# coganlab/cross_patient_speech_decoding

Hardware: AMD Instinct MI355X
Metric: ECoG trials/sec seq2seq-RNN training (higher is better)
Workload: dtype bf16x3; 1 GPU; configs[3] per-GPU shard: 8-patient MCCA-aligned input (d = 30), enc 2x bi-GRU H=512, dec 1x GRU, T=200 (T'=20), F=100, full-batch step of 2048 trials per GPU (8 patients x 2048 trials over 8 GPUs), dropout 0.3, teacher forcing 0.5, clip 0.5, AdamW; trials_per_gpu=2048, global_batch=2048, parallelism=dp1, collective=none (single process)

## Files before the change

cross_patient_speech_decoding_amd/csrc/xps_gru.hip:

```cpp
#include <stdlib.h>
#include "xps_common.h"
#include "xps_gemm_tile.h"
using xps_tile::bf16x4;
using xps_tile::bf16x8;
using xps_tile::bf_split;

bool xps_internal_gru_cluster_usable(int B, int H, int ndir);
size_t xps_internal_gru_cluster_fwd_workspace(int B, int H, int ndir);
size_t xps_internal_gru_cluster_bwd_workspace(int B, int H, int ndir);
size_t xps_internal_gru_cluster_status_offset(int B, int H, int ndir);
int xps_internal_gru_cluster_fwd(const float* gi, const float* const* w_hh, const float* const* b_hh, const float* h0,
                                 float* y_ext, float* saved, int T, int B, int H, int ndir, void* workspace, hipStream_t st,
                                 float* y_split, float* yd_split, float drop_p, unsigned long long drop_seed);
int xps_internal_gru_cluster_bwd(const float* dy, const float* dhn, const float* y_ext, const float* saved,
                                 const float* const* w_hh_t, float* dgi, float* dghn, float* dh0,
                                 int T, int B, int H, int ndir, void* workspace, hipStream_t st, int split_out);
bool xps_internal_gru_cluster_ximg_ok(int B, int H, int ndir);

namespace {

constexpr int GBM = 16;
#ifndef XPS_GRU_BF_WAVES
#define XPS_GRU_BF_WAVES 8
#endif
constexpr int GRU_BF_WAVES = XPS_GRU_BF_WAVES;

struct GruFwdParams {
    const float* gi;
    const float* w_hh[2];
    const float* b_hh[2];
    const float* h0;
    float* y_ext;
    float* saved;
    int T, B, H, ndir, Hp, ldh;
    float* y_drop;
    float drop_p, drop_scale;
    unsigned long long drop_seed;
};

template <bool VEC>
__device__ inline float4 load_w4(const float* __restrict__ row, int k, int H) {
    if (VEC) {
        if (k + 3 < H) return *reinterpret_cast<const float4*>(row + k);
    }
    float4 t = make_float4(0.f, 0.f, 0.f, 0.f);
    if (k + 0 < H) t.x = row[k + 0];
    if (k + 1 < H) t.y = row[k + 1];
    if (k + 2 < H) t.z = row[k + 2];
    if (k + 3 < H) t.w = row[k + 3];
    return t;
}

__device__ inline float f4get(const float4& v, int i) { return i == 0 ? v.x : (i == 1 ? v.y : (i == 2 ? v.z : v.w)); }

template <bool VEC>
__global__ __launch_bounds__(256) void gru_fwd_kernel(GruFwdParams p) {
    extern __shared__ __attribute__((aligned(16))) float lds[];
    const int tid = threadIdx.x, lane = tid & 63, wave = tid >> 6;
    const int n = lane & 15, kq = lane >> 4;
    const int dir = blockIdx.y, b0 = blockIdx.x * GBM;
    const int T = p.T, B = p.B, H = p.H, Hp = p.Hp, ldh = p.ldh;
    const int ldy = p.ndir * H;
    const float* __restrict__ W = p.w_hh[dir];
    const float* __restrict__ bh = p.b_hh[dir];
    const float* __restrict__ gi = p.gi + (long long)dir * T * B * 3 * H;

    for (int i = tid; i < 2 * GBM * ldh; i += 256) lds[i] = 0.f;
    __syncthreads();
    {
        const int slot_h0 = (dir == 0) ? 0 : T + 1, slot_other = (dir == 0) ? T + 1 : 0;
        for (int i = tid; i < GBM * H; i += 256) {
            const int r = i / H, k = i % H, b = b0 + r;
            if (b < B) {
                float v = p.h0 ? p.h0[((long long)dir * B + b) * H + k] : 0.f;
                lds[r * ldh + k] = v;
                p.y_ext[((long long)slot_h0 * B + b) * ldy + dir * H + k] = v;
                p.y_ext[((long long)slot_other * B + b) * ldy + dir * H + k] = 0.f;
            }
        }
    }
    __syncthreads();

    const int ntile = Hp / 16;
    for (int s = 0; s < T; ++s) {
        const int t = (dir == 0) ? s : T - 1 - s;
        const float* hc = lds + (s & 1) * GBM * ldh;
        float* hn = lds + ((s & 1) ^ 1) * GBM * ldh;

        for (int jt = wave; jt < ntile; jt += 4) {
            const int j = jt * 16 + n;
            const int jc = j < H ? j : H - 1;
            float g_r[4], g_z[4], g_n[4];
#pragma unroll
            for (int i = 0; i < 4; ++i) {
                int b = b0 + 4 * kq + i;
                b = b < B ? b : B - 1;
                const float* gp = gi + ((long long)t * B + b) * 3 * H;
                g_r[i] = gp[jc];
                g_z[i] = gp[H + jc];
                g_n[i] = gp[2 * H + jc];
// ... 941 lines not shown
    const int t = (dir == 0) ? p.s : T - 1 - p.s;
    const int slot_prev = (dir == 0) ? t : t + 2;
    const float* __restrict__ in_dhn = p.dhn;
    const float* __restrict__ in_keep = p.keep_in;
    const float* __restrict__ in_dy = p.dy;
    const float* __restrict__ in_saved = p.saved;
    const float* __restrict__ in_y = p.y_ext;
    float* __restrict__ out_dgi = p.dgi;
    float* __restrict__ out_dghn = p.dghn;
    float* __restrict__ out_keep = p.keep_out;
    float* __restrict__ out_dh0 = p.dh0;
#pragma unroll
    for (int jn = 0; jn < 2; ++jn) {
        const int j = n0 + wn + jn * 32 + li;
        if (j >= H) continue;
        float v_base[16], v_dy[16], v_r[16], v_z[16], v_n[16], v_q[16], v_hp[16];
#pragma unroll
        for (int r = 0; r < 16; ++r) {
            const int b = m0 + wm + (r & 3) + 8 * (r >> 2) + 4 * lk;
            const bool ok = b < B;
            const int bc = ok ? b : 0;
            const long long ob = ((long long)dir * B + bc) * H + j;
            v_base[r] = p.first ? (in_dhn ? in_dhn[ob] : 0.f) : in_keep[ob];
            if (!p.final) {
                v_dy[r] = in_dy ? in_dy[((long long)t * B + bc) * ldy + dir * H + j] : 0.f;
                const float* sv = in_saved + (((long long)dir * T + t) * B + bc) * 4 * H;
                v_r[r] = sv[j]; v_z[r] = sv[H + j]; v_n[r] = sv[2 * H + j]; v_q[r] = sv[3 * H + j];
                v_hp[r] = in_y[((long long)slot_prev * B + bc) * ldy + dir * H + j];
            }
        }
#pragma unroll
        for (int r = 0; r < 16; ++r) {
            const int b = m0 + wm + (r & 3) + 8 * (r >> 2) + 4 * lk;
            if (b >= B) continue;
            const long long ob = ((long long)dir * B + b) * H + j;
            float dh = p.first ? v_base[r] : acc[0][jn][r] + v_base[r];
            if (p.final) { out_dh0[ob] = dh; continue; }
            dh += v_dy[r];
            const float rg = v_r[r], zg = v_z[r], ng = v_n[r], q = v_q[r], hp = v_hp[r];
            const float dn = dh * (1.f - zg);
            const float dz = dh * (hp - ng);
            const float dan = dn * (1.f - ng * ng);
            const long long o = (((long long)dir * T + t) * B + b) * 3 * H;
            out_dgi[o + j] = dan * q * rg * (1.f - rg);
            out_dgi[o + H + j] = dz * zg * (1.f - zg);
            out_dgi[o + 2 * H + j] = dan;
            out_dghn[(((long long)dir * T + t) * B + b) * H + j] = dan * rg;
            out_keep[ob] = dh * zg;
        }
    }
}

__global__ void transpose_kernel(const float* __restrict__ src, float* __restrict__ dst, int rows, int cols) {
    __shared__ float tile[32][33];
    const int bx = blockIdx.x * 32, by = blockIdx.y * 32;
    for (int i = threadIdx.y; i < 32; i += blockDim.y) {
        int r = by + i, c = bx + threadIdx.x;
        tile[i][threadIdx.x] = (r < rows && c < cols) ? src[(long long)r * cols + c] : 0.f;
    }
    __syncthreads();
    for (int i = threadIdx.y; i < 32; i += blockDim.y) {
        int c = bx + i, r = by + threadIdx.x;
        if (c < cols && r < rows) dst[(long long)c * rows + r] = tile[threadIdx.x][i];
    }
}

struct TransposeBatch { const float* src[4]; float* dst[4]; };
__global__ void transpose_batched_kernel(TransposeBatch tb, int rows, int cols) {
    __shared__ float tile[32][33];
    const float* __restrict__ src = tb.src[blockIdx.z];
    float* __restrict__ dst = tb.dst[blockIdx.z];
    const int bx = blockIdx.x * 32, by = blockIdx.y * 32;
    for (int i = threadIdx.y; i < 32; i += blockDim.y) {
        int r = by + i, c = bx + threadIdx.x;
        tile[i][threadIdx.x] = (r < rows && c < cols) ? src[(long long)r * cols + c] : 0.f;
    }
    __syncthreads();
    for (int i = threadIdx.y; i < 32; i += blockDim.y) {
        int c = bx + i, r = by + threadIdx.x;
        if (c < cols && r < rows) dst[(long long)c * rows + r] = tile[threadIdx.x][i];
    }
}

inline bool aligned16(const void* p) { return (reinterpret_cast<uintptr_t>(p) & 15) == 0; }

inline bool use_step_path() {
    static const bool on = [] { const char* e = getenv("XPS_GRU_STEP_PATH"); return !(e && e[0] == '0'); }();
    return on;
}

}

static bool cluster_shape_ok(int T, int B, int H, int ndir) {
    return xps_internal_gru_cluster_usable(B, H, ndir) && (long long)ndir * (T + 2) * B * 4 * H * 4 < (1ll << 32);
}

extern "C" size_t xps_gru_seq_fwd_f32_workspace(int T, int B, int H, int ndir) {
    if (T <= 0 || B <= 0 || H <= 0 || (ndir != 1 && ndir != 2)) return 16;
    return cluster_shape_ok(T, B, H, ndir) ? xps_internal_gru_cluster_fwd_workspace(B, H, ndir) : 16;
}

extern "C" long long xps_gru_seq_status_offset(int T, int B, int H, int ndir) {
    if (T <= 0 || B <= 0 || H <= 0 || (ndir != 1 && ndir != 2)) return -1;
    return cluster_shape_ok(T, B, H, ndir) ? (long long)xps_internal_gru_cluster_status_offset(B, H, ndir) : -1;
}

extern "C" int xps_gru_seq_fused_dropout_supported(int T, int B, int H, int ndir) {
    if (T < 1 || B < 1 || (ndir != 1 && ndir != 2)) return 0;
    if (cluster_shape_ok(T, B, H, ndir)) return 0;
    return (H == 128 || H == 64) ? 1 : 0;
}

static int gru_seq_fwd_impl(const float* gi, const float* const* w_hh, const float* const* b_hh,
                            const float* h0, float* y_ext, float* saved,
                            int T, int B, int H, int ndir, float* y_drop, float drop_p, unsigned long long drop_seed,
                            void* workspace, size_t workspace_bytes, void* stream);

extern "C" int xps_gru_seq_fwd_f32(const float* gi, const float* const* w_hh, const float* const* b_hh,
                                   const float* h0, float* y_ext, float* saved,
                                   int T, int B, int H, int ndir, void* workspace, size_t workspace_bytes, void* stream) {
    return gru_seq_fwd_impl(gi, w_hh, b_hh, h0, y_ext, saved, T, B, H, ndir, nullptr, 0.f, 0ull, workspace, workspace_bytes, stream);
}

extern "C" int xps_gru_seq_fwd_drop_f32(const float* gi, const float* const* w_hh, const float* const* b_hh,
                                        const float* h0, float* y_ext, float* saved,
                                        int T, int B, int H, int ndir, float* y_drop, float drop_p, uint64_t drop_seed,
                                        void* workspace, size_t workspace_bytes, void* stream) {
    XPS_CHECK_ARG(y_drop && drop_p >= 0.f && drop_p < 1.f, "y_drop must be given, 0 <= p < 1");
    XPS_CHECK_ARG(xps_gru_seq_fused_dropout_supported(T, B, H, ndir) && aligned16(y_drop),
                  "fused dropout: shape not on the resident kernels (see xps_gru_seq_fused_dropout_supported)");
    return gru_seq_fwd_impl(gi, w_hh, b_hh, h0, y_ext, saved, T, B, H, ndir, y_drop, drop_p, (unsigned long long)drop_seed, workspace,
                            workspace_bytes, stream);
}

extern "C" int xps_gru_seq_fwd_images_supported(int T, int B, int H, int ndir) {
    if (T < 1 || B < 1 || H < 1 || (ndir != 1 && ndir != 2)) return 0;
    return (cluster_shape_ok(T, B, H, ndir) && xps_internal_gemm_mode() == 1 && H % 4 == 0) ? 1 : 0;
}

extern "C" int xps_gru_seq_fwd_image_exchange_supported(int T, int B, int H, int ndir) {
    return (xps_gru_seq_fwd_images_supported(T, B, H, ndir) && xps_internal_gru_cluster_ximg_ok(B, H, ndir)) ? 1 : 0;
}

extern "C" int xps_gru_seq_fwd_images_f32(const float* gi, const float* const* w_hh, const float* const* b_hh,
                                          const float* h0, float* y_ext, float* saved, int T, int B, int H, int ndir,
                                          float* y_split, float* y_drop_split, float drop_p, uint64_t drop_seed,
                                          void* workspace, size_t workspace_bytes, void* stream) {
    XPS_CHECK_ARG(gi && w_hh && b_hh && y_ext, "null argument");
    XPS_CHECK_ARG(T >= 1 && B >= 1 && H >= 1 && (ndir == 1 || ndir == 2), "bad shape");
    XPS_CHECK_ARG(drop_p >= 0.f && drop_p < 1.f, "0 <= p < 1");
    XPS_CHECK_ARG(xps_gru_seq_fwd_images_supported(T, B, H, ndir),
                  "XPS_FMT_SPLIT4 images: cluster-persistent shapes in bf16x3 mode only (see xps_gru_seq_fwd_images_supported)");
    XPS_CHECK_ARG(w_hh[0] && b_hh[0] && (ndir == 1 || (w_hh[1] && b_hh[1])), "null weight pointer");
    if (!workspace || workspace_bytes < xps_gru_seq_fwd_f32_workspace(T, B, H, ndir)) {
        xps_set_error("xps_gru_seq_fwd_images_f32: workspace too small");
        return XPS_E_WORKSPACE;
    }
    return xps_internal_gru_cluster_fwd(gi, w_hh, b_hh, h0, y_ext, saved, T, B, H, ndir, workspace, (hipStream_t)stream,
                                        y_split, y_drop_split, drop_p, (unsigned long long)drop_seed);
}

static int gru_seq_fwd_impl(const float* gi, const float* const* w_hh, const float* const* b_hh,
                            const float* h0, float* y_ext, float* saved,
                            int T, int B, int H, int ndir, float* y_drop, float drop_p, unsigned long long drop_seed,
                            void* workspace, size_t workspace_bytes, void* stream) {
    XPS_CHECK_ARG(gi && w_hh && b_hh && y_ext, "null argument");
    XPS_CHECK_ARG(T >= 1 && B >= 1 && H >= 1, "T, B, H must be >= 1");
    XPS_CHECK_ARG(ndir == 1 || ndir == 2, "ndir must be 1 or 2");
    if (cluster_shape_ok(T, B, H, ndir)) {
        XPS_CHECK_ARG(w_hh[0] && b_hh[0] && (ndir == 1 || (w_hh[1] && b_hh[1])), "null weight pointer");
        if (!workspace || workspace_bytes < xps_gru_seq_fwd_f32_workspace(T, B, H, ndir)) {
            xps_set_error("xps_gru_seq_fwd_f32: workspace too small");
            return XPS_E_WORKSPACE;
        }
        return xps_internal_gru_cluster_fwd(gi, w_hh, b_hh, h0, y_ext, saved, T, B, H, ndir, workspace, (hipStream_t)stream,
                                            nullptr, nullptr, 0.f, 0ull);
    }
    GruFwdParams p;
    p.gi = gi; p.h0 = h0; p.y_ext = y_ext; p.saved = saved;
    p.T = T; p.B = B; p.H = H; p.ndir = ndir;
    p.y_drop = y_drop; p.drop_p = drop_p; p.drop_scale = 1.0f / (1.0f - drop_p); p.drop_seed = drop_seed;
    p.Hp = ((H + 15) / 16) * 16;
    p.ldh = p.Hp + 4;
    bool vec = (H % 4 == 0);
    for (int d = 0; d < 2; ++d) {
        p.w_hh[d] = w_hh[d < ndir ? d : 0];
        p.b_hh[d] = b_hh[d < ndir ? d : 0];
        XPS_CHECK_ARG(p.w_hh[d] && p.b_hh[d], "null weight pointer");
        vec = vec && aligned16(p.w_hh[d]);
    }
    const size_t lds_bytes = (size_t)2 * GBM * p.ldh * sizeof(float);
    XPS_CHECK_ARG(lds_bytes <= 160 * 1024, "hidden size too large for the LDS-resident state tile");
    XPS_CHECK_ARG(!y_drop || vec, "fused dropout needs 16-byte aligned weights");
    if (H > 128 && use_step_path()) {
        hipStream_t st = (hipStream_t)stream;
        hipLaunchKernelGGL(gru_init_slots_kernel, dim3(cdiv((long long)ndir * B * H, 256) > 1024 ? 1024 : cdiv((long long)ndir * B * H, 256)),
                           dim3(256), 0, st, h0, y_ext, T, B, H, ndir);
        GruStepFwd q;
        q.gi = gi; q.y_ext = y_ext; q.saved = saved; q.T = T; q.B = B; q.H = H; q.ndir = ndir;
        for (int d = 0; d < 2; ++d) { q.w_hh[d] = p.w_hh[d]; q.b_hh[d] = p.b_hh[d]; }
        q.vecA = (int)(H % 4 == 0 && aligned16(y_ext));
        q.vecB = (int)vec;
        dim3 sgrid(cdiv(H, 32), cdiv(B, 128), ndir);
        for (int s = 0; s < T; ++s) {
            q.s = s;
            if (xps_internal_gemm_mode() == 1) hipLaunchKernelGGL(gru_step_fwd_kernel<true>, sgrid, dim3(256), 0, st, q);
            else hipLaunchKernelGGL(gru_step_fwd_kernel<false>, sgrid, dim3(256), 0, st, q);
        }
        XPS_CHECK_LAUNCH();
        return XPS_OK;
    }
    dim3 grid(cdiv(B, GBM), ndir);
    if (vec && (H == 128 || H == 64)) {
        const bool bf = xps_internal_gemm_mode() == 1;
        if (H == 128 && bf) hipLaunchKernelGGL((gru_fwd_resident_kernel<128, true, GRU_BF_WAVES>), grid, dim3(GRU_BF_WAVES * 64), 0, (hipStream_t)stream, p);
        else if (H == 128) hipLaunchKernelGGL((gru_fwd_resident_kernel<128, false>), grid, dim3(256), 0, (hipStream_t)stream, p);
        else if (bf) hipLaunchKernelGGL((gru_fwd_resident_kernel<64, true>), grid, dim3(256), 0, (hipStream_t)stream, p);
        else hipLaunchKernelGGL((gru_fwd_resident_kernel<64, false>), grid, dim3(256), 0, (hipStream_t)stream, p);
        XPS_CHECK_LAUNCH();
        return XPS_OK;
    }
    if (vec) {
        if (lds_bytes > 64 * 1024)
            if (hipFuncSetAttribute((const void*)gru_fwd_kernel<true>, hipFuncAttributeMaxDynamicSharedMemorySize, (int)lds_bytes) != hipSuccess) { xps_set_error("hipFuncSetAttribute failed"); return XPS_E_HIP; }
        hipLaunchKernelGGL(gru_fwd_kernel<true>, grid, dim3(256), lds_bytes, (hipStream_t)stream, p);
    } else {
        if (lds_bytes > 64 * 1024)
            if (hipFuncSetAttribute((const void*)gru_fwd_kernel<false>, hipFuncAttributeMaxDynamicSharedMemorySize, (int)lds_bytes) != hipSuccess) { xps_set_error("hipFuncSetAttribute failed"); return XPS_E_HIP; }
        hipLaunchKernelGGL(gru_fwd_kernel<false>, grid, dim3(256), lds_bytes, (hipStream_t)stream, p);
    }
    XPS_CHECK_LAUNCH();
    return XPS_OK;
}

extern "C" size_t xps_gru_seq_bwd_f32_workspace(int T, int B, int H, int ndir) {
    (void)T;
    if (B <= 0 || H <= 0 || ndir <= 0) return 16;
    if (T > 0 && (ndir == 1 || ndir == 2) && cluster_shape_ok(T, B, H, ndir)) return xps_internal_gru_cluster_bwd_workspace(B, H, ndir);
    return (size_t)2 * ndir * B * H * sizeof(float) + 16;
}

static int gru_seq_bwd_impl(const float* dy, const float* dhn, const float* y_ext, const float* saved,
                            const float* const* w_hh, const float* const* w_hh_t, float* dgi, float* dghn, float* dh0,
                            int T, int B, int H, int ndir, int has_drop, float drop_p, unsigned long long drop_seed,
                            void* workspace, size_t workspace_bytes, void* stream, int split_out = 0);

extern "C" int xps_gru_seq_bwd_f32(const float* dy, const float* dhn, const float* y_ext, const float* saved,
                                   const float* const* w_hh, const float* const* w_hh_t, float* dgi, float* dghn, float* dh0,
                                   int T, int B, int H, int ndir, void* workspace, size_t workspace_bytes, void* stream) {
    return gru_seq_bwd_impl(dy, dhn, y_ext, saved, w_hh, w_hh_t, dgi, dghn, dh0, T, B, H, ndir, 0, 0.f, 0ull, workspace, workspace_bytes, stream);
}

extern "C" int xps_gru_seq_bwd_drop_f32(const float* dy, const float* dhn, const float* y_ext, const float* saved,
                                        const float* const* w_hh, const float* const* w_hh_t, float* dgi, float* dghn, float* dh0,
                                        int T, int B, int H, int ndir, float drop_p, uint64_t drop_seed,
                                        void* workspace, size_t workspace_bytes, void* stream) {
    XPS_CHECK_ARG(dy && drop_p >= 0.f && drop_p < 1.f, "dy must be given, 0 <= p < 1");
    XPS_CHECK_ARG(xps_gru_seq_fused_dropout_supported(T, B, H, ndir),
                  "fused dropout: shape not on the resident kernels (see xps_gru_seq_fused_dropout_supported)");
    return gru_seq_bwd_impl(dy, dhn, y_ext, saved, w_hh, w_hh_t, dgi, dghn, dh0, T, B, H, ndir, 1, drop_p, (unsigned long long)drop_seed,
                            workspace, workspace_bytes, stream);
}

extern "C" int xps_gru_seq_bwd_split4_supported(int T, int B, int H, int ndir) {
    if (T < 1 || B < 1 || (ndir != 1 && ndir != 2) || xps_internal_gemm_mode() != 1) return 0;
    if (cluster_shape_ok(T, B, H, ndir)) return 1;
    return xps_gru_seq_fused_dropout_supported(T, B, H, ndir);
}

extern "C" int xps_gru_seq_bwd_split4_f32(const float* dy, const float* dhn, const float* y_ext, const float* saved,
                                          const float* const* w_hh, const float* const* w_hh_t, float* dgi, float* dghn, float* dh0,
                                          int T, int B, int H, int ndir, float drop_p, uint64_t drop_seed,
                                          void* workspace, size_t workspace_bytes, void* stream) {
    XPS_CHECK_ARG(drop_p >= 0.f && drop_p < 1.f, "0 <= p < 1");
    XPS_CHECK_ARG(drop_p == 0.f || (dy && xps_gru_seq_fused_dropout_supported(T, B, H, ndir) && !cluster_shape_ok(T, B, H, ndir)),
                  "fused dropout: dy must be given and the shape must be on the resident kernels");
    return gru_seq_bwd_impl(dy, dhn, y_ext, saved, w_hh, w_hh_t, dgi, dghn, dh0, T, B, H, ndir, drop_p > 0.f ? 1 : 0, drop_p,
                            (unsigned long long)drop_seed, workspace, workspace_bytes, stream, 1);
}

static int gru_seq_bwd_impl(const float* dy, const float* dhn, const float* y_ext, const float* saved,
                            const float* const* w_hh, const float* const* w_hh_t, float* dgi, float* dghn, float* dh0,
                            int T, int B, int H, int ndir, int has_drop, float drop_p, unsigned long long drop_seed,
                            void* workspace, size_t workspace_bytes, void* stream, int split_out) {
    XPS_CHECK_ARG(y_ext && saved && w_hh && w_hh_t && dgi && dghn, "null argument");
    XPS_CHECK_ARG(!split_out || xps_gru_seq_bwd_split4_supported(T, B, H, ndir),
                  "XPS_FMT_SPLIT4 outputs: shape / precision mode not served (see xps_gru_seq_bwd_split4_supported)");
    XPS_CHECK_ARG(dy || dhn, "at least one of dy / dhn must be given");
    XPS_CHECK_ARG(T >= 1 && B >= 1 && H >= 1, "T, B, H must be >= 1");
    XPS_CHECK_ARG(ndir == 1 || ndir == 2, "ndir must be 1 or 2");
    if (cluster_shape_ok(T, B, H, ndir)) {
        XPS_CHECK_ARG(w_hh_t[0] && (ndir == 1 || w_hh_t[1]), "null weight pointer");
        if (!workspace || workspace_bytes < xps_gru_seq_bwd_f32_workspace(T, B, H, ndir)) {
            xps_set_error("xps_gru_seq_bwd_f32: workspace too small");
            return XPS_E_WORKSPACE;
        }
        return xps_internal_gru_cluster_bwd(dy, dhn, y_ext, saved, w_hh_t, dgi, dghn, dh0, T, B, H, ndir, workspace, (hipStream_t)stream, split_out);
    }
    GruBwdParams p;
    p.dy = dy; p.dhn = dhn; p.y_ext = y_ext; p.saved = saved; p.dgi = dgi; p.dghn = dghn; p.dh0 = dh0;
    p.T = T; p.B = B; p.H = H; p.ndir = ndir;
    p.has_drop = has_drop; p.drop_p = drop_p; p.drop_scale = 1.0f / (1.0f - drop_p); p.drop_seed = drop_seed;
    p.split_out = split_out;
    p.Hp = ((H + 15) / 16) * 16;
    p.ldg = 3 * p.Hp + 4;
    p.ldc = p.Hp + 4;
    bool vec = (H % 4 == 0);
    for (int d = 0; d < 2; ++d) {
        p.w_hh_t[d] = w_hh_t[d < ndir ? d : 0];
        XPS_CHECK_ARG(p.w_hh_t[d], "null weight pointer");
        vec = vec && aligned16(p.w_hh_t[d]);
    }
    const size_t lds_bytes = (size_t)GBM * (p.ldg + p.ldc) * sizeof(float);
    XPS_CHECK_ARG(lds_bytes <= 160 * 1024, "hidden size too large for the LDS-resident gradient tile");
    XPS_CHECK_ARG(!has_drop || vec, "fused dropout needs 16-byte aligned weights");
    XPS_CHECK_ARG(!split_out || (vec && (H == 128 || H == 64)), "XPS_FMT_SPLIT4 outputs need the resident kernels (16-byte aligned weights)");
    if (H > 128 && use_step_path()) {
        if (!workspace || workspace_bytes < xps_gru_seq_bwd_f32_workspace(T, B, H, ndir) || !aligned16(workspace)) {
            xps_set_error("xps_gru_seq_bwd_f32: workspace too small or misaligned");
            return XPS_E_WORKSPACE;
        }
        hipStream_t st = (hipStream_t)stream;
        GruStepBwd q;
        q.dy = dy; q.dhn = dhn; q.y_ext = y_ext; q.saved = saved; q.dgi = dgi; q.dghn = dghn; q.dh0 = dh0;
        q.T = T; q.B = B; q.H = H; q.ndir = ndir;
        bool vb = (H % 4 == 0);
        for (int d = 0; d < 2; ++d) {
            q.w_hh[d] = w_hh[d < ndir ? d : 0];
            XPS_CHECK_ARG(q.w_hh[d], "null weight pointer");
            vb = vb && aligned16(q.w_hh[d]);
        }
        q.vecB = (int)vb;
        q.vecA1 = (int)(H % 4 == 0 && aligned16(dgi));
        q.vecA2 = (int)(H % 4 == 0 && aligned16(dghn));
        float* keep[2] = {(float*)workspace, (float*)workspace + (size_t)ndir * B * H};
        dim3 sgrid(cdiv(H, 128), cdiv(B, 64), ndir);
        int pp = 0;
        for (int s = T - 1; s >= 0; --s) {
            q.s = s; q.first = (s == T - 1); q.final = 0;
            q.keep_in = keep[pp]; q.keep_out = keep[pp ^ 1];
            if (xps_internal_gemm_mode() == 1) hipLaunchKernelGGL(gru_step_bwd_kernel<true>, sgrid, dim3(256), 0, st, q);
            else hipLaunchKernelGGL(gru_step_bwd_kernel<false>, sgrid, dim3(256), 0, st, q);
            pp ^= 1;
        }
        if (dh0) {
            q.s = 0; q.first = 0; q.final = 1; q.keep_in = keep[pp]; q.keep_out = keep[pp ^ 1];
            if (xps_internal_gemm_mode() == 1) hipLaunchKernelGGL(gru_step_bwd_kernel<true>, sgrid, dim3(256), 0, st, q);
            else hipLaunchKernelGGL(gru_step_bwd_kernel<false>, sgrid, dim3(256), 0, st, q);
        }
        XPS_CHECK_LAUNCH();
        return XPS_OK;
    }
    dim3 grid(cdiv(B, GBM), ndir);
    if (vec && (H == 128 || H == 64)) {
        const bool bf = xps_internal_gemm_mode() == 1;
        if (H == 128 && bf) hipLaunchKernelGGL((gru_bwd_resident_kernel<128, true, GRU_BF_WAVES>), grid, dim3(GRU_BF_WAVES * 64), 0, (hipStream_t)stream, p);
        else if (H == 128) hipLaunchKernelGGL((gru_bwd_resident_kernel<128, false>), grid, dim3(256), 0, (hipStream_t)stream, p);
        else if (bf) hipLaunchKernelGGL((gru_bwd_resident_kernel<64, true>), grid, dim3(256), 0, (hipStream_t)stream, p);
        else hipLaunchKernelGGL((gru_bwd_resident_kernel<64, false>), grid, dim3(256), 0, (hipStream_t)stream, p);
        XPS_CHECK_LAUNCH();
        return XPS_OK;
    }
    if (vec) {
        if (lds_bytes > 64 * 1024)
            if (hipFuncSetAttribute((const void*)gru_bwd_kernel<true>, hipFuncAttributeMaxDynamicSharedMemorySize, (int)lds_bytes) != hipSuccess) { xps_set_error("hipFuncSetAttribute failed"); return XPS_E_HIP; }
        hipLaunchKernelGGL(gru_bwd_kernel<true>, grid, dim3(256), lds_bytes, (hipStream_t)stream, p);
    } else {
        if (lds_bytes > 64 * 1024)
            if (hipFuncSetAttribute((const void*)gru_bwd_kernel<false>, hipFuncAttributeMaxDynamicSharedMemorySize, (int)lds_bytes) != hipSuccess) { xps_set_error("hipFuncSetAttribute failed"); return XPS_E_HIP; }
        hipLaunchKernelGGL(gru_bwd_kernel<false>, grid, dim3(256), lds_bytes, (hipStream_t)stream, p);
    }
    XPS_CHECK_LAUNCH();
    return XPS_OK;
}

#ifdef XPS_STAMP
extern "C" int xps_debug_read_stamps(unsigned long long* host, int n) {
    return hipMemcpyFromSymbol(host, HIP_SYMBOL(g_stamp), sizeof(unsigned long long) * n) == hipSuccess ? 0 : -2;
}
#endif

extern "C" int xps_transpose_f32(const float* src, float* dst, int rows, int cols, void* stream) {
    XPS_CHECK_ARG(src && dst && rows >= 0 && cols >= 0, "bad argument");
    if (rows == 0 || cols == 0) return XPS_OK;
    dim3 grid(cdiv(cols, 32), cdiv(rows, 32));
    hipLaunchKernelGGL(transpose_kernel, grid, dim3(32, 8), 0, (hipStream_t)stream, src, dst, rows, cols);
    XPS_CHECK_LAUNCH();
    return XPS_OK;
}

extern "C" int xps_transpose_batched_f32(const float* const* src, float* const* dst, int n, int rows, int cols, void* stream) {
    XPS_CHECK_ARG(src && dst && n >= 1 && n <= 4 && rows >= 0 && cols >= 0, "bad argument (1..4 matrices)");
    if (rows == 0 || cols == 0) return XPS_OK;
    TransposeBatch tb;
    for (int i = 0; i < 4; ++i) {
        const int j = i < n ? i : 0;
        XPS_CHECK_ARG(src[j] && dst[j], "null matrix pointer");
        tb.src[i] = src[j]; tb.dst[i] = dst[j];
    }
    hipLaunchKernelGGL(transpose_batched_kernel, dim3(cdiv(cols, 32), cdiv(rows, 32), n), dim3(32, 8), 0, (hipStream_t)stream,
                       tb, rows, cols);
    XPS_CHECK_LAUNCH();
    return XPS_OK;
}
```

cross_patient_speech_decoding_amd/csrc/xps_gru_cluster.hip:

```cpp
#include <stdlib.h>
#include <string.h>
#include <type_traits>
#include "xps_common.h"
#include <atomic>
#include "xps_gemm_tile.h"
using xps_tile::bf16x4;
using xps_tile::bf16x8;
using xps_tile::bf_split;

namespace {

typedef unsigned u32x4 __attribute__((ext_vector_type(4)));
typedef unsigned u32x2 __attribute__((ext_vector_type(2)));
constexpr int AUX_SC1 = 16;
constexpr unsigned RSRC_FLAGS = 0x00020000;

template <int KSPLIT, bool BF, int KSEG>
struct ClCfg {
    static constexpr int KP = 256 * KSPLIT;
    static constexpr int NUT = 4 / KSPLIT;
    static constexpr int U = 16 * NUT;
    static constexpr int CHUNK_BYTES = 32 * KP * 4;
    static constexpr int NPIECE = CHUNK_BYTES / 1024;
    static constexpr int TRIAL_BYTES = KP * 4;
    static constexpr int PPT = TRIAL_BYTES / 1024;
    static constexpr int TS = TRIAL_BYTES + 32;
    static constexpr int PS = BF ? (PPT == 2 ? 1040 : 512) : 0;
    static constexpr int TILE_BYTES = 32 * TS;
    static constexpr int XACC_BYTES = KSEG == 1 ? 4 * 2 * 3 * 1024 : 2 * 4 * 2 * 1024;
    static constexpr int LDS_BYTES = 2 * TILE_BYTES + XACC_BYTES + 64;
    static constexpr int KSEGS = KSEG;
    __host__ __device__ static constexpr int piece_off(int j) {
        return PPT == 2 ? (j >> 1) * TS + (j & 1) * (BF ? PS : 1024) : j * TS;
    }
};

#ifdef XPS_CL_STAMP
__device__ unsigned long long g_clstamp[2048 * 8];
__device__ unsigned long long g_clstamp2[2048 * 8];
#define CL_STAMP(var)                                                                  \
    __builtin_amdgcn_sched_barrier(0);                                                 \
    asm volatile("s_memtime %0\n\ts_waitcnt lgkmcnt(0)" : "=s"(var)::"memory");        \
    __builtin_amdgcn_sched_barrier(0);
#define CL_ACC(sum, a, b) sum += (b) - (a);
#else
#define CL_STAMP(var)
#define CL_ACC(sum, a, b)
#endif

__device__ inline float cl_sigmoid(float x) { return __builtin_amdgcn_rcpf(1.0f + __expf(-x)); }
__device__ inline float cl_tanh(float x) { return 2.0f * cl_sigmoid(2.0f * x) - 1.0f; }

__device__ inline void cl_wait(const unsigned* flags, unsigned need, int cs, int lane, unsigned first, unsigned* status, unsigned* sticky) {
    unsigned v = first;
    if (__all(v >= need)) return;
    const unsigned long long t0 = __builtin_amdgcn_s_memrealtime();
    bool ok = false;
    for (;;) {
        v = need;
        if (lane < cs) v = __hip_atomic_load(flags + lane, __ATOMIC_RELAXED, __HIP_MEMORY_SCOPE_AGENT);
        if (__all(v >= need)) { ok = true; break; }
        __builtin_amdgcn_s_sleep(2);
        if (__builtin_amdgcn_s_memrealtime() - t0 > 300000000ull) break;
    }
    if (lane == 0) {
        const unsigned dt = (unsigned)(__builtin_amdgcn_s_memrealtime() - t0);
        if (!ok) {
            __hip_atomic_store(status, 1u, __ATOMIC_RELAXED, __HIP_MEMORY_SCOPE_AGENT);
            if (sticky) __hip_atomic_store(sticky, 1u, __ATOMIC_RELAXED, __HIP_MEMORY_SCOPE_AGENT);
        }
        __hip_atomic_fetch_add(status + 1, 1u, __ATOMIC_RELAXED, __HIP_MEMORY_SCOPE_AGENT);
        __hip_atomic_fetch_add(status + 2, dt, __ATOMIC_RELAXED, __HIP_MEMORY_SCOPE_AGENT);
        __hip_atomic_fetch_max(status + 3, dt, __ATOMIC_RELAXED, __HIP_MEMORY_SCOPE_AGENT);
    }
}

__device__ inline bool cl_same_xcd(unsigned* tab, int member, int cs, int lane, bool leader, unsigned* status, unsigned* sticky, unsigned* lds_word) {
    if (leader) {
        unsigned id;
        asm volatile("s_getreg_b32 %0, hwreg(HW_REG_XCC_ID)" : "=s"(id));
        id = (id & 15u) + 1u;
        if (lane == 0) __hip_atomic_store(tab + member, id, __ATOMIC_RELAXED, __HIP_MEMORY_SCOPE_AGENT);
        const unsigned long long t0 = __builtin_amdgcn_s_memrealtime();
        unsigned v = id;
        bool ok = false;
        for (;;) {
            v = id;
            if (lane < cs) v = __hip_atomic_load(tab + lane, __ATOMIC_RELAXED, __HIP_MEMORY_SCOPE_AGENT);
// ... 405 lines not shown
            const unsigned so = !live ? CL_OOB : p.saved_mm
                ? (unsigned)((((((long long)dir * T + t) * p.CS + cm.member) * B + b) * 128 + (ju & 31)) * 4)
                : (unsigned)(((((long long)dir * T + t) * B + b) * 4 * H + ju) * 4);
            __builtin_amdgcn_raw_buffer_store_b128(__builtin_bit_cast(u32x4, rg), sr, so, 0, 0);
            __builtin_amdgcn_raw_buffer_store_b128(__builtin_bit_cast(u32x4, zg), sr, live ? so + gstride : CL_OOB, 0, 0);
            __builtin_amdgcn_raw_buffer_store_b128(__builtin_bit_cast(u32x4, ng), sr, live ? so + 2u * gstride : CL_OOB, 0, 0);
            __builtin_amdgcn_raw_buffer_store_b128(__builtin_bit_cast(u32x4, qv), sr, live ? so + 3u * gstride : CL_OOB, 0, 0);
        }
    };
    f32x4 prod[3];
    auto take_products = [&](int rounds_done) {
#pragma unroll
        for (int g = 0; g < 3; ++g) {
            const int ut_ = guq >> 2, te_ = gtr >> 4, lo_ = ((guq & 3) * 16 + (gtr & 15)) * 16;
            const f32x4 lo = *reinterpret_cast<const f32x4*>(xacc + (((2 * ut_) * 2 + te_) * 3 + g) * 1024 + lo_);
            const f32x4 hi = *reinterpret_cast<const f32x4*>(xacc + (((2 * ut_ + 1) * 2 + te_) * 3 + g) * 1024 + lo_);
            prod[g] = lo + hi;
        }
        if (lane == 0) __hip_atomic_store(consumed + hw, (unsigned)rounds_done, __ATOMIC_RELEASE, __HIP_MEMORY_SCOPE_WORKGROUP);
    };

    EpiIn ein[3];
    int s_pv = p.s_begin, r_pv = -1;
    int s_n2 = p.s_begin, r_n2 = 0;
    epi_load(s_n2, r_n2, ein[0]);
    if (++r_n2 == NR) { r_n2 = 0; ++s_n2; }
    if (it_begin + 1 < it_end) epi_load(s_n2, r_n2, ein[1]);
    if (++r_n2 == NR) { r_n2 = 0; ++s_n2; }
    auto round_body = [&](int it, auto SLOT) {
        constexpr int cur = decltype(SLOT)::value;
        constexpr int prv = (cur + 2) % 3;
        if (p.handoff && wave == 4 && lane == 0 && it >= it_begin + 2) {
            int rp = r_pv - 1, sp = s_pv;
            if (rp < 0) { rp = NR - 1; --sp; }
            __hip_atomic_store(myflags + rp * 16 + cm.member, (unsigned)(sp + 1), __ATOMIC_RELAXED, __HIP_MEMORY_SCOPE_AGENT);
        }
        const bool do_poll = p.handoff && wave == 4 && it + 2 < it_end && s_n2 > p.s_begin;
        unsigned fl = 0xffffffffu;
        if (do_poll && lane < p.CS) fl = __hip_atomic_load(myflags + r_n2 * 16 + lane, __ATOMIC_RELAXED, __HIP_MEMORY_SCOPE_AGENT);
        CL_FENCE();
        int younger = 0;
        if (it > it_begin) {
            take_products(it - it_begin);
            epilogue(s_pv, r_pv, ein[prv], prod);
            younger += (has_saved ? 5 : 1) + (images ? 2 : 0) + (img_drop ? 1 : 0);
        }
        CL_FENCE();
        if (it + 2 < it_end) {
            epi_load(s_n2, r_n2, ein[prv]);
#ifndef XPS_CL_ABL_NOLOAD
            younger += 4;
#endif
        }
        CL_FENCE();
        CL_STAMP(sb3)
        cl_wait_vmcnt(younger);
        if (do_poll) cl_wait(myflags + r_n2 * 16, (unsigned)s_n2, p.CS, lane, fl, p.status, p.sticky);
        CL_STAMP(sb0)
        __syncthreads();
        CL_STAMP(sb1)
        CL_ACC(s_bar, sb0, sb1) CL_ACC(s_work, sb2, sb3) CL_ACC(s_drain, sb3, sb0)
#ifdef XPS_CL_STAMP
        sb2 = sb1;
#endif
        if (++r_pv == NR) { r_pv = 0; ++s_pv; }
        if (++r_n2 == NR) { r_n2 = 0; ++s_n2; }
    };
    for (int it = it_begin; it < it_end; it += 3) {
        round_body(it, std::integral_constant<int, 0>{});
        if (it + 1 < it_end) round_body(it + 1, std::integral_constant<int, 1>{});
        if (it + 2 < it_end) round_body(it + 2, std::integral_constant<int, 2>{});
    }
    if (it_end > it_begin) {
        take_products(it_end - it_begin);
        const int slot = (it_end - 1 - it_begin) % 3;
        if (slot == 0) epilogue(s_pv, r_pv, ein[0], prod);
        else if (slot == 1) epilogue(s_pv, r_pv, ein[1], prod);
        else epilogue(s_pv, r_pv, ein[2], prod);
    }
    CL_STORE_STAMPS()
}

template <bool BF>
__global__ void gru_cluster_init_kernel(const float* __restrict__ h0, float* __restrict__ y_ext, void* __restrict__ xbuf,
                                        int T, int B, int H, int ndir, int Bp, int KP, u32x4* __restrict__ header, int header_u4,
                                        float* __restrict__ y_split) {
    for (int i = blockIdx.x * blockDim.x + threadIdx.x; i < header_u4; i += gridDim.x * blockDim.x) header[i] = (u32x4){0u, 0u, 0u, 0u};
    const long long total = (long long)ndir * Bp * (KP / 4);
    for (long long i = (long long)blockIdx.x * blockDim.x + threadIdx.x; i < total; i += (long long)gridDim.x * blockDim.x) {
        const int k = (int)(i % (KP / 4)) * 4;
        const long long rb = i / (KP / 4);
        const int b = (int)(rb % Bp), dir = (int)(rb / Bp);
        f32x4 v = {0.f, 0.f, 0.f, 0.f};
        const bool in = b < B && k < H;
        if (in && h0) v = *reinterpret_cast<const f32x4*>(h0 + ((long long)dir * B + b) * H + k);
        if (in) {
            const int slot_h0 = (dir == 0) ? 0 : T + 1, slot_other = (dir == 0) ? T + 1 : 0;
            const int ldy = ndir * H;
            *reinterpret_cast<f32x4*>(y_ext + ((long long)slot_h0 * B + b) * ldy + dir * H + k) = v;
            *reinterpret_cast<f32x4*>(y_ext + ((long long)slot_other * B + b) * ldy + dir * H + k) = (f32x4){0.f, 0.f, 0.f, 0.f};
            if constexpr (BF) {
                if (y_split) {
                    *reinterpret_cast<f32x4*>(y_split + ((long long)slot_h0 * B + b) * ldy + dir * H + k) = split4_pack(v);
                    *reinterpret_cast<f32x4*>(y_split + ((long long)slot_other * B + b) * ldy + dir * H + k) = (f32x4){0.f, 0.f, 0.f, 0.f};
                }
            }
        }
        if (!xbuf) continue;
        unsigned char* row = reinterpret_cast<unsigned char*>(xbuf) + ((long long)dir * Bp + b) * KP * 4;
        if constexpr (BF) {
            if (XPS_CL_FWD_PLANES) {
                bf16x4 sh, sl;
#pragma unroll
                for (int e = 0; e < 4; ++e) { __bf16 a, c; bf_split(v[e], a, c); sh[e] = a; sl[e] = c; }
                *reinterpret_cast<bf16x4*>(row + k * 2) = sh;
                *reinterpret_cast<bf16x4*>(row + KP * 2 + k * 2) = sl;
            } else {
                *reinterpret_cast<f32x4*>(row + (k & ~31) * 4 + cl_xslot((unsigned)k >> 2) * 16) = split4_pack(v);
            }
        } else {
            *reinterpret_cast<f32x4*>(row + k * 4) = v;
        }
    }
}

struct ClBwd {
    const float* dy;
    const float* dhn;
    const float* y_ext;
    const float* saved;
    const float* w_hh_t[2];
    float* dgi;
    float* dghn;
    float* dh0;
    float* keep;
    void* xbuf;
    unsigned* flags;
    unsigned* xcc;
    unsigned* status;
    unsigned* sticky;
    unsigned xbuf_bytes;
    int T, B, H, ndir, Bp, Mc, NR, nblk, CS;
    int ps_begin, ps_end, ps_total, handoff;
    int saved_mm;
    int split_out;
};

template <int KSPLIT, bool BF, bool XOUT = false>
__global__ __launch_bounds__(512, 2) void gru_cluster_bwd_kernel(ClBwd p) {
    static_assert(KSPLIT == 2, "the cluster kernels cover 256 < H <= 512");
    static_assert(!XOUT || BF, "outputs as exchange rows: bf16x3 mode only");
    using Cf = ClCfg<KSPLIT, BF, 3>;
    constexpr int KP = Cf::KP, TS = Cf::TS, PS = Cf::PS, TILE = Cf::TILE_BYTES;
    extern __shared__ __attribute__((aligned(16))) unsigned char smem[];
    unsigned char* xacc = smem + 2 * TILE;
    const unsigned lds0 = cl_lds_base(smem);
    const int tid = threadIdx.x, lane = tid & 63;
    const int wave = __builtin_amdgcn_readfirstlane(tid >> 6);
    const int n = lane & 15, kq = lane >> 4;
    const ClMap cm = cl_map(p.CS);
    const int dir = cm.cluster / p.nblk, blk = cm.cluster % p.nblk;
    const int T = p.T, B = p.B, H = p.H, NR = p.NR;
    const int ldy = p.ndir * H;
    const int m_base = blk * p.Mc;
    const int NQ = 3 * NR;
    unsigned* myflags = p.flags + (long long)cm.cluster * NR * 16;
    const bool fast = !p.handoff || cl_same_xcd(p.xcc + cm.cluster * 16, cm.member, p.CS, lane, wave == 4, p.status, p.sticky, reinterpret_cast<unsigned*>(smem));

    const int hw = wave >= 4 ? wave - 4 : 0;
    const int gtr = 8 * hw + (lane >> 3);
    const int guq = lane & 7;
    const int ju = cm.member * Cf::U + 4 * guq;
    const bool ulive = ju < H;
    const int juc = ulive ? ju : 0;
    __amdgpu_buffer_rsrc_t xr = __builtin_amdgcn_make_buffer_rsrc(p.xbuf, 0, p.xbuf_bytes, RSRC_FLAGS);
    __amdgpu_buffer_rsrc_t kr = __builtin_amdgcn_make_buffer_rsrc(p.keep, 0, (unsigned)((long long)p.ndir * p.CS * B * 32 * 4), RSRC_FLAGS);
    __amdgpu_buffer_rsrc_t gr = __builtin_amdgcn_make_buffer_rsrc(p.dgi, 0, (unsigned)((long long)p.ndir * T * B * 3 * H * 4), RSRC_FLAGS);
    __amdgpu_buffer_rsrc_t nr = __builtin_amdgcn_make_buffer_rsrc(p.dghn, 0, (unsigned)((long long)p.ndir * T * B * H * 4), RSRC_FLAGS);
    __amdgpu_buffer_rsrc_t hr = __builtin_amdgcn_make_buffer_rsrc(p.dh0, 0, p.dh0 ? (unsigned)((long long)p.ndir * B * H * 4) : 0u, RSRC_FLAGS);
    const bool has_dy = p.dy != nullptr;

    const unsigned char* xb = reinterpret_cast<const unsigned char*>(p.xbuf);
    const int dw = wave & 3;
    auto dma_src = [&](int ps_, int r_, int g_) -> const unsigned char* {
        if constexpr (XOUT) {
            const int sp = T - 1 - (ps_ - 1);
            const int tp = (dir == 0) ? sp : T - 1 - sp;
            const long long row = ((long long)dir * T + tp) * B + m_base + 32 * r_ + 8 * dw;
            const float* base = g_ < 2 ? p.dgi + row * 3 * H + g_ * H : p.dghn + row * H;
            return reinterpret_cast<const unsigned char*>(base) + cl_ximg_lane(lane) * 16;
        }
        const size_t chunk = (size_t)(((((ps_ - 1) & 1) * p.ndir + dir) * (p.Bp / 32) + (m_base / 32) + r_) * 3 + g_);
        return xb + chunk * Cf::CHUNK_BYTES + (size_t)(dw * 16) * 1024 + lane * 16;
    };
    auto dma_group = [&](const unsigned char* src, int buf, int grp, int g_ = 0) {
        const int j = dw * 16 + grp * 4;
        const unsigned base = lds0 + (unsigned)(buf * TILE) + (unsigned)((j >> 1) * TS);
        const unsigned h = BF ? PS : 1024;
        if constexpr (XOUT) {
            const long long st = (g_ < 2 ? 3LL : 1LL) * H * 4;
            cl_dma2x2(src + (2 * grp) * st, src + (2 * grp + 1) * st, base, base + h - 1024, base + TS, base + TS + h - 1024);
        } else {
            cl_dma4(src + grp * 4096, base, base + h - 1024, base + TS - 2048, base + TS + h - 3072);
        }
    };

// ... 999 lines not shown
    pl.grid = ndir * pl.nblk * 16;
    pl.flags_bytes = (((size_t)ndir * pl.nblk * (pl.NR * 160 + 16) * 4 + 256 + 255) / 256) * 256;
    pl.keep_bytes = (((size_t)ndir * B * 16 * 32 * 4 + 255) / 256) * 256;
    pl.xbuf = (size_t)2 * ndir * (pl.Bp / C2_RT) * 4 * C2_IMG;
    pl.pbuf = (size_t)2 * ndir * pl.nblk * pl.NR * 64 * 2048;
    pl.ok = pl.xbuf < ((size_t)1 << 31) && pl.pbuf < ((size_t)1 << 32);
    return pl;
}

template <typename K>
bool cl_set_lds(K kernel, int bytes) {
    return hipFuncSetAttribute((const void*)kernel, hipFuncAttributeMaxDynamicSharedMemorySize, bytes) == hipSuccess;
}

inline bool cl_aligned16(const void* p) { return (reinterpret_cast<uintptr_t>(p) & 15) == 0; }

template <typename K>
int cl_resident(K kernel, int lds, int kind, int bf) {
    const int dev = cl_device();
    if (dev < 0) return 0;
    std::atomic<int>& slot = g_cldev[dev].resident[kind][bf];
    int v = slot.load(std::memory_order_relaxed);
    if (v < 0) {
        int per_cu = 0;
        if (hipOccupancyMaxActiveBlocksPerMultiprocessor(&per_cu, (const void*)kernel, 512, (size_t)lds) != hipSuccess) per_cu = 0;
        v = per_cu * cl_num_cus();
        slot.store(v, std::memory_order_relaxed);
    }
    return v;
}

bool cl_ximg_enabled() {
    const char* e = getenv("XPS_GRU_XIMG");
    return !(e && e[0] == '0');
}

bool cl_xout_enabled() {
    const char* e = getenv("XPS_GRU_XOUT");
    return e && e[0] == '1';
}

unsigned* cl_sticky() {
    const int dev = cl_device();
    return dev < 0 ? nullptr : g_cldev[dev].sticky;
}

}

extern "C" int xps_gru_set_status_word(unsigned* device_word) {
    const int dev = cl_device();
    if (dev < 0) { xps_set_error("xps_gru_set_status_word: no current device"); return XPS_E_HIP; }
    g_cldev[dev].sticky = device_word;
    return XPS_OK;
}

bool xps_internal_gru_cluster_usable(int B, int H, int ndir) { return cl_plan(B, H, ndir).ok; }

size_t xps_internal_gru_cluster_fwd_workspace(int B, int H, int ndir) {
    const ClPlan pl = cl_plan(B, H, ndir);
    return pl.ok ? pl.flags_bytes + pl.xbuf_fwd : 0;
}

size_t xps_internal_gru_cluster_bwd_workspace(int B, int H, int ndir) {
    const ClPlan pl = cl_plan(B, H, ndir);
    if (!pl.ok) return 0;
    size_t n = pl.flags_bytes + pl.keep_bytes + pl.xbuf_bwd;
    const ClPlan2 p2 = cl_plan2(B, H, ndir);
    if (p2.ok) { const size_t n2 = p2.flags_bytes + p2.keep_bytes + p2.xbuf + p2.pbuf; if (n2 > n) n = n2; }
    return n;
}

size_t xps_internal_gru_cluster_status_offset(int B, int H, int ndir) {
    const ClPlan pl = cl_plan(B, H, ndir);
    return pl.ok ? pl.flags_bytes - 256 : 0;
}

bool xps_internal_gru_cluster_ximg_ok(int B, int H, int ndir) {
    const ClPlan pl = cl_plan(B, H, ndir);
    return pl.ok && H == pl.KP && pl.Bp == B && cl_ximg_enabled();
}

int xps_internal_gru_cluster_fwd(const float* gi, const float* const* w_hh, const float* const* b_hh, const float* h0,
                                 float* y_ext, float* saved, int T, int B, int H, int ndir, void* workspace, hipStream_t st,
                                 float* y_split, float* yd_split, float drop_p, unsigned long long drop_seed) {
    const ClPlan pl = cl_plan(B, H, ndir);
    if (!pl.ok) { xps_set_error("gru cluster forward: unsupported shape"); return XPS_E_INVALID; }
    const bool bf = xps_internal_gemm_mode() == 1;
    if ((y_split || yd_split) && (!bf || H % 4 != 0 || !cl_aligned16(y_split) || !cl_aligned16(yd_split))) {
        xps_set_error("gru cluster forward: XPS_FMT_SPLIT4 images exist in bf16x3 mode only (H a multiple of 4, 16-byte aligned)");
        return XPS_E_INVALID;
    }
    ClFwd p;
    p.gi = gi; p.y_ext = y_ext; p.saved = saved;
    p.y_split = y_split; p.yd_split = yd_split; p.drop_p = drop_p; p.drop_scale = 1.0f / (1.0f - drop_p); p.drop_seed = drop_seed;
    const bool ximg = bf && y_split && H == pl.KP && pl.Bp == B && cl_ximg_enabled();
    for (int d = 0; d < 2; ++d) { p.w_hh[d] = w_hh[d < ndir ? d : 0]; p.b_hh[d] = b_hh[d < ndir ? d : 0]; }
    if (!cl_aligned16(gi) || !cl_aligned16(y_ext) || !cl_aligned16(saved) || !cl_aligned16(p.w_hh[0]) || !cl_aligned16(p.w_hh[1]) ||
        !cl_aligned16(p.b_hh[0]) || !cl_aligned16(p.b_hh[1]) || !cl_aligned16(h0) || !cl_aligned16(workspace)) {
        xps_set_error("gru cluster forward: operands must be 16-byte aligned");
        return XPS_E_INVALID;
    }
    unsigned char* ws = (unsigned char*)workspace;
    p.flags = (unsigned*)ws;
    p.xcc = p.flags + (size_t)ndir * pl.nblk * pl.NR * 16;
    p.status = (unsigned*)(ws + pl.flags_bytes - 256);
    p.xbuf = ws + pl.flags_bytes;
    p.xbuf_bytes = (unsigned)pl.xbuf_fwd;
    p.T = T; p.B = B; p.H = H; p.ndir = ndir; p.Bp = pl.Bp; p.Mc = pl.Mc; p.NR = pl.NR; p.nblk = pl.nblk; p.CS = pl.CS;
    p.saved_mm = (H % 32 == 0) ? 1 : 0;
    if (pl.CS * pl.U < pl.KP) {
        if (hipMemsetAsync(p.xbuf, 0, pl.xbuf_fwd, st) != hipSuccess) { xps_set_error("gru cluster forward: memset failed"); return XPS_E_HIP; }
    }
    {
        const long long total = (long long)ndir * pl.Bp * (pl.KP / 4);
        const int blocks = (int)((total + 255) / 256 > 2048 ? 2048 : (total + 255) / 256);
        if (bf) hipLaunchKernelGGL(gru_cluster_init_kernel<true>, dim3(blocks), dim3(256), 0, st, h0, y_ext, ximg ? (void*)nullptr : p.xbuf, T, B, H, ndir, pl.Bp, pl.KP, (u32x4*)ws, (int)(pl.flags_bytes / 16), y_split);
        else hipLaunchKernelGGL(gru_cluster_init_kernel<false>, dim3(blocks), dim3(256), 0, st, h0, y_ext, p.xbuf, T, B, H, ndir, pl.Bp, pl.KP, (u32x4*)ws, (int)(pl.flags_bytes / 16), (float*)nullptr);
    }
    p.sticky = cl_sticky();
    auto launch = [&](auto kernel, int lds) -> bool {
        if (!cl_set_lds(kernel, lds)) return false;
        const bool persistent = cl_mode() == 2 && pl.grid <= cl_resident(kernel, lds, ximg ? 3 : 0, bf ? 1 : 0);
        if (persistent) {
            p.s_begin = 0; p.s_end = T; p.handoff = 1;
            hipLaunchKernelGGL(kernel, dim3(pl.grid), dim3(512), lds, st, p);
        } else {
            p.handoff = 0;
            for (int s = 0; s < T; ++s) {
                p.s_begin = s; p.s_end = s + 1;
                hipLaunchKernelGGL(kernel, dim3(pl.grid), dim3(512), lds, st, p);
            }
        }
        return true;
    };
    bool ok;
    ok = ximg ? launch(gru_cluster_fwd_kernel<2, true, true>, ClCfg<2, true, 1>::LDS_BYTES)
       : bf ? launch(gru_cluster_fwd_kernel<2, true>, ClCfg<2, true, 1>::LDS_BYTES) : launch(gru_cluster_fwd_kernel<2, false>, ClCfg<2, false, 1>::LDS_BYTES);
    if (!ok) { xps_set_error("gru cluster forward: cannot raise the dynamic LDS limit"); return XPS_E_HIP; }
    XPS_CHECK_LAUNCH();
    return XPS_OK;
}

int xps_internal_gru_cluster_bwd(const float* dy, const float* dhn, const float* y_ext, const float* saved,
                                 const float* const* w_hh_t, float* dgi, float* dghn, float* dh0,
                                 int T, int B, int H, int ndir, void* workspace, hipStream_t st, int split_out) {
    const ClPlan pl = cl_plan(B, H, ndir);
    if (!pl.ok) { xps_set_error("gru cluster backward: unsupported shape"); return XPS_E_INVALID; }
    const bool bf = xps_internal_gemm_mode() == 1;
    if (split_out && !bf) { xps_set_error("gru cluster backward: XPS_FMT_SPLIT4 outputs exist in bf16x3 mode only"); return XPS_E_INVALID; }
    const ClPlan2 p2 = cl_plan2(B, H, ndir);
    if (bf && p2.ok) {
        ClBwd2 q;
        q.dy = dy; q.dhn = dhn; q.y_ext = y_ext; q.saved = saved; q.dgi = dgi; q.dghn = dghn; q.dh0 = dh0;
        q.split_out = split_out;
        for (int d = 0; d < 2; ++d) q.w_hh_t[d] = w_hh_t[d < ndir ? d : 0];
        if (!cl_aligned16(dy) || !cl_aligned16(dhn) || !cl_aligned16(y_ext) || !cl_aligned16(saved) || !cl_aligned16(q.w_hh_t[0]) ||
            !cl_aligned16(q.w_hh_t[1]) || !cl_aligned16(dgi) || !cl_aligned16(dghn) || !cl_aligned16(dh0) || !cl_aligned16(workspace)) {
            xps_set_error("gru cluster backward: operands must be 16-byte aligned");
            return XPS_E_INVALID;
        }
        unsigned char* ws = (unsigned char*)workspace;
        q.flags = (unsigned*)ws;
        q.xcc = q.flags + (size_t)ndir * p2.nblk * p2.NR * 160;
        q.status = (unsigned*)(ws + p2.flags_bytes - 256);
        q.sticky = cl_sticky();
        q.keep = (float*)(ws + p2.flags_bytes);
        q.xbuf = ws + p2.flags_bytes + p2.keep_bytes;
        q.pbuf = (float*)(ws + p2.flags_bytes + p2.keep_bytes + p2.xbuf);
        q.xbuf_bytes = (unsigned)p2.xbuf;
        q.pbuf_bytes = (unsigned)p2.pbuf;
        q.T = T; q.B = B; q.H = H; q.ndir = ndir; q.Bp = p2.Bp; q.Mc = p2.Mc; q.NR = p2.NR; q.nblk = p2.nblk;
        q.saved_mm = (H % 32 == 0) ? 1 : 0;
        if (hipMemsetAsync(ws, 0, p2.flags_bytes, st) != hipSuccess) { xps_set_error("gru cluster backward: memset failed"); return XPS_E_HIP; }
        const int ps_total = T + (dh0 ? 1 : 0);
        q.ps_total = ps_total;
        if (!cl_set_lds(gru_cluster2_bwd_kernel, C2_LDS)) { xps_set_error("gru cluster backward: cannot raise the dynamic LDS limit"); return XPS_E_HIP; }
        const int n_it = (ps_total - 1) * p2.NR;
        const bool persistent = cl_mode() == 2 && p2.grid <= cl_resident(gru_cluster2_bwd_kernel, C2_LDS, 2, 1);
        if (persistent) {
            q.handoff = 1; q.do_ps0 = 1; q.c_begin = 0; q.c_end = n_it; q.g_begin = 0; q.g_end = n_it;
            hipLaunchKernelGGL(gru_cluster2_bwd_kernel, dim3(p2.grid), dim3(512), C2_LDS, st, q);
        } else {
            q.handoff = 0; q.do_ps0 = 1; q.c_begin = q.c_end = q.g_begin = q.g_end = 0;
            hipLaunchKernelGGL(gru_cluster2_bwd_kernel, dim3(p2.grid), dim3(512), C2_LDS, st, q);
            q.do_ps0 = 0;
            for (int ps = 1; ps < ps_total; ++ps) {
                q.c_begin = (ps - 1) * p2.NR; q.c_end = ps * p2.NR; q.g_begin = q.g_end = 0;
                hipLaunchKernelGGL(gru_cluster2_bwd_kernel, dim3(p2.grid), dim3(512), C2_LDS, st, q);
                q.g_begin = q.c_begin; q.g_end = q.c_end; q.c_begin = q.c_end = 0;
                hipLaunchKernelGGL(gru_cluster2_bwd_kernel, dim3(p2.grid), dim3(512), C2_LDS, st, q);
            }
        }
        XPS_CHECK_LAUNCH();
        return XPS_OK;
    }
    ClBwd p;
    p.dy = dy; p.dhn = dhn; p.y_ext = y_ext; p.saved = saved; p.dgi = dgi; p.dghn = dghn; p.dh0 = dh0;
    if (split_out && !bf) { xps_set_error("gru cluster backward: XPS_FMT_SPLIT4 outputs exist in bf16x3 mode only"); return XPS_E_INVALID; }
    p.split_out = split_out;
    for (int d = 0; d < 2; ++d) p.w_hh_t[d] = w_hh_t[d < ndir ? d : 0];
    if (!cl_aligned16(dy) || !cl_aligned16(dhn) || !cl_aligned16(y_ext) || !cl_aligned16(saved) || !cl_aligned16(p.w_hh_t[0]) ||
        !cl_aligned16(p.w_hh_t[1]) || !cl_aligned16(dgi) || !cl_aligned16(dghn) || !cl_aligned16(dh0) || !cl_aligned16(workspace)) {
        xps_set_error("gru cluster backward: operands must be 16-byte aligned");
        return XPS_E_INVALID;
    }
    unsigned char* ws = (unsigned char*)workspace;
    p.flags = (unsigned*)ws;
    p.xcc = p.flags + (size_t)ndir * pl.nblk * pl.NR * 16;
    p.status = (unsigned*)(ws + pl.flags_bytes - 256);
    p.keep = (float*)(ws + pl.flags_bytes);
    p.xbuf = ws + pl.flags_bytes + pl.keep_bytes;
    p.xbuf_bytes = (unsigned)pl.xbuf_bwd;
    p.T = T; p.B = B; p.H = H; p.ndir = ndir; p.Bp = pl.Bp; p.Mc = pl.Mc; p.NR = pl.NR; p.nblk = pl.nblk; p.CS = pl.CS;
    p.saved_mm = (H % 32 == 0) ? 1 : 0;
    const bool xout = bf && split_out && H == pl.KP && pl.Bp == B && cl_xout_enabled();
    if (hipMemsetAsync(ws, 0, pl.flags_bytes, st) != hipSuccess) { xps_set_error("gru cluster backward: memset failed"); return XPS_E_HIP; }
    if (pl.CS * pl.U < pl.KP) {
        if (hipMemsetAsync(p.xbuf, 0, pl.xbuf_bwd, st) != hipSuccess) { xps_set_error("gru cluster backward: memset failed"); return XPS_E_HIP; }
    }
    const int ps_total = T + (dh0 ? 1 : 0);
    p.ps_total = ps_total;
    p.sticky = cl_sticky();
    auto launch = [&](auto kernel, int lds) -> bool {
        if (!cl_set_lds(kernel, lds)) return false;
        const bool persistent = cl_mode() == 2 && pl.grid <= cl_resident(kernel, lds, xout ? 4 : 1, bf ? 1 : 0);
        if (persistent) {
            p.ps_begin = 0; p.ps_end = ps_total; p.handoff = 1;
            hipLaunchKernelGGL(kernel, dim3(pl.grid), dim3(512), lds, st, p);
        } else {
            p.handoff = 0;
            for (int ps = 0; ps < ps_total; ++ps) {
                p.ps_begin = ps; p.ps_end = ps + 1;
                hipLaunchKernelGGL(kernel, dim3(pl.grid), dim3(512), lds, st, p);
            }
        }
        return true;
    };
    bool ok;
    ok = xout ? launch(gru_cluster_bwd_kernel<2, true, true>, ClCfg<2, true, 3>::LDS_BYTES)
       : bf ? launch(gru_cluster_bwd_kernel<2, true>, ClCfg<2, true, 3>::LDS_BYTES) : launch(gru_cluster_bwd_kernel<2, false>, ClCfg<2, false, 3>::LDS_BYTES);
    if (!ok) { xps_set_error("gru cluster backward: cannot raise the dynamic LDS limit"); return XPS_E_HIP; }
    XPS_CHECK_LAUNCH();
    return XPS_OK;
}

extern "C" long long xps_debug_gru_bwd_status_offset(int B, int H, int ndir) {
    const ClPlan2 p2 = cl_plan2(B, H, ndir);
    if (xps_internal_gemm_mode() == 1 && p2.ok) return (long long)p2.flags_bytes - 256;
    const ClPlan pl = cl_plan(B, H, ndir);
    return pl.ok ? (long long)pl.flags_bytes - 256 : -1;
}

#ifdef XPS_CL_STAMP
extern "C" int xps_debug_read_cluster_stamps2(unsigned long long* host, int n) {
    return hipMemcpyFromSymbol(host, HIP_SYMBOL(g_clstamp2), sizeof(unsigned long long) * n) == hipSuccess ? 0 : -2;
}
extern "C" int xps_debug_read_cluster_stamps(unsigned long long* host, int n) {
    return hipMemcpyFromSymbol(host, HIP_SYMBOL(g_clstamp), sizeof(unsigned long long) * n) == hipSuccess ? 0 : -2;
}
#endif

extern "C" int xps_set_gru_cluster_mode(int mode) {
    if (mode < 0 || mode > 2) { xps_set_error("xps_set_gru_cluster_mode: mode must be 0 (off), 1 (one step per launch) or 2 (persistent)"); return XPS_E_INVALID; }
    g_cluster_mode = mode;
    return XPS_OK;
}
extern "C" int xps_get_gru_cluster_mode(void) { return cl_mode(); }
extern "C" int xps_set_gru_bptt_grid(int two_dimensional) {
    if (two_dimensional != 0 && two_dimensional != 1) { xps_set_error("xps_set_gru_bptt_grid: 0 (1-D cluster kernel) or 1 (4 x 4 grid)"); return XPS_E_INVALID; }
    g_cl2 = two_dimensional;
    return XPS_OK;
}
extern "C" int xps_get_gru_bptt_grid(void) { return cl2_enabled() ? 1 : 0; }
```

cross_patient_speech_decoding_amd/csrc/xps_nn.hip:

```cpp
#include "xps_common.h"
#include "xps_ce.h"

namespace {

constexpr int RED_ROWS = 64;

__global__ __launch_bounds__(256) void colsum_stage1(const float* __restrict__ X, long long ldx, int rows, int cols,
                                                     float* __restrict__ part, float* __restrict__ part_sq) {
    __shared__ float s1[4][64], s2[4][64];
    const int c = blockIdx.x * 64 + (threadIdx.x & 63), rq = threadIdx.x >> 6;
    const int r0 = blockIdx.y * RED_ROWS;
    const int r1 = min(rows, r0 + RED_ROWS);
    float a = 0.f, a2 = 0.f;
    if (c < cols) {
#pragma unroll 4
        for (int r = r0 + rq; r < r1; r += 4) {
            float v = X[(long long)r * ldx + c];
            a += v;
            a2 += v * v;
        }
    }
    s1[rq][threadIdx.x & 63] = a;
    s2[rq][threadIdx.x & 63] = a2;
    __syncthreads();
    if (rq == 0 && c < cols) {
        const int l = threadIdx.x;
        part[(long long)blockIdx.y * cols + c] = (s1[0][l] + s1[1][l]) + (s1[2][l] + s1[3][l]);
        if (part_sq) part_sq[(long long)blockIdx.y * cols + c] = (s2[0][l] + s2[1][l]) + (s2[2][l] + s2[3][l]);
    }
}

constexpr int S2_GROUPS = 16;
__global__ __launch_bounds__(1024) void colsum_stage2(const float* __restrict__ part, const float* __restrict__ part_sq,
                                                      int nparts, int cols, float* __restrict__ out,
                                                      float* __restrict__ out_sq, int accumulate,
                                                      float* __restrict__ acc_lo = nullptr, float* __restrict__ acc_hi = nullptr,
                                                      int split = 0) {
    __shared__ float s1[S2_GROUPS][64], s2[S2_GROUPS][64];
    const int l = threadIdx.x & 63, q = threadIdx.x >> 6;
    const int c = blockIdx.x * 64 + l;
    float a = 0.f, a2 = 0.f;
    if (c < cols) {
        int i = q;
        for (; i + 7 * S2_GROUPS < nparts; i += 8 * S2_GROUPS) {
            float v[8], w[8];
#pragma unroll
            for (int u = 0; u < 8; ++u) {
                v[u] = part[(long long)(i + u * S2_GROUPS) * cols + c];
                w[u] = part_sq ? part_sq[(long long)(i + u * S2_GROUPS) * cols + c] : 0.f;
            }
#pragma unroll
            for (int u = 0; u < 8; ++u) { a += v[u]; a2 += w[u]; }
        }
        for (; i < nparts; i += S2_GROUPS) {
            a += part[(long long)i * cols + c];
            if (part_sq) a2 += part_sq[(long long)i * cols + c];
        }
    }
    s1[q][l] = a;
    s2[q][l] = a2;
    __syncthreads();
    if (q == 0 && c < cols) {
        a = 0.f; a2 = 0.f;
#pragma unroll
        for (int k = 0; k < S2_GROUPS; ++k) { a += s1[k][l]; a2 += s2[k][l]; }
        if (accumulate) {
            a += out[c];
            if (out_sq) a2 += out_sq[c];
        }
        out[c] = a;
        if (out_sq) out_sq[c] = a2;
        if (acc_lo && c < split) acc_lo[c] += a;
        if (acc_hi && c >= split) acc_hi[c - split] += a;
    }
}

__device__ __forceinline__ double bn_stats_mean(const float* __restrict__ stats, double count, int c) {
    return (double)stats[c] / count;
}
__device__ __forceinline__ double bn_stats_var(const float* __restrict__ stats, double count, int F, int c, double m) {
    const double d = m - (double)(float)m;
    double var = (double)stats[F + c] / count - d * d;
    return var < 0 ? 0 : var;
}
// ... 137 lines not shown
                                    long long total, int F) {
    for (long long i = (long long)blockIdx.x * blockDim.x + threadIdx.x; i < total; i += (long long)gridDim.x * blockDim.x) {
        const int c = (int)(i % F);
        float g = dout[i];
        if (mask) g = g * mask[i] * scale;
        if (relu && !(out[i] > 0.f)) g = 0.f;
        const float xh = (y[i] - mean[c]) * rstd[c];
        dy[i] = gamma[c] * rstd[c] * (g - sums[c] * inv_count - xh * sums[F + c] * inv_count);
    }
}

__global__ void gather_rows_kernel(const float* __restrict__ table, const long long* __restrict__ idx, float* __restrict__ out,
                                   int B, int cols, int n_rows) {
    const long long total = (long long)B * cols;
    for (long long i = (long long)blockIdx.x * blockDim.x + threadIdx.x; i < total; i += (long long)gridDim.x * blockDim.x) {
        const int b = (int)(i / cols), c = (int)(i % cols);
        long long r = idx[b];
        r = r < 0 ? 0 : (r >= n_rows ? n_rows - 1 : r);
        out[i] = table[r * cols + c];
    }
}

constexpr int SC_CHUNK = 64, SC_MAXROWS = 16;
__global__ __launch_bounds__(256) void scatter_rows_stage1(const float* __restrict__ dout, const long long* __restrict__ idx,
                                                           float* __restrict__ part, int B, int cols, int n_rows) {
    __shared__ float tab[4][SC_MAXROWS][64];
    const int l = threadIdx.x & 63, q = threadIdx.x >> 6;
    const int c = blockIdx.x * 64 + l;
    for (int r = 0; r < n_rows; ++r) tab[q][r][l] = 0.f;
    const int b0 = blockIdx.y * SC_CHUNK;
    const int b1 = min(B, b0 + SC_CHUNK);
    if (c < cols)
        for (int b = b0 + q; b < b1; b += 4) {
            long long r = idx[b];
            r = r < 0 ? 0 : (r >= n_rows ? n_rows - 1 : r);
            tab[q][r][l] += dout[(long long)b * cols + c];
        }
    __syncthreads();
    if (c < cols)
        for (int r = q; r < n_rows; r += 4)
            part[((long long)blockIdx.y * n_rows + r) * cols + c] = (tab[0][r][l] + tab[1][r][l]) + (tab[2][r][l] + tab[3][r][l]);
}
__global__ __launch_bounds__(256) void scatter_rows_stage2(const float* __restrict__ part, int nchunks, float* __restrict__ dtable,
                                                           long long total, int accumulate) {
    __shared__ float red[4][64];
    const int l = threadIdx.x & 63, w = threadIdx.x >> 6;
    const long long i = (long long)blockIdx.x * 64 + l;
    float a = 0.f;
    if (i < total) {
        int k = w;
        for (; k + 28 < nchunks; k += 32) {
            float v[8];
#pragma unroll
            for (int u = 0; u < 8; ++u) v[u] = part[(long long)(k + 4 * u) * total + i];
#pragma unroll
            for (int u = 0; u < 8; ++u) a += v[u];
        }
        for (; k < nchunks; k += 4) a += part[(long long)k * total + i];
    }
    red[w][l] = a;
    __syncthreads();
    if (w == 0 && i < total) {
        a = (red[0][l] + red[1][l]) + (red[2][l] + red[3][l]);
        dtable[i] = accumulate ? dtable[i] + a : a;
    }
}

__global__ void next_token_kernel(const float* __restrict__ logits, int C, const long long* __restrict__ teacher,
                                  long long tstride, const int* __restrict__ use_teacher, long long* __restrict__ next, int B) {
    const int b = blockIdx.x * blockDim.x + threadIdx.x;
    if (b >= B) return;
    if (use_teacher && teacher && use_teacher[0]) {
        next[b] = teacher[(long long)b * tstride];
        return;
    }
    const float* p = logits + (long long)b * C;
    float best = p[0];
    int bi = 0;
    for (int c = 1; c < C; ++c)
        if (p[c] > best) { best = p[c]; bi = c; }
    next[b] = bi;
}

constexpr int SEL_MAXC = 16;
__global__ __launch_bounds__(256) void decoder_select_kernel(const float* __restrict__ h, const float* __restrict__ w_fc,
                                                             const float* __restrict__ b_fc, float* __restrict__ logits,
                                                             const long long* __restrict__ teacher, long long tstride,
                                                             const int* __restrict__ use_teacher, const float* __restrict__ table,
                                                             long long* __restrict__ next, float* __restrict__ gi_next,
                                                             int B, int H, int C, int ntok) {
    const int lane = threadIdx.x & 63;
    const int b = blockIdx.x * 4 + (threadIdx.x >> 6);
    if (b >= B) return;
    float acc[SEL_MAXC];
#pragma unroll
    for (int c = 0; c < SEL_MAXC; ++c) acc[c] = 0.f;
    const float* hr = h + (long long)b * H;
    for (int k = lane * 4; k < H; k += 256) {
        const f32x4 hv = *reinterpret_cast<const f32x4*>(hr + k);
#pragma unroll
        for (int c = 0; c < SEL_MAXC; ++c) {
            if (c < C) {
                const f32x4 wv = *reinterpret_cast<const f32x4*>(w_fc + (long long)c * H + k);
                acc[c] += (hv[0] * wv[0] + hv[1] * wv[1]) + (hv[2] * wv[2] + hv[3] * wv[3]);
            }
        }
    }
#pragma unroll
    for (int c = 0; c < SEL_MAXC; ++c) {
        if (c < C) {
#pragma unroll
            for (int o = 32; o > 0; o >>= 1) acc[c] += __shfl_xor(acc[c], o);
        }
    }
    float best = 0.f;
    int bi = 0;
#pragma unroll
    for (int c = 0; c < SEL_MAXC; ++c) {
        if (c < C) {
            const float v = acc[c] + b_fc[c];
            if (lane == c) logits[(long long)b * C + c] = v;
            if (c == 0 || v > best) { best = v; bi = c; }
        }
    }
    if (!next) return;
    long long tok = bi;
    if (use_teacher && teacher && use_teacher[0]) tok = teacher[(long long)b * tstride];
    if (lane == 0) next[b] = tok;
    if (gi_next && tok >= 0 && tok < ntok) {
        const float* src = table + tok * 3LL * H;
        float* dst = gi_next + (long long)b * 3 * H;
        for (int k = lane * 4; k < 3 * H; k += 256) *reinterpret_cast<f32x4*>(dst + k) = *reinterpret_cast<const f32x4*>(src + k);
    }
}

__global__ void mask_scale_kernel(const float* __restrict__ x, const float* __restrict__ mask, float scale,
                                  float* __restrict__ out, long long n) {
    for (long long i = (long long)blockIdx.x * blockDim.x + threadIdx.x; i < n; i += (long long)gridDim.x * blockDim.x)
        out[i] = x[i] * mask[i] * scale;
}

template <bool VEC>
__global__ void dropout_kernel(const float* __restrict__ x, float* __restrict__ out, float* __restrict__ mask,
                               long long n, float p, float scale, unsigned long long seed) {
    if (VEC) {
        const long long nquad = n / 4;
        for (long long q = (long long)blockIdx.x * blockDim.x + threadIdx.x; q < nquad; q += (long long)gridDim.x * blockDim.x) {
            const f32x4 m = dropout_keep4(seed, q, p);
            if (mask) *reinterpret_cast<f32x4*>(mask + 4 * q) = m;
            if (x) {
                const f32x4 v = *reinterpret_cast<const f32x4*>(x + 4 * q);
                *reinterpret_cast<f32x4*>(out + 4 * q) = v * m * scale;
            }
        }
        return;
    }
    const long long npair = (n + 1) / 2;
    for (long long q = (long long)blockIdx.x * blockDim.x + threadIdx.x; q < npair; q += (long long)gridDim.x * blockDim.x) {
        float u0, u1;
        rng_pair(seed, q, u0, u1);
        const long long i = 2 * q;
        const float m0 = u0 >= p ? 1.f : 0.f, m1 = u1 >= p ? 1.f : 0.f;
        if (i + 1 < n) {
            if (mask) *reinterpret_cast<float2*>(mask + i) = make_float2(m0, m1);
            if (x) {
                const float2 v = *reinterpret_cast<const float2*>(x + i);
                *reinterpret_cast<float2*>(out + i) = make_float2(v.x * m0 * scale, v.y * m1 * scale);
            }
        } else {
            if (mask) mask[i] = m0;
            if (x) out[i] = x[i] * m0 * scale;
        }
    }
}

__global__ void split4_kernel(const float* __restrict__ x, float* __restrict__ out, long long nquad, float p, float scale,
                              unsigned long long seed) {
    for (long long q = (long long)blockIdx.x * blockDim.x + threadIdx.x; q < nquad; q += (long long)gridDim.x * blockDim.x) {
        f32x4 v = *reinterpret_cast<const f32x4*>(x + 4 * q);
        if (p > 0.f) v = v * dropout_keep4(seed, q, p) * scale;
        *reinterpret_cast<f32x4*>(out + 4 * q) = split4_pack(v);
    }
}

__global__ void add_kernel(const float* __restrict__ a, const float* __restrict__ b, float* __restrict__ out, long long n) {
    for (long long i = (long long)blockIdx.x * blockDim.x + threadIdx.x; i < n; i += (long long)gridDim.x * blockDim.x)
        out[i] = a[i] + b[i];
}

__global__ void ce_rows_kernel(const float* __restrict__ logits, const long long* __restrict__ target,
                               float* __restrict__ row_loss, long long rows, int C) {
    const long long r = (long long)blockIdx.x * blockDim.x + threadIdx.x;
    if (r >= rows) return;
    const float* p = logits + r * C;
    float mx = p[0];
    for (int c = 1; c < C; ++c) mx = fmaxf(mx, p[c]);
    float s = 0.f;
    for (int c = 0; c < C; ++c) s += expf(p[c] - mx);
    row_loss[r] = (logf(s) + mx) - p[target[r]];
}

__global__ __launch_bounds__(1024) void ce_mean_kernel(const float* __restrict__ row_loss, long long rows, float* loss) {
    __shared__ double sh[1024];
    double a = 0.0;
    for (long long i = threadIdx.x; i < rows; i += 1024) a += (double)row_loss[i];
    sh[threadIdx.x] = a;
    __syncthreads();
    for (int s = 512; s > 0; s >>= 1) {
        if ((int)threadIdx.x < s) sh[threadIdx.x] += sh[threadIdx.x + s];
        __syncthreads();
    }
    if (threadIdx.x == 0) loss[0] = (float)(sh[0] / (double)rows);
}

constexpr int CE_FUSED_ROWS = 1024;
__global__ __launch_bounds__(1024) void ce_fused_kernel(const float* __restrict__ logits, const long long* __restrict__ target,
                                                        float* __restrict__ row_loss, float* __restrict__ loss, long long rows,
                                                        int C) {
    __shared__ double sh[1024];
    double a = 0.0;
    for (long long r = threadIdx.x; r < rows; r += 1024) {
        const float* p = logits + r * C;
        float mx = p[0];
        for (int c = 1; c < C; ++c) mx = fmaxf(mx, p[c]);
        float s = 0.f;
        for (int c = 0; c < C; ++c) s += expf(p[c] - mx);
        const float l = (logf(s) + mx) - p[target[r]];
        row_loss[r] = l;
        a += (double)l;
    }
    sh[threadIdx.x] = a;
    __syncthreads();
    for (int s = 512; s > 0; s >>= 1) {
        if ((int)threadIdx.x < s) sh[threadIdx.x] += sh[threadIdx.x + s];
        __syncthreads();
    }
    if (threadIdx.x == 0) loss[0] = (float)(sh[0] / (double)rows);
}

__global__ void ce_bwd_kernel(const float* __restrict__ logits, const long long* __restrict__ target,
                              const float* __restrict__ gout, float* __restrict__ dlogits, long long rows, int C) {
    const long long r = (long long)blockIdx.x * blockDim.x + threadIdx.x;
    if (r >= rows) return;
    const float* p = logits + r * C;
    float mx = p[0];
    for (int c = 1; c < C; ++c) mx = fmaxf(mx, p[c]);
    float s = 0.f;
    for (int c = 0; c < C; ++c) s += expf(p[c] - mx);
    const float g = gout[0] / (float)rows, inv = 1.f / s;
    const long long tg = target[r];
    for (int c = 0; c < C; ++c) dlogits[r * C + c] = g * (expf(p[c] - mx) * inv - (c == tg ? 1.f : 0.f));
}

constexpr int SS_CHUNK = 2048;
__global__ __launch_bounds__(256) void sumsq_stage1(const float* __restrict__ g, long long n, double* __restrict__ part) {
    __shared__ double sh[256];
    const long long i0 = (long long)blockIdx.x * SS_CHUNK;
    const long long i1 = i0 + SS_CHUNK < n ? i0 + SS_CHUNK : n;
    double a = 0.0;
    for (long long i = i0 + threadIdx.x; i < i1; i += 256) { const double v = g[i]; a += v * v; }
    sh[threadIdx.x] = a;
    __syncthreads();
    for (int s = 128; s > 0; s >>= 1) {
        if ((int)threadIdx.x < s) sh[threadIdx.x] += sh[threadIdx.x + s];
        __syncthreads();
// ... 190 lines not shown
                       dout, out, y, mean, rstd, drop_mask, drop_scale, relu, (long long)rows, F, part);
    XPS_CHECK_LAUNCH();
    hipLaunchKernelGGL(colsum_stage2, dim3(cdiv(2 * F, 64)), dim3(1024), 0, (hipStream_t)stream,
                       part, (const float*)nullptr, nparts, 2 * F, sums, (float*)nullptr, 0, dbeta_acc, dgamma_acc, F);
    XPS_CHECK_LAUNCH();
    return XPS_OK;
}

extern "C" int xps_bn_bwd_apply_f32(const float* dout, const float* out, const float* y, const float* mean,
                                    const float* rstd, const float* gamma, const float* drop_mask, float drop_scale,
                                    int relu, const float* sums, double count, float* dy, int64_t rows, int F,
                                    void* stream) {
    XPS_CHECK_ARG(dout && y && mean && rstd && gamma && sums && dy && rows >= 0 && F >= 1 && count >= 1, "bad argument");
    XPS_CHECK_ARG(!relu || out, "relu backward needs the forward output");
    const long long total = (long long)rows * F;
    if (total == 0) return XPS_OK;
    hipLaunchKernelGGL(bn_bwd_apply_kernel, dim3(ew_grid(total)), dim3(256), 0, (hipStream_t)stream,
                       dout, out, y, mean, rstd, gamma, drop_mask, drop_scale, relu, sums, (float)(1.0 / count), dy,
                       total, F);
    XPS_CHECK_LAUNCH();
    return XPS_OK;
}

extern "C" int xps_gather_rows_f32(const float* table, const int64_t* idx, float* out, int B, int cols, int n_rows,
                                   void* stream) {
    XPS_CHECK_ARG(table && idx && out && B >= 0 && cols >= 1 && n_rows >= 1, "bad argument");
    if (B == 0) return XPS_OK;
    hipLaunchKernelGGL(gather_rows_kernel, dim3(ew_grid((long long)B * cols)), dim3(256), 0, (hipStream_t)stream,
                       table, (const long long*)idx, out, B, cols, n_rows);
    XPS_CHECK_LAUNCH();
    return XPS_OK;
}

extern "C" size_t xps_scatter_rows_f32_workspace(int B, int cols, int n_rows) {
    if (B <= 0 || cols <= 0 || n_rows <= 0) return 16;
    return (size_t)cdiv(B, SC_CHUNK) * n_rows * cols * sizeof(float) + 16;
}

extern "C" int xps_scatter_rows_f32(const float* dout, const int64_t* idx, float* dtable, int B, int cols, int n_rows,
                                    int accumulate, void* workspace, size_t workspace_bytes, void* stream) {
    XPS_CHECK_ARG(dout && idx && dtable && B >= 0 && cols >= 1 && n_rows >= 1, "bad argument");
    XPS_CHECK_ARG(n_rows <= SC_MAXROWS, "table has too many rows for the scatter kernel (max 16)");
    if (workspace_bytes < xps_scatter_rows_f32_workspace(B, cols, n_rows) || !workspace) {
        xps_set_error("xps_scatter_rows_f32: workspace too small");
        return XPS_E_WORKSPACE;
    }
    const int nchunks = B > 0 ? cdiv(B, SC_CHUNK) : 0;
    float* part = (float*)workspace;
    if (nchunks > 0) {
        hipLaunchKernelGGL(scatter_rows_stage1, dim3(cdiv(cols, 64), nchunks), dim3(256), 0, (hipStream_t)stream,
                           dout, (const long long*)idx, part, B, cols, n_rows);
        XPS_CHECK_LAUNCH();
    }
    const long long total = (long long)n_rows * cols;
    hipLaunchKernelGGL(scatter_rows_stage2, dim3(cdiv(total, 64)), dim3(256), 0, (hipStream_t)stream,
                       part, nchunks, dtable, total, accumulate);
    XPS_CHECK_LAUNCH();
    return XPS_OK;
}

extern "C" int xps_next_token(const float* logits, int n_classes, const int64_t* teacher, int64_t teacher_stride,
                              const int32_t* use_teacher, int64_t* next, int B, void* stream) {
    XPS_CHECK_ARG(logits && next && n_classes >= 1 && B >= 0, "bad argument");
    if (B == 0) return XPS_OK;
    hipLaunchKernelGGL(next_token_kernel, dim3(cdiv(B, 256)), dim3(256), 0, (hipStream_t)stream,
                       logits, n_classes, (const long long*)teacher, (long long)teacher_stride, (const int*)use_teacher,
                       (long long*)next, B);
    XPS_CHECK_LAUNCH();
    return XPS_OK;
}

extern "C" int xps_decoder_select_f32(const float* h, const float* w_fc, const float* b_fc, float* logits,
                                      const int64_t* teacher, int64_t teacher_stride, const int32_t* use_teacher,
                                      const float* table, int64_t* next, float* gi_next, int B, int H, int C, int ntok,
                                      void* stream) {
    XPS_CHECK_ARG(h && w_fc && b_fc && logits && B >= 0 && H >= 4 && C >= 1, "bad argument");
    XPS_CHECK_ARG(C <= SEL_MAXC && H % 4 == 0, "at most 16 classes, H a multiple of 4");
    XPS_CHECK_ARG(!gi_next || (table && next && ntok >= 1), "the gather needs the table and the token output");
    const uintptr_t bits = reinterpret_cast<uintptr_t>(h) | reinterpret_cast<uintptr_t>(w_fc) | reinterpret_cast<uintptr_t>(table) |
                           reinterpret_cast<uintptr_t>(gi_next);
    XPS_CHECK_ARG((bits & 15) == 0, "h, w_fc, table and gi_next must be 16-byte aligned");
    if (B == 0) return XPS_OK;
    hipLaunchKernelGGL(decoder_select_kernel, dim3(cdiv(B, 4)), dim3(256), 0, (hipStream_t)stream, h, w_fc, b_fc, logits,
                       (const long long*)teacher, (long long)teacher_stride, (const int*)use_teacher, table, (long long*)next,
                       gi_next, B, H, C, ntok);
    XPS_CHECK_LAUNCH();
    return XPS_OK;
}

extern "C" int xps_mask_scale_f32(const float* x, const float* mask, float scale, float* out, int64_t n, void* stream) {
    XPS_CHECK_ARG(x && mask && out && n >= 0, "bad argument");
    if (n == 0) return XPS_OK;
    hipLaunchKernelGGL(mask_scale_kernel, dim3(ew_grid(n)), dim3(256), 0, (hipStream_t)stream, x, mask, scale, out,
                       (long long)n);
    XPS_CHECK_LAUNCH();
    return XPS_OK;
}

extern "C" int xps_dropout_f32(const float* x, float* out, float* mask, int64_t n, float p, uint64_t seed, void* stream) {
    XPS_CHECK_ARG(n >= 0 && p >= 0.f && p < 1.f, "bad argument");
    XPS_CHECK_ARG(mask || x, "nothing to produce: give mask, or x and out");
    XPS_CHECK_ARG((x == nullptr) == (out == nullptr), "x and out must both be given or both NULL");
    const uintptr_t bits = reinterpret_cast<uintptr_t>(mask) | reinterpret_cast<uintptr_t>(x) | reinterpret_cast<uintptr_t>(out);
    XPS_CHECK_ARG((bits & 7) == 0, "buffers must be 8-byte aligned");
    if (n == 0) return XPS_OK;
    if ((bits & 15) == 0 && n % 4 == 0)
        hipLaunchKernelGGL(dropout_kernel<true>, dim3(ew_grid(n / 4)), dim3(256), 0, (hipStream_t)stream, x, out, mask,
                           (long long)n, p, 1.0f / (1.0f - p), (unsigned long long)seed);
    else
        hipLaunchKernelGGL(dropout_kernel<false>, dim3(ew_grid((n + 1) / 2)), dim3(256), 0, (hipStream_t)stream, x, out, mask,
                           (long long)n, p, 1.0f / (1.0f - p), (unsigned long long)seed);
    XPS_CHECK_LAUNCH();
    return XPS_OK;
}

extern "C" int xps_split4_f32(const float* x, float* out, int64_t n, float drop_p, uint64_t seed, void* stream) {
    XPS_CHECK_ARG(x && out && n >= 0 && n % 4 == 0, "bad argument (n must be a multiple of 4)");
    XPS_CHECK_ARG(drop_p >= 0.f && drop_p < 1.f, "drop_p must be in [0, 1)");
    XPS_CHECK_ARG(((reinterpret_cast<uintptr_t>(x) | reinterpret_cast<uintptr_t>(out)) & 15) == 0, "buffers must be 16-byte aligned");
    if (n == 0) return XPS_OK;
    hipLaunchKernelGGL(split4_kernel, dim3(ew_grid(n / 4)), dim3(256), 0, (hipStream_t)stream, x, out, (long long)(n / 4), drop_p,
                       1.0f / (1.0f - drop_p), (unsigned long long)seed);
    XPS_CHECK_LAUNCH();
    return XPS_OK;
}

namespace {
__global__ __launch_bounds__(256) void split4_pad_kernel(const float* __restrict__ x, long long ldx, int rows, int cols, float* __restrict__ out,
                                                         long long ldo) {
    const long long g4 = ldo / 4, idx = (long long)blockIdx.x * 256 + threadIdx.x;
    if (idx >= (long long)rows * g4) return;
    const long long r = idx / g4;
    const int c = (int)(idx % g4) * 4;
    f32x4 v = {0.f, 0.f, 0.f, 0.f};
    if (c < cols) v = split4_pack(*reinterpret_cast<const f32x4*>(x + r * ldx + c));
    *reinterpret_cast<f32x4*>(out + r * ldo + c) = v;
}
}

extern "C" int xps_split4_pad_f32(const float* x, int64_t ldx, int rows, int cols, float* out, int64_t ldo, void* stream) {
    XPS_CHECK_ARG(x && out && rows >= 0 && cols >= 0 && cols % 4 == 0 && ldo % 4 == 0 && ldo >= cols && ldx % 4 == 0 && ldx >= cols, "bad argument");
    XPS_CHECK_ARG(((reinterpret_cast<uintptr_t>(x) | reinterpret_cast<uintptr_t>(out)) & 15) == 0, "buffers must be 16-byte aligned");
    if (rows == 0 || ldo == 0) return XPS_OK;
    hipLaunchKernelGGL(split4_pad_kernel, dim3(cdiv((long long)rows * (ldo / 4), 256)), dim3(256), 0, (hipStream_t)stream, x, (long long)ldx, rows,
                       cols, out, (long long)ldo);
    XPS_CHECK_LAUNCH();
    return XPS_OK;
}

extern "C" int xps_add_f32(const float* a, const float* b, float* out, int64_t n, void* stream) {
    XPS_CHECK_ARG(a && b && out && n >= 0, "bad argument");
    if (n == 0) return XPS_OK;
    hipLaunchKernelGGL(add_kernel, dim3(ew_grid(n)), dim3(256), 0, (hipStream_t)stream, a, b, out, (long long)n);
    XPS_CHECK_LAUNCH();
    return XPS_OK;
}

extern "C" int xps_cross_entropy_fwd_f32(const float* logits, const int64_t* target, float* row_loss, float* loss,
                                         int64_t rows, int n_classes, void* stream) {
    XPS_CHECK_ARG(logits && target && row_loss && loss && rows >= 1 && n_classes >= 1, "bad argument");
    if (rows <= CE_FUSED_ROWS) {
        hipLaunchKernelGGL(ce_fused_kernel, dim3(1), dim3(1024), 0, (hipStream_t)stream, logits, (const long long*)target,
                           row_loss, loss, (long long)rows, n_classes);
        XPS_CHECK_LAUNCH();
        return XPS_OK;
    }
    hipLaunchKernelGGL(ce_rows_kernel, dim3(cdiv(rows, 256)), dim3(256), 0, (hipStream_t)stream,
                       logits, (const long long*)target, row_loss, (long long)rows, n_classes);
    XPS_CHECK_LAUNCH();
    hipLaunchKernelGGL(ce_mean_kernel, dim3(1), dim3(1024), 0, (hipStream_t)stream, row_loss, (long long)rows, loss);
    XPS_CHECK_LAUNCH();
    return XPS_OK;
}

__global__ __launch_bounds__(CE_BLOCK) void ce_loss_grad_kernel(const float* __restrict__ logits, const long long* __restrict__ target,
                                                                float* __restrict__ row_loss, float* __restrict__ loss,
                                                                float* __restrict__ dlogits, double* part, unsigned* ticket,
                                                                long long rows, int C) {
    __shared__ double sh[CE_BLOCK];
    __shared__ unsigned last;
    const long long r = (long long)blockIdx.x * CE_BLOCK + threadIdx.x;
    double l = 0.0;
    if (r < rows) {
        const float rl = ce_row(logits + r * C, target[r], C, rows, dlogits ? dlogits + r * C : nullptr);
        row_loss[r] = rl;
        l = (double)rl;
    }
    if (ce_block_sum_ticket(l, sh, &last, part, ticket) && threadIdx.x == 0) {
        loss[0] = ce_mean_of_partials(part, rows);
        __hip_atomic_store(ticket, 0u, __ATOMIC_RELAXED, __HIP_MEMORY_SCOPE_AGENT);
    }
}

extern "C" size_t xps_cross_entropy_loss_grad_f32_workspace(int64_t rows) {
    return (size_t)(cdiv(rows > 0 ? rows : 1, 256) + 2) * sizeof(double);
}

extern "C" int xps_cross_entropy_loss_grad_f32(const float* logits, const int64_t* target, float* row_loss, float* loss,
                                               float* dlogits, void* workspace, size_t workspace_bytes, int64_t rows,
                                               int n_classes, void* stream) {
    XPS_CHECK_ARG(logits && target && row_loss && loss && rows >= 1 && n_classes >= 1, "bad argument");
    if (!workspace || workspace_bytes < xps_cross_entropy_loss_grad_f32_workspace(rows) || (reinterpret_cast<uintptr_t>(workspace) & 7)) {
        xps_set_error("xps_cross_entropy_loss_grad_f32: workspace too small or misaligned");
        return XPS_E_WORKSPACE;
    }
    const int blocks = cdiv(rows, CE_BLOCK);
    unsigned* ticket = (unsigned*)workspace;
    double* part = (double*)workspace + 2;
    hipLaunchKernelGGL(ce_loss_grad_kernel, dim3(blocks), dim3(CE_BLOCK), 0, (hipStream_t)stream, logits, (const long long*)target,
// ... 70 lines not shown
```

cross_patient_speech_decoding_amd/nn_models/functional.py:

```python
import ctypes as C
import os
from typing import NamedTuple

import torch

from .._dev import need_gpu as _need_gpu, ptr as _ptr, ptr_array as _ptr_array, stream as _stream, workspace as _ws
from .._lib import TnProblem, call, lib, rowmap

_f32 = torch.float32

GEMM_PRECISIONS = {'fp32': 0, 'bf16x3': 1}


def set_gemm_precision(name):
    if name not in GEMM_PRECISIONS:
        raise ValueError(f"gemm precision must be one of {sorted(GEMM_PRECISIONS)}")
    call('xps_set_gemm_precision', GEMM_PRECISIONS[name])


def get_gemm_precision():
    mode = lib().xps_get_gemm_precision()
    return {v: k for k, v in GEMM_PRECISIONS.items()}[mode]


# ... 237 lines not shown
def split4_wanted(T, B, H, ndir):
    return H > 256 and split4_supported(T, B, H, ndir)


def _launch_form(B, H):
    return (lib().xps_get_gru_cluster_mode() != 0, B, H)


def _check_form(was, B, H):
    now = _launch_form(B, H)
    if was is not None and was != now:
        raise RuntimeError(f'GRU backward: the saved gates were written with cluster path {"on" if was[0] else "off"} (B, H = {was[1:]}) '
                           f'but the backward runs with it {"on" if now[0] else "off"} (B, H = {now[1:]}): the launch form '
                           '(set_gru_cluster_mode / XPS_GRU_CLUSTER) must not change between a forward and its backward')


def _gru_forward(gi, w_hh, b_hh, h0, T, B, H, ndir, save, drop=None):
    dev = gi.device
    y_ext = torch.empty(T + 2, B, ndir * H, dtype=_f32, device=dev)
    saved = torch.empty(ndir, T, B, 4 * H, dtype=_f32, device=dev) if save else None
    if save:
        saved.launch_form = _launch_form(B, H)
    nbytes = _gru_ws_bytes('xps_gru_seq_fwd_f32_workspace', T, B, H, ndir)
    ws = _ws(nbytes, dev)
    if nbytes > 16:
        _gru_status_register(dev)
    if drop is not None:
        y_drop = torch.empty(T, B, ndir * H, dtype=_f32, device=dev)
        call('xps_gru_seq_fwd_drop_f32', _ptr(gi), _ptr_array(w_hh), _ptr_array(b_hh), _ptr(h0), _ptr(y_ext),
             _ptr(saved), T, B, H, ndir, _ptr(y_drop), float(drop[0]), int(drop[1]), _ptr(ws), nbytes, _stream())
        return y_ext, saved, y_drop
    call('xps_gru_seq_fwd_f32', _ptr(gi), _ptr_array(w_hh), _ptr_array(b_hh), _ptr(h0), _ptr(y_ext),
         _ptr(saved), T, B, H, ndir, _ptr(ws), nbytes, _stream())
    return y_ext, saved


def hprev_split_wanted(T, B, H, ndir, split4=None):
    return ((split4_wanted(T, B, H, ndir) if split4 is None else split4) and (ndir * H) % 4 == 0 and T * B >= 4096 and H % 256 == 0
            and os.environ.get('XPS_HPREV_SPLIT', '1') != '0' and os.environ.get('XPS_GEMM_DMA', '1') != '0')


def fwd_ysplit_wanted(T, B, H, ndir, hprev=None):
    return (os.environ.get('XPS_FWD_YSPLIT', '1') != '0' and (hprev_split_wanted(T, B, H, ndir) if hprev is None else hprev)
            and bool(lib().xps_gru_seq_fwd_image_exchange_supported(T, B, H, ndir)))


def fwd_images_wanted(T, B, H, ndir, hprev=None):
    return (os.environ.get('XPS_FWD_IMAGES', '0') == '1' and (hprev_split_wanted(T, B, H, ndir) if hprev is None else hprev)
            and bool(lib().xps_gru_seq_fwd_images_supported(T, B, H, ndir)))


def _gru_forward_images(gi, w_hh, b_hh, T, B, H, ndir, save, want_dropped, drop):
    dev = gi.device
    y_ext = torch.empty(T + 2, B, ndir * H, dtype=_f32, device=dev)
    y_split = torch.empty(T + 2, B, ndir * H, dtype=_f32, device=dev) if save else None
    yd_split = torch.empty(T, B, ndir * H, dtype=_f32, device=dev) if want_dropped else None
    saved = torch.empty(ndir, T, B, 4 * H, dtype=_f32, device=dev) if save else None
    if save:
        saved.launch_form = _launch_form(B, H)
    nbytes = _gru_ws_bytes('xps_gru_seq_fwd_f32_workspace', T, B, H, ndir)
    ws = _ws(nbytes, dev)
    _gru_status_register(dev)
    call('xps_gru_seq_fwd_images_f32', _ptr(gi), _ptr_array(w_hh), _ptr_array(b_hh), None, _ptr(y_ext), _ptr(saved), T, B, H, ndir,
         _ptr(y_split), _ptr(yd_split), float(drop[0]) if (drop and want_dropped) else 0.0, int(drop[1]) if (drop and want_dropped) else 0,
         _ptr(ws), nbytes, _stream())
    return y_ext, saved, y_split, yd_split


def gru_forward_training_form(gi, w_hh, b_hh, T, B, H, ndir):
    if fwd_ysplit_wanted(T, B, H, ndir):
        return _gru_forward_images(gi, w_hh, b_hh, T, B, H, ndir, True, False, None)[:2]
    return _gru_forward(gi, w_hh, b_hh, None, T, B, H, ndir, True)


def _gru_backward(dy, dhn, y_ext, saved, w_hh, T, B, H, ndir, need_dh0, drop=None, split4=False, form=None):
    dev = y_ext.device
    _check_form(form if form is not None else getattr(saved, 'launch_form', None), B, H)
    if dy is not None and not dy.is_contiguous():
        dy = dy.contiguous()
    if dhn is not None and not dhn.is_contiguous():
        dhn = dhn.contiguous()
    if dy is None and dhn is None:
        dhn = torch.zeros(ndir, B, H, dtype=_f32, device=dev)
    if len(w_hh) > 1:
        w_t = [torch.empty(H, 3 * H, dtype=_f32, device=dev) for _ in w_hh]
        call('xps_transpose_batched_f32', _ptr_array(w_hh), _ptr_array(w_t), len(w_hh), 3 * H, H, _stream())
    else:
        w_t = [transpose(w, 3 * H, H) for w in w_hh]
    dgi = torch.empty(ndir, T, B, 3 * H, dtype=_f32, device=dev)
    dghn = torch.empty(ndir, T, B, H, dtype=_f32, device=dev)
    dh0 = torch.empty(ndir, B, H, dtype=_f32, device=dev) if need_dh0 else None
    nbytes = _gru_ws_bytes('xps_gru_seq_bwd_f32_workspace', T, B, H, ndir)
    ws = _ws(nbytes, dev)
    _gru_status_register(dev)
    if split4:
        fused = drop is not None and dy is not None
        call('xps_gru_seq_bwd_split4_f32', _ptr(dy), _ptr(dhn), _ptr(y_ext), _ptr(saved), _ptr_array(w_hh), _ptr_array(w_t), _ptr(dgi),
             _ptr(dghn), _ptr(dh0), T, B, H, ndir, float(drop[0]) if fused else 0.0, int(drop[1]) if fused else 0, _ptr(ws), nbytes,
             _stream())
        return dgi, dghn, dh0
    if drop is not None and dy is not None:
        call('xps_gru_seq_bwd_drop_f32', _ptr(dy), _ptr(dhn), _ptr(y_ext), _ptr(saved), _ptr_array(w_hh), _ptr_array(w_t), _ptr(dgi),
             _ptr(dghn), _ptr(dh0), T, B, H, ndir, float(drop[0]), int(drop[1]), _ptr(ws), nbytes, _stream())
        return dgi, dghn, dh0
    call('xps_gru_seq_bwd_f32', _ptr(dy), _ptr(dhn), _ptr(y_ext), _ptr(saved), _ptr_array(w_hh), _ptr_array(w_t), _ptr(dgi),
         _ptr(dghn), _ptr(dh0), T, B, H, ndir, _ptr(ws), nbytes, _stream())
    return dgi, dghn, dh0


def _recurrent_grad_problems(dgi, dghn, y_ext, w_hh_params, b_hh_params, T, B, H, ndir, fmt=0, y_fmt=0):
    dev = y_ext.device
    ldy = ndir * H
    probs, rets = [], []
    for d in range(ndir):
        dw, db, acc_w, rw, rb = _grad_targets(w_hh_params[d], (3 * H, H), b_hh_params[d], (3 * H,), dev)
        first_slot = 0 if d == 0 else 2
        hprev = y_ext.view(-1)[first_slot * B * ldy + d * H:]
        probs.append(tn_problem(dgi[d], hprev, dw, 2 * H, H, T * B, ra=rowmap(3 * H, fmt=fmt), rb=rowmap(ldy, fmt=y_fmt), rc=rowmap(H),
                                colsum_out=db, accumulate=acc_w))
        probs.append(tn_problem(dghn[d], hprev, dw[2 * H:], H, H, T * B, ra=rowmap(H, fmt=fmt), rb=rowmap(ldy, fmt=y_fmt), rc=rowmap(H),
                                colsum_out=db[2 * H:], accumulate=acc_w))
        rets.append((rw, rb))
    return probs, rets


class GRURecurFn(torch.autograd.Function):

    @staticmethod
    def forward(ctx, gi, h0, ndir, *wb):
        _need_gpu(gi, h0, *wb)
        w_hh = [w.contiguous() for w in wb[:ndir]]
        b_hh = [b.contiguous() for b in wb[ndir:]]
        gi = gi.contiguous()
        _, T, B, H3 = gi.shape
        H = H3 // 3
        h0c = None if h0 is None else h0.contiguous()
        save = any(ctx.needs_input_grad)
        y_ext, saved = _gru_forward(gi, w_hh, b_hh, h0c, T, B, H, ndir, save)
        if save:
            ctx.save_for_backward(y_ext, saved, *w_hh)
            ctx.form = saved.launch_form
        ctx.params = wb
        ctx.dims = (T, B, H, ndir)
        ctx.has_h0 = h0 is not None
        return y_ext

    @staticmethod
    def backward(ctx, dy_ext):
        y_ext, saved, *w_hh = ctx.saved_tensors
        T, B, H, ndir = ctx.dims
        need_dh0 = ctx.has_h0 and ctx.needs_input_grad[1]
        dgi, dghn, dh0 = _gru_backward(dy_ext[1:T + 1], None, y_ext, saved, w_hh, T, B, H, ndir, need_dh0, form=ctx.form)
        if need_dh0:
            dh0[0] += dy_ext[0, :, :H]
            if ndir == 2:
                dh0[1] += dy_ext[T + 1, :, H:]
        probs, rets = _recurrent_grad_problems(dgi, dghn, y_ext, ctx.params[:ndir], ctx.params[ndir:], T, B, H, ndir)
        gemm_tn_grouped(probs, y_ext.device)
        return (dgi, dh0, None, *[r[0] for r in rets], *[r[1] for r in rets])


HN_NONE, HN_STACK, HN_SUM = 0, 1, 2


FMT_X_SPLIT4, FMT_Y_SPLIT4 = 1, 2


def split4_mode():
    return lib().xps_get_gemm_precision() == 1 and os.environ.get('XPS_SPLIT4', '1') != '0'


def layer_output_split4_ok(T, B, H, ndir, drop_p):
    return bool(drop_p and drop_p > 0.0 and split4_mode() and H > 256 and (ndir * H) % 4 == 0
                and not fused_dropout_supported(T, B, H, ndir))


def _presplit_weights_ok(rows, In, H3):
    return (split4_mode() and In % 4 == 0 and rows >= 4096 and In * H3 >= int(os.environ.get('XPS_SPLIT4_WEIGHTS_MIN', 1 << 19))
            and os.environ.get('XPS_SPLIT4_WEIGHTS', '1') != '0')


def skinny_dx_wanted(rows, In, K):
    return (os.environ.get('XPS_SKINNY_DX', '0') == '1' and split4_mode() and In % 4 == 0 and In < 256 and rows % 256 == 0
            and rows >= 96 * 256 and K % 32 == 0 and K >= 512 and os.environ.get('XPS_GEMM_DMA', '1') != '0')


def split4_pad(w, ldo):
    w = w.contiguous()
    out = torch.empty(w.shape[0], ldo, dtype=_f32, device=w.device)
    call('xps_split4_pad_f32', _ptr(w), w.shape[1], w.shape[0], w.shape[1], _ptr(out), ldo, _stream())
    return out


def split4(x, drop_p=0.0, seed=0):
    out = torch.empty_like(x)
    call('xps_split4_f32', _ptr(x), _ptr(out), x.numel(), float(drop_p), int(seed), _stream())
    return out


class GruPlan(NamedTuple):
    cluster_on: bool
    precision: int
    drop_fused: bool
    x_fmt: int
    w_fmt: int
    y_out_split: bool
    fwd_images: bool
    fwd_ysplit: bool
    want_dropped: bool
    bwd_split4: int
    y_fmt: int
    skinny_dx: bool


def gru_layer_plan(T, B, In, H, ndir, drop_p, fmt):
    has_drop = bool(drop_p and drop_p > 0.0)
    drop_fused = bool(has_drop and fused_dropout_supported(T, B, H, ndir))
    y_out_split = bool(fmt & FMT_Y_SPLIT4)
    if y_out_split and (not has_drop or drop_fused):
        raise ValueError('FMT_Y_SPLIT4: only with a separate dropout pass (see layer_output_split4_ok)')
    w_fmt = 1 if _presplit_weights_ok(T * B, In, 3 * H) else 0
    split4 = bool(split4_wanted(T, B, H, ndir))
    hprev = bool(hprev_split_wanted(T, B, H, ndir, split4))
    fwd_images = bool(fwd_images_wanted(T, B, H, ndir, hprev))
    return GruPlan(cluster_on=lib().xps_get_gru_cluster_mode() != 0, precision=lib().xps_get_gemm_precision(), drop_fused=drop_fused,
                   x_fmt=1 if (fmt & FMT_X_SPLIT4) else 0, w_fmt=w_fmt, y_out_split=y_out_split, fwd_images=fwd_images,
                   fwd_ysplit=bool(fwd_ysplit_wanted(T, B, H, ndir, hprev)), want_dropped=fwd_images and y_out_split,
                   bwd_split4=int(split4), y_fmt=int(hprev),
                   skinny_dx=bool(split4 and not w_fmt and skinny_dx_wanted(T * B, In, 3 * H)))


class GRULayerFmtFn(torch.autograd.Function):

    @staticmethod
    def forward(ctx, x, ndir, hn_mode, drop_p, fmt, *wb):
        ctx.set_materialize_grads(False)
        _need_gpu(x, *wb)
        x = x.contiguous()
        T, B, In = x.shape
        w_ih = [wb[4 * d + 0].contiguous() for d in range(ndir)]
        w_hh = [wb[4 * d + 1].contiguous() for d in range(ndir)]
        b_ih = [wb[4 * d + 2].contiguous() for d in range(ndir)]
        b_hh = [wb[4 * d + 3].contiguous() for d in range(ndir)]
        H = w_hh[0].shape[1]
        plan = ctx.plan = gru_layer_plan(T, B, In, H, ndir, drop_p, fmt)
        gi = torch.empty(ndir, T, B, 3 * H, dtype=_f32, device=x.device)
        if plan.w_fmt:
            w_ih = [split4(w) for w in w_ih]
        ra, rb, rc = rowmap(In, fmt=plan.x_fmt), rowmap(In, fmt=plan.w_fmt), rowmap(3 * H)
        call('xps_gemm_nt_multi_f32', _ptr(x), C.byref(ra), _ptr_array(w_ih), C.byref(rb), _ptr_array([gi[d] for d in range(ndir)]),
             C.byref(rc), _ptr_array(b_ih), ndir, T * B, 3 * H, In, _stream())
        save = any(ctx.needs_input_grad)
        drop = None
        y_drop = None
        if drop_p and drop_p > 0.0:
            drop = (float(drop_p), next_dropout_seed())
        ctx.drop = drop
        y_split = None
        if (save and (plan.fwd_images or plan.fwd_ysplit)) or plan.want_dropped:
            y_ext, saved, y_split, y_drop = _gru_forward_images(gi, w_hh, b_hh, T, B, H, ndir, save, plan.want_dropped, drop)
        elif plan.drop_fused:
            y_ext, saved, y_drop = _gru_forward(gi, w_hh, b_hh, None, T, B, H, ndir, save, drop)
        else:
            y_ext, saved = _gru_forward(gi, w_hh, b_hh, None, T, B, H, ndir, save)
        if save:
            ctx.save_for_backward(x, y_ext, saved, *w_ih, *w_hh, *([y_split] if y_split is not None else []))
        ctx.params = wb
        ctx.dims = (T, B, H, ndir, In, hn_mode)
        y = y_ext[1:T + 1]
        if y_drop is not None:
            y = y_drop
        elif drop is not None:
            out = torch.empty(T, B, ndir * H, dtype=_f32, device=x.device)
            if plan.y_out_split:
                call('xps_split4_f32', _ptr(y), _ptr(out), out.numel(), drop[0], drop[1], _stream())
            else:
                call('xps_dropout_f32', _ptr(y), _ptr(out), None, out.numel(), drop[0], drop[1], _stream())
            y = out
        if hn_mode == HN_NONE:
            hn = None
        elif hn_mode == HN_SUM:
            hn = y_ext[T, :, :H] + y_ext[1, :, H:] if ndir == 2 else y_ext[T, :, :H].clone()
        else:
            hn = torch.stack([y_ext[T, :, :H]] + ([y_ext[1, :, H:]] if ndir == 2 else []), dim=0)
        return y, hn

    @staticmethod
    def backward(ctx, dy, dhn):
        T, B, H, ndir, In, hn_mode = ctx.dims
        if dhn is not None and hn_mode == HN_SUM:
            dhn = dhn.unsqueeze(0).expand(ndir, B, H).contiguous()
        plan = ctx.plan
        if lib().xps_get_gemm_precision() != plan.precision:
            names = {v: k for k, v in GEMM_PRECISIONS.items()}
            raise RuntimeError(f'GRU backward: the forward chose its operand formats in {names[plan.precision]} mode but the backward '
                               f'runs in {names[lib().xps_get_gemm_precision()]} mode: the product precision (set_gemm_precision / '
                               'XPS_GEMM_PRECISION) must not change between a forward and its backward')
        x, y_ext, saved, *w = ctx.saved_tensors
        y_split = w.pop() if (plan.fwd_images or plan.fwd_ysplit) else None
        w_ih, w_hh = w[:ndir], w[ndir:]
        fmt, y_fmt, x_fmt, w_fmt = plan.bwd_split4, plan.y_fmt, plan.x_fmt, plan.w_fmt
        wb = ctx.params
        if ctx.drop is not None and dy is not None and not plan.drop_fused:
            dyc = dy.contiguous()
            dyd = torch.empty_like(dyc)
            call('xps_dropout_f32', _ptr(dyc), _ptr(dyd), None, dyc.numel(), ctx.drop[0], ctx.drop[1], _stream())
            dy = dyd
        dgi, dghn, _ = _gru_backward(dy, dhn, y_ext, saved, w_hh, T, B, H, ndir, False, ctx.drop if plan.drop_fused else None,
                                     split4=bool(fmt), form=(plan.cluster_on, B, H))
        dev = x.device
        have_img = y_split is not None
        y_src = (y_split if have_img else torch.empty_like(y_ext)) if y_fmt else y_ext
        probs, rets_hh = _recurrent_grad_problems(dgi, dghn, y_src, [wb[4 * d + 1] for d in range(ndir)],
                                                  [wb[4 * d + 3] for d in range(ndir)], T, B, H, ndir, fmt, y_fmt)
        rets_ih = []
        for d in range(ndir):
            dw, db, acc_w, rw, rb = _grad_targets(wb[4 * d + 0], (3 * H, In), wb[4 * d + 2], (3 * H,), dev)
            probs.append(tn_problem(dgi[d], x, dw, 3 * H, In, T * B, ra=rowmap(3 * H, fmt=fmt), rb=rowmap(In, fmt=x_fmt),
                                    colsum_out=db, accumulate=acc_w))
            rets_ih.append((rw, rb))
        direct = all(r[0] is None and r[1] is None for r in rets_ih + rets_hh)
        def launch_group(st):
            if y_fmt and not have_img:
                call('xps_split4_f32', _ptr(y_ext), _ptr(y_src), y_ext.numel(), 0.0, 0, _stream() if st is None else st)
            return gemm_tn_grouped(probs, dev, st)
        _launch_weight_grads(launch_group, dev, (dgi, dghn, x, y_ext, y_src), direct)
        dx = None
        if ctx.needs_input_grad[0]:
            dx = torch.empty(T, B, In, dtype=_f32, device=dev)
            if plan.skinny_dx:
                w_ih = [split4_pad(w, 256) for w in w_ih]
                w_fmt, ldw = 1, 256
            else:
                ldw = In
            if ndir == 2:
                ra, rb, rc = rowmap(3 * H, fmt=fmt), rowmap(ldw, fmt=w_fmt), rowmap(In)
                call('xps_gemm_nn2_f32', _ptr(dgi[0]), _ptr(w_ih[0]), 3 * H, _ptr(dgi[1]), _ptr(w_ih[1]), 3 * H,
                     C.byref(ra), C.byref(rb), _ptr(dx), C.byref(rc), T * B, In, 0, _stream())
            else:
                gemm_nn(dgi[0], w_ih[0], dx, T * B, In, 3 * H, ra=rowmap(3 * H, fmt=fmt), rb=rowmap(ldw, fmt=w_fmt))
        grads = []
        for d in range(ndir):
            grads += [rets_ih[d][0], rets_hh[d][0], rets_ih[d][1], rets_hh[d][1]]
        return (dx, None, None, None, None, *grads)


class GRULayerDropFn(torch.autograd.Function):

    @staticmethod
    def forward(ctx, x, ndir, hn_mode, drop_p, *wb):
        return GRULayerFmtFn.forward(ctx, x, ndir, hn_mode, drop_p, 0, *wb)

    @staticmethod
    def backward(ctx, dy, dhn):
        g = GRULayerFmtFn.backward(ctx, dy, dhn)
        return g[:4] + g[5:]


class GRULayerFn(torch.autograd.Function):

    @staticmethod
    def forward(ctx, x, ndir, hn_mode, *wb):
        return GRULayerDropFn.forward(ctx, x, ndir, hn_mode, 0.0, *wb)

    @staticmethod
    def backward(ctx, dy, dhn):
        g = GRULayerDropFn.backward(ctx, dy, dhn)
        return g[:3] + g[4:]


POST_SYNCBN_HOOKS = []
def _dp_world(group):
    import torch.distributed as dist
    if group is not None and dist.is_available() and dist.is_initialized():
        return dist.get_world_size(group)
    return 1


def _dp_enabled(group):
    return _dp_world(group) > 1


def _dist_sum_(t, group):
    if _dp_enabled(group):
        import torch.distributed as dist
        dist.all_reduce(t, op=dist.ReduceOp.SUM, group=group)
        return True
    return False


def _global_rows(rows, group, device, global_trials, Tp):
    if global_trials is not None:
        return float(global_trials) * Tp
    cnt = torch.tensor([float(rows)], dtype=torch.float64, device=device)
    _dist_sum_(cnt, group)
    return float(cnt.item())


class TemporalConvFn(torch.autograd.Function):

    @staticmethod
    def forward(ctx, x, conv_w, conv_b, gamma, beta, running_mean, running_var, stride, training,
                relu, drop_mask, drop_scale, momentum, eps, group, global_trials=None, num_batches_tracked=None):
        _need_gpu(x, conv_w)
        x = x.contiguous()
        B, T, Cin = x.shape
        F, _, k = conv_w.shape
        Tp = (T - k) // stride + 1
        if Tp < 1:
            raise ValueError('TemporalConv: sequence shorter than the kernel')
        w2 = conv_w.permute(0, 2, 1).contiguous().view(F, k * Cin)
        rows = Tp * B
        y = torch.empty(Tp, B, F, dtype=_f32, device=x.device)
        ra = rowmap(stride * Cin, rpg=Tp, gs=T * Cin)
        rc = rowmap(B * F, rpg=Tp, gs=F)
        gemm_nt(x, w2, y, rows, F, k * Cin, bias=conv_b, ra=ra, rc=rc)
        out = torch.empty_like(y)
        if training:
            stats = torch.empty(2 * F, dtype=_f32, device=x.device)
            nbytes = lib().xps_colsum_f32_workspace(rows, F)
            ws = _ws(nbytes, x.device)
            call('xps_colsum_f32', _ptr(y), F, rows, F, _ptr(stats), None, 0, _ptr(ws), nbytes, _stream())
            count = float(rows)
            if _dist_sum_(stats[:F], group):
                count = _global_rows(rows, group, x.device, global_trials, Tp)
            call('xps_bn_centered_sumsq_f32', _ptr(y), rows, F, _ptr(stats), count, _ptr(stats[F:]), _ptr(ws), nbytes,
                 _stream())
            _dist_sum_(stats[F:], group)
            mean = torch.empty(F, dtype=_f32, device=x.device)
            rstd = torch.empty(F, dtype=_f32, device=x.device)
            call('xps_bn_finalize_apply_f32', _ptr(y), _ptr(stats), count, _ptr(gamma), _ptr(beta), _ptr(mean), _ptr(rstd),
                 _ptr(running_mean), _ptr(running_var), _ptr(num_batches_tracked), momentum, eps, _ptr(drop_mask), drop_scale,
                 _ptr(out), rows, F, int(relu), _stream())
            ctx.save_for_backward(x, w2, y, out, mean, rstd, gamma, drop_mask)
            ctx.cfg = (B, T, Cin, F, k, stride, Tp, relu, drop_scale, count, group)
            ctx.conv_w = conv_w
            ctx.conv_b = conv_b
            ctx.bn_params = (gamma, beta)
        else:
            call('xps_bn_apply_eval_f32', _ptr(y), _ptr(running_mean), _ptr(running_var), eps, _ptr(gamma),
                 _ptr(beta), _ptr(out), rows, F, int(relu), _stream())
        return out

    @staticmethod
    def backward(ctx, dout):
        x, w2, y, out, mean, rstd, gamma, drop_mask = ctx.saved_tensors
        B, T, Cin, F, k, stride, Tp, relu, drop_scale, count, group = ctx.cfg
        rows = Tp * B
        dev = x.device
        dout = dout.contiguous()
        sums = torch.empty(2 * F, dtype=_f32, device=dev)
        nbytes = lib().xps_bn_bwd_workspace(rows, F)
        ws = _ws(nbytes, dev)
        g_beta, acc_beta, _ = _grad_target(ctx.bn_params[1], (F,), dev)
        g_gamma, acc_gamma, _ = _grad_target(ctx.bn_params[0], (F,), dev)
        direct_bn = acc_beta and acc_gamma
        dp = _dp_enabled(group)
        call('xps_bn_bwd_reduce_f32', _ptr(dout), _ptr(out), _ptr(y), _ptr(mean), _ptr(rstd), _ptr(drop_mask),
             drop_scale, int(relu), _ptr(sums), _ptr(g_beta) if direct_bn else None, _ptr(g_gamma) if direct_bn else None,
             rows, F, _ptr(ws), nbytes, _stream())
        dbeta = dgamma = None
        if not direct_bn:
            local = sums.clone() if dp else sums
            dbeta, dgamma = local[:F], local[F:]
        if dp:
            _dist_sum_(sums, group)
            for hook in list(POST_SYNCBN_HOOKS):
                hook()
        dy = torch.empty_like(y)
        call('xps_bn_bwd_apply_f32', _ptr(dout), _ptr(out), _ptr(y), _ptr(mean), _ptr(rstd), _ptr(gamma),
             _ptr(drop_mask), drop_scale, int(relu), _ptr(sums), count, _ptr(dy), rows, F, _stream())
        dconv_b, acc_cb, r_cb = _grad_target(ctx.conv_b, (F,), dev) if ctx.conv_b is not None else (None, False, None)
        if dconv_b is None:
            dconv_b = r_cb = torch.empty(F, dtype=_f32, device=dev)
        dw2 = torch.empty(F, k * Cin, dtype=_f32, device=dev)
        gemm_tn_grouped([tn_problem(dy, x, dw2, F, k * Cin, rows, ra=rowmap(F),
                                    rb=rowmap(T * Cin, rpg=B, gs=stride * Cin), colsum_out=dconv_b,
                                    accumulate_colsum=acc_cb)], dev)
        gw, acc_w, _ = _grad_target(ctx.conv_w, (F, Cin, k), dev)
        if acc_w:
            gw.add_(dw2.view(F, k, Cin).permute(0, 2, 1))
            dconv_w = None
        else:
            dconv_w = dw2.view(F, k, Cin).permute(0, 2, 1).contiguous()
        return (None, dconv_w, r_cb, dgamma, dbeta) + (None,) * 12


def decoder_supported(H, C, L):
    return bool(lib().xps_decoder_supported(int(H), int(C), int(L)))


class DecoderFn(torch.autograd.Function):

    @staticmethod
    def forward(ctx, table, h0, w_hh, b_hh, w_fc, b_fc, teacher, flags, start_token, L):
        ctx.set_materialize_grads(False)
        _need_gpu(table, h0, w_hh, w_fc)
        table, h0c = table.contiguous(), h0.contiguous()
        w_hh_c, b_hh_c, w_fc_c, b_fc_c = w_hh.contiguous(), b_hh.contiguous(), w_fc.contiguous(), b_fc.contiguous()
        B, H = h0c.shape
        C = w_fc_c.shape[0]
        ntok = table.shape[0]
        dev = h0c.device
        save = any(ctx.needs_input_grad)
        logits = torch.empty(B, L, C, dtype=_f32, device=dev)
        tokens = torch.empty(L, B, dtype=torch.int64, device=dev)
        hs = torch.empty(L + 1, B, H, dtype=_f32, device=dev)
        saved = torch.empty(L, B, 4 * H, dtype=_f32, device=dev) if save else None
        if teacher is not None:
            teacher = teacher.contiguous()
            if tuple(teacher.shape) != (B, L):
                raise ValueError('teacher tokens must be (batch, seq_length)')
        call('xps_decoder_fwd_f32', _ptr(table), _ptr(w_hh_c), _ptr(b_hh_c), _ptr(h0c), _ptr(w_fc_c), _ptr(b_fc_c),
             _ptr(teacher), _ptr(flags) if teacher is not None else None, _ptr(logits), _ptr(tokens), _ptr(hs),
             _ptr(saved), B, H, C, L, ntok, int(start_token), _stream())
        if save:
            ctx.save_for_backward(tokens, hs, saved, w_hh_c, w_fc_c)
        ctx.params = (w_hh, b_hh, w_fc, b_fc)
        ctx.dims = (B, H, C, L, ntok)
        ctx.mark_non_differentiable(tokens)
        return logits, tokens

    @staticmethod
    def backward(ctx, dlogits, _dtok):
        tokens, hs, saved, w_hh_c, w_fc_c = ctx.saved_tensors
        B, H, C, L, ntok = ctx.dims
        w_hh, b_hh, w_fc, b_fc = ctx.params
        dev = hs.device
        if dlogits is None:
            return (None,) * 10
        dlogits = dlogits.contiguous()
        w_t = transpose(w_hh_c, 3 * H, H)
        dgi = torch.empty(L, B, 3 * H, dtype=_f32, device=dev)
        dghn = torch.empty(L, B, H, dtype=_f32, device=dev)
        dh0 = torch.empty(B, H, dtype=_f32, device=dev)
        call('xps_decoder_bwd_f32', _ptr(dlogits), _ptr(hs), _ptr(saved), _ptr(w_t), _ptr(w_fc_c), _ptr(dgi), _ptr(dghn),
             _ptr(dh0), B, H, C, L, _stream())
        dtable, r_wh, r_bh, r_wf, r_bf = _decoder_weight_grads(dlogits, dgi, dghn, hs, tokens, ctx.params, B, H, C, L, ntok)
        return dtable, dh0, r_wh, r_bh, r_wf, r_bf, None, None, None, None


def _decoder_weight_grads(dlogits, dgi, dghn, hs, tokens, params, B, H, C, L, ntok):
    w_hh, b_hh, w_fc, b_fc = params
    dev = hs.device
    dwh, acc_h, r_wh = _grad_target(w_hh, (3 * H, H), dev)
    dbh, acc_bh, r_bh = _grad_target(b_hh, (3 * H,), dev)
    dwf, acc_f, r_wf = _grad_target(w_fc, (C, H), dev)
    dbf, acc_bf, r_bf = _grad_target(b_fc, (C,), dev)
    if not (acc_h == acc_bh and acc_f == acc_bf):
        dwh, dbh = torch.empty(3 * H, H, dtype=_f32, device=dev), torch.empty(3 * H, dtype=_f32, device=dev)
        dwf, dbf = torch.empty(C, H, dtype=_f32, device=dev), torch.empty(C, dtype=_f32, device=dev)
        acc_h = acc_f = False
        r_wh, r_bh, r_wf, r_bf = dwh, dbh, dwf, dbf
    hprev = hs
    hnext = hs.view(-1)[B * H:]
    probs = [
        tn_problem(dgi, hprev, dwh, 2 * H, H, L * B, ra=rowmap(3 * H), rb=rowmap(H), rc=rowmap(H),
                   colsum_out=dbh, accumulate=acc_h),
        tn_problem(dghn, hprev, dwh[2 * H:], H, H, L * B, ra=rowmap(H), rb=rowmap(H), rc=rowmap(H),
                   colsum_out=dbh[2 * H:], accumulate=acc_h),
        tn_problem(dlogits, hnext, dwf, C, H, L * B, ra=rowmap(L * C, rpg=B, gs=C), rb=rowmap(H), rc=rowmap(H),
                   colsum_out=dbf, accumulate=acc_f),
    ]
    _launch_weight_grads(lambda st: gemm_tn_grouped(probs, dev, st), dev, (dgi, dghn, hs, dlogits),
                         r_wh is None and r_bh is None and r_wf is None and r_bf is None)
    dtable = torch.empty(ntok, 3 * H, dtype=_f32, device=dev)
    nbytes = lib().xps_scatter_rows_f32_workspace(L * B, 3 * H, ntok)
    ws = _ws(nbytes, dev)
    call('xps_scatter_rows_f32', _ptr(dgi), _ptr(tokens), _ptr(dtable), L * B, 3 * H, ntok, 0, _ptr(ws), nbytes,
         _stream())
    return dtable, r_wh, r_bh, r_wf, r_bf


class DecoderWideFn(torch.autograd.Function):

    @staticmethod
    def forward(ctx, table, h0, w_hh, b_hh, w_fc, b_fc, teacher, flags, start_token, L):
        ctx.set_materialize_grads(False)
        _need_gpu(table, h0, w_hh, w_fc)
        table, h0c = table.contiguous(), h0.contiguous()
        w_hh_c, b_hh_c, w_fc_c, b_fc_c = w_hh.contiguous(), b_hh.contiguous(), w_fc.contiguous(), b_fc.contiguous()
        B, H = h0c.shape
        C = w_fc_c.shape[0]
        ntok = table.shape[0]
        dev = h0c.device
        save = any(ctx.needs_input_grad)
        if teacher is not None:
            teacher = teacher.contiguous()
            if tuple(teacher.shape) != (B, L):
                raise ValueError('teacher tokens must be (batch, seq_length)')
        steps = torch.empty(L, B, C, dtype=_f32, device=dev)
        tokens = torch.empty(L, B, dtype=torch.int64, device=dev)
        tokens[0].fill_(int(start_token))
        hs = torch.empty(L + 2, B, H, dtype=_f32, device=dev)
        saved = torch.empty(1, L, B, 4 * H, dtype=_f32, device=dev) if save else None
        ctx.form = _launch_form(B, H)
        gi = torch.empty(B, 3 * H, dtype=_f32, device=dev)
        nbytes = _gru_ws_bytes('xps_gru_seq_fwd_f32_workspace', 1, B, H, 1)
        _gru_status_register(dev)
        w_arr, b_arr = _ptr_array([w_hh_c]), _ptr_array([b_hh_c])
        rc = rowmap(C)
        fused_select = C <= 16
        for s in range(L):
            if s == 0 or not fused_select:
                call('xps_gather_rows_f32', _ptr(table), _ptr(tokens[s]), _ptr(gi), B, 3 * H, ntok, _stream())
            ws = _ws(nbytes, dev)
            call('xps_gru_seq_fwd_f32', _ptr(gi), w_arr, b_arr, _ptr(h0c if s == 0 else hs[s]), _ptr(hs[s:]),
                 _ptr(saved[0, s]) if save else None, 1, B, H, 1, _ptr(ws), nbytes, _stream())
            tstride = teacher.stride(0) if teacher is not None else 0
            if fused_select:
                last = s + 1 == L
                call('xps_decoder_select_f32', _ptr(hs[s + 1]), _ptr(w_fc_c), _ptr(b_fc_c), _ptr(steps[s]),
                     _ptr(teacher[:, s]) if (teacher is not None and not last) else None, tstride,
                     _ptr(flags[s:s + 1]) if (teacher is not None and not last) else None, _ptr(table),
                     None if last else _ptr(tokens[s + 1]), None if last else _ptr(gi), B, H, C, ntok, _stream())
                continue
            gemm_nt(hs[s + 1], w_fc_c, steps[s], B, C, H, bias=b_fc_c, rc=rc)
            if s + 1 < L:
                call('xps_next_token', _ptr(steps[s]), C, _ptr(teacher[:, s]) if teacher is not None else None, tstride,
                     _ptr(flags[s:s + 1]) if teacher is not None else None, _ptr(tokens[s + 1]), B, _stream())
        logits = steps.permute(1, 0, 2).contiguous()
        if save:
            ctx.save_for_backward(tokens, hs, saved, w_hh_c, w_fc_c)
        ctx.params = (w_hh, b_hh, w_fc, b_fc)
        ctx.dims = (B, H, C, L, ntok)
        ctx.mark_non_differentiable(tokens)
        return logits, tokens

    @staticmethod
    def backward(ctx, dlogits, _dtok):
        tokens, hs, saved, w_hh_c, w_fc_c = ctx.saved_tensors
        B, H, C, L, ntok = ctx.dims
        dev = hs.device
        if dlogits is None:
            return (None,) * 10
        dlogits = dlogits.contiguous()
        dy = torch.empty(L, B, H, dtype=_f32, device=dev)
        gemm_nn(dlogits, w_fc_c, dy, L * B, H, C, ra=rowmap(L * C, rpg=B, gs=C))
        dgi, dghn, dh0 = _gru_backward(dy, None, hs, saved, [w_hh_c], L, B, H, 1, True, form=ctx.form)
        dtable, r_wh, r_bh, r_wf, r_bf = _decoder_weight_grads(dlogits, dgi[0], dghn[0], hs, tokens, ctx.params, B, H, C, L, ntok)
        return dtable, dh0[0], r_wh, r_bh, r_wf, r_bf, None, None, None, None


class GatherRowsFn(torch.autograd.Function):

    @staticmethod
    def forward(ctx, table, idx):
        _need_gpu(table, idx)
        table = table.contiguous()
        idx = idx.contiguous()
        n_rows, cols = table.shape
        out = torch.empty(idx.shape[0], cols, dtype=_f32, device=table.device)
        call('xps_gather_rows_f32', _ptr(table), _ptr(idx), _ptr(out), idx.shape[0], cols, n_rows, _stream())
        ctx.save_for_backward(idx)
        ctx.shape = (n_rows, cols)
        return out

    @staticmethod
    def backward(ctx, dout):
        (idx,) = ctx.saved_tensors
        n_rows, cols = ctx.shape
        dout = dout.contiguous()
        dt = torch.empty(n_rows, cols, dtype=_f32, device=dout.device)
        nbytes = lib().xps_scatter_rows_f32_workspace(idx.shape[0], cols, n_rows)
        ws = _ws(nbytes, dout.device)
        call('xps_scatter_rows_f32', _ptr(dout), _ptr(idx), _ptr(dt), idx.shape[0], cols, n_rows, 0, _ptr(ws), nbytes,
             _stream())
        return dt, None


def gather_rows(table, idx):
    return GatherRowsFn.apply(table, idx)


def next_token(logits, teacher, use_teacher):
    B, Cn = logits.shape
    nxt = torch.empty(B, dtype=torch.int64, device=logits.device)
    tstride = teacher.stride(0) if teacher is not None else 0
    call('xps_next_token', _ptr(logits.contiguous()), Cn, _ptr(teacher), tstride, _ptr(use_teacher), _ptr(nxt),
         B, _stream())
    return nxt


class MaskScaleFn(torch.autograd.Function):
    @staticmethod
    def forward(ctx, x, mask, scale):
        x = x.contiguous()
        out = torch.empty_like(x)
        call('xps_mask_scale_f32', _ptr(x), _ptr(mask), scale, _ptr(out), x.numel(), _stream())
        ctx.save_for_backward(mask)
        ctx.scale = scale
        return out

    @staticmethod
    def backward(ctx, dout):
        (mask,) = ctx.saved_tensors
        dout = dout.contiguous()
        dx = torch.empty_like(dout)
        call('xps_mask_scale_f32', _ptr(dout), _ptr(mask), ctx.scale, _ptr(dx), dout.numel(), _stream())
        return dx, None, None


_DROP_COUNTER = [0]

# ... 443 lines not shown
```

cross_patient_speech_decoding_amd/nn_models/models.py:

```python
import os

import torch
import torch.nn as nn

from . import functional as XF
from ._lightning import LightningModule


def cmat_acc(y_hat, y, num_classes):
    y_pred = torch.argmax(y_hat, dim=1)
    cm = torch.bincount(y * num_classes + y_pred, minlength=num_classes * num_classes)
    cm = cm.view(num_classes, num_classes)
    return cm.diag().sum() / cm.sum()


class _HipCrossEntropyLoss(nn.CrossEntropyLoss):

    def forward(self, input, target):
        plain = (self.weight is None and self.reduction == 'mean' and self.ignore_index == -100
                 and self.label_smoothing == 0.0 and input.dim() == 2 and input.is_cuda)
        if plain:
            return XF.cross_entropy(input, target)
        return super().forward(input, target)


class BaseLightningModel(LightningModule):

    def __init__(self, criterion=None, learning_rate=1e-3, l2_reg=1e-5):
        super().__init__()
        self.criterion = criterion if criterion is not None else _HipCrossEntropyLoss()
        self.learning_rate = learning_rate
        self.l2_reg = l2_reg

    def _shared_step(self, batch, stage):
        x, y = batch
        y_hat = self(x)
        loss = self.criterion(y_hat, y)
        acc = cmat_acc(y_hat, y, self.num_classes)
        self.log_dict({f'{stage}_loss': loss, f'{stage}_acc': acc}, prog_bar=True)
        return loss

    def training_step(self, batch, batch_idx):
        return self._shared_step(batch, 'train')

    def validation_step(self, batch, batch_idx):
        return self._shared_step(batch, 'val')

    def test_step(self, batch, batch_idx):
        return self._shared_step(batch, 'test')

    def predict_step(self, batch, batch_idx):
        x, _ = batch
        return self(x)

    def configure_optimizers(self):
        return torch.optim.AdamW(self.parameters(), lr=self.learning_rate, weight_decay=self.l2_reg)


class TemporalConv(nn.Module):

    def __init__(self, in_channels, out_channels, kernel_size, stride=1, padding=0, dropout=0.2,
                 activation=True):
        super().__init__()
        self.conv = nn.Conv1d(in_channels, out_channels, kernel_size, stride=stride, padding=padding)
        self.bn = nn.BatchNorm1d(out_channels)
        self.relu = nn.ReLU()
        self.dropout = nn.Dropout(dropout)
        self.activation = activation
        self.process_group = None
        self.global_batch = None

    def forward_tm(self, x):
        k, s, pad = self.conv.kernel_size[0], self.conv.stride[0], self.conv.padding[0]
        if pad > 0:
            x = torch.nn.functional.pad(x, (0, 0, pad, pad))
        B, T, _ = x.shape
        Tp = (T - k) // s + 1
        F = self.conv.out_channels
        training = self.training
        mask, scale, p = None, 1.0, self.dropout.p
        if training and p > 0:
            mask = XF.dropout_mask((Tp, B, F), p, x.device)
            scale = 1.0 / (1.0 - p)
        momentum = 0.1 if self.bn.momentum is None else self.bn.momentum
        nbt = self.bn.num_batches_tracked if training and self.bn.track_running_stats else None
        return XF.TemporalConvFn.apply(x, self.conv.weight, self.conv.bias, self.bn.weight, self.bn.bias,
                                       self.bn.running_mean, self.bn.running_var, s, training,
                                       bool(self.activation), mask, scale, momentum, self.bn.eps,
                                       self.process_group, self.global_batch if self.process_group is not None else None,
                                       nbt)

    def forward(self, x):
        return self.forward_tm(x.permute(0, 2, 1)).permute(1, 2, 0)


def _gru_layer_weights(rnn, layer, ndir):
    out = []
    for d in range(ndir):
        sfx = f'_l{layer}' + ('_reverse' if d == 1 else '')
        out += [getattr(rnn, 'weight_ih' + sfx), getattr(rnn, 'weight_hh' + sfx),
                getattr(rnn, 'bias_ih' + sfx), getattr(rnn, 'bias_hh' + sfx)]
    return out


class EncoderRNN(nn.Module):

    def __init__(self, input_size, hidden_size, num_layers, dropout=0.3, model_type='gru'):
        super().__init__()
        self.model_type = model_type
        if model_type == 'gru':
            self.rnn = nn.GRU(input_size, hidden_size, num_layers, batch_first=True, dropout=dropout,
                              bidirectional=True)
        elif model_type == 'lstm':
            raise NotImplementedError("model_type='lstm' is not on the accelerated path (the reference's LSTM "
                                      'branch is itself broken: models.py:280 repeats a tuple)')
        else:
            raise ValueError('model_type must be one of "gru" or "lstm"')

    def forward_tm(self, x):
        y, last = self.forward_tm_last(x)
        return y, last.unsqueeze(0)

    def forward_tm_last(self, x):
        rnn = self.rnn
        L = rnn.num_layers
        y = x
        fmt = 0
        for l in range(L):
            p_drop = float(rnn.dropout) if (l < L - 1 and self.training) else 0.0
            T_, B_ = y.shape[0], y.shape[1]
            out_split = XF.layer_output_split4_ok(T_, B_, rnn.hidden_size, 2, p_drop)
            y, last = XF.GRULayerFmtFn.apply(y, 2, XF.HN_SUM if l == L - 1 else XF.HN_NONE, p_drop,
                                             fmt | (XF.FMT_Y_SPLIT4 if out_split else 0), *_gru_layer_weights(rnn, l, 2))
            fmt = XF.FMT_X_SPLIT4 if out_split else 0
        return y, last

    def forward(self, x):
        y, h = self.forward_tm(x.permute(1, 0, 2))
        return y.permute(1, 0, 2), h


class DecoderRNN(nn.Module):

    def __init__(self, hidden_size, output_size, num_layers, dropout=0.3, model_type='gru'):
        super().__init__()
        self.embedding = nn.Embedding(output_size + 1, hidden_size)
        if model_type != 'gru':
            raise NotImplementedError("model_type='lstm' is not on the accelerated path")
        self.rnn = nn.GRU(hidden_size, hidden_size, num_layers, batch_first=True, dropout=dropout)
        self.fc_out = nn.Linear(hidden_size, output_size)

    def token_projection(self):
        return XF.linear(self.embedding.weight, self.rnn.weight_ih_l0, self.rnn.bias_ih_l0)

    def step(self, tok, hidden, table):
        rnn = self.rnn
        B = tok.shape[0]
        H = rnn.hidden_size
        new_h = []
        gi = XF.gather_rows(table, tok).view(1, 1, B, 3 * H)
        y_ext = XF.GRURecurFn.apply(gi, hidden[0:1], 1, rnn.weight_hh_l0, rnn.bias_hh_l0)
        h = y_ext[1]
        new_h.append(h)
        for l in range(1, rnn.num_layers):
            inp = XF.dropout(h, rnn.dropout, self.training)
            gi = XF.linear(inp, getattr(rnn, f'weight_ih_l{l}'), getattr(rnn, f'bias_ih_l{l}')).view(1, 1, B, 3 * H)
            y_ext = XF.GRURecurFn.apply(gi, hidden[l:l + 1], 1, getattr(rnn, f'weight_hh_l{l}'),
                                        getattr(rnn, f'bias_hh_l{l}'))
            h = y_ext[1]
            new_h.append(h)
        logits = XF.linear(h, self.fc_out.weight, self.fc_out.bias)
        return logits, torch.stack(new_h, dim=0)

# ... 325 lines not shown
```

include/xps.h:

```cpp
#ifndef XPS_H
#define XPS_H

#include <stddef.h>
#include <stdint.h>

#ifdef __cplusplus
extern "C" {
#endif

#define XPS_OK 0
#define XPS_E_INVALID (-1)
#define XPS_E_HIP (-2)
#define XPS_E_WORKSPACE (-3)

typedef struct xps_rowmap {
    int64_t gs;
    int64_t ld;
    int32_t rpg;
    int32_t fmt;
} xps_rowmap;
#define XPS_FMT_F32 0
#define XPS_FMT_SPLIT4 1

const char* xps_last_error(void);
int xps_abi_version(void);
int xps_stream_create_low_priority(void** stream);
int xps_stream_destroy(void* stream);
int xps_set_gemm_precision(int mode);
int xps_get_gemm_precision(void);
int xps_set_gemm_big_tiles(int on);
int xps_get_gemm_big_tiles(void);


int xps_gemm_nt_f32(const float* A, const xps_rowmap* ra, const float* B, const xps_rowmap* rb,
                    float* C, const xps_rowmap* rc, const float* bias,
                    int M, int N, int K, int accumulate, void* stream);
int xps_gemm_nn_f32(const float* A, const xps_rowmap* ra, const float* B, const xps_rowmap* rb,
                    float* C, const xps_rowmap* rc,
                    int M, int N, int K, int accumulate, void* stream);
int xps_gemm_nt_multi_f32(const float* A, const xps_rowmap* ra, const float* const* B, const xps_rowmap* rb,
                          float* const* C, const xps_rowmap* rc, const float* const* bias, int nprob,
                          int M, int N, int K, void* stream);
int xps_gemm_nn2_f32(const float* A1, const float* B1, int K1, const float* A2, const float* B2, int K2,
                     const xps_rowmap* ra, const xps_rowmap* rb, float* C, const xps_rowmap* rc,
                     int M, int N, int accumulate, void* stream);
size_t xps_gemm_tn_f32_workspace(int M, int N, int K);
int xps_gemm_tn_f32(const float* A, const xps_rowmap* ra, const float* B, const xps_rowmap* rb,
                    float* C, const xps_rowmap* rc,
                    int M, int N, int K, int accumulate,
                    void* workspace, size_t workspace_bytes, void* stream);

typedef struct xps_tn_problem {
    const float* A; const float* B; float* C; float* colsum_a;
    xps_rowmap ra, rb, rc;
    int32_t M, N, K, accumulate;
} xps_tn_problem;
size_t xps_gemm_tn_grouped_f32_workspace(const xps_tn_problem* probs, int n);
int xps_gemm_tn_grouped_f32(const xps_tn_problem* probs, int n, void* workspace, size_t workspace_bytes,
                            void* stream);

size_t xps_colsum_f32_workspace(int rows, int cols);
int xps_colsum_f32(const float* X, int64_t ldx, int rows, int cols, float* out, float* out_sq,
                   int accumulate, void* workspace, size_t workspace_bytes, void* stream);

size_t xps_gru_seq_fwd_f32_workspace(int T, int B, int H, int ndir);
long long xps_gru_seq_status_offset(int T, int B, int H, int ndir);
int xps_gru_set_status_word(unsigned* device_word);
int xps_set_gru_bptt_grid(int two_dimensional);
int xps_get_gru_bptt_grid(void);
int xps_set_gru_cluster_mode(int mode);
int xps_get_gru_cluster_mode(void);
int xps_gru_seq_fwd_f32(const float* gi, const float* const* w_hh, const float* const* b_hh,
                        const float* h0, float* y_ext, float* saved,
                        int T, int B, int H, int ndir, void* workspace, size_t workspace_bytes, void* stream);

size_t xps_gru_seq_bwd_f32_workspace(int T, int B, int H, int ndir);
int xps_gru_seq_bwd_f32(const float* dy, const float* dhn, const float* y_ext, const float* saved,
                        const float* const* w_hh, const float* const* w_hh_t, float* dgi, float* dghn, float* dh0,
                        int T, int B, int H, int ndir, void* workspace, size_t workspace_bytes, void* stream);
int xps_gru_seq_fused_dropout_supported(int T, int B, int H, int ndir);
int xps_gru_seq_fwd_drop_f32(const float* gi, const float* const* w_hh, const float* const* b_hh,
                             const float* h0, float* y_ext, float* saved,
                             int T, int B, int H, int ndir, float* y_drop, float drop_p, uint64_t drop_seed,
                             void* workspace, size_t workspace_bytes, void* stream);
int xps_gru_seq_bwd_drop_f32(const float* dy, const float* dhn, const float* y_ext, const float* saved,
                             const float* const* w_hh, const float* const* w_hh_t, float* dgi, float* dghn, float* dh0,
                             int T, int B, int H, int ndir, float drop_p, uint64_t drop_seed,
                             void* workspace, size_t workspace_bytes, void* stream);
int xps_gru_seq_fwd_images_supported(int T, int B, int H, int ndir);
int xps_gru_seq_fwd_image_exchange_supported(int T, int B, int H, int ndir);
int xps_gru_seq_fwd_images_f32(const float* gi, const float* const* w_hh, const float* const* b_hh,
                               const float* h0, float* y_ext, float* saved, int T, int B, int H, int ndir,
                               float* y_split, float* y_drop_split, float drop_p, uint64_t drop_seed,
                               void* workspace, size_t workspace_bytes, void* stream);
int xps_gru_seq_bwd_split4_supported(int T, int B, int H, int ndir);
int xps_gru_seq_bwd_split4_f32(const float* dy, const float* dhn, const float* y_ext, const float* saved,
                               const float* const* w_hh, const float* const* w_hh_t, float* dgi, float* dghn, float* dh0,
                               int T, int B, int H, int ndir, float drop_p, uint64_t drop_seed,
                               void* workspace, size_t workspace_bytes, void* stream);

int xps_transpose_f32(const float* src, float* dst, int rows, int cols, void* stream);
int xps_transpose_batched_f32(const float* const* src, float* const* dst, int n, int rows, int cols, void* stream);

int xps_bn_centered_sumsq_f32(const float* y, int rows, int F, const float* stats, double count, float* out_sq,
                              void* workspace, size_t workspace_bytes, void* stream);
int xps_bn_finalize_f32(const float* stats, double count, float* mean, float* rstd,
                        float* running_mean, float* running_var, int64_t* num_batches_tracked,
                        float momentum, float eps, int F, void* stream);
int xps_bn_apply_f32(const float* y, const float* mean, const float* rstd,
                     const float* gamma, const float* beta, const float* drop_mask, float drop_scale,
                     float* out, int64_t rows, int F, int relu, void* stream);
int xps_bn_finalize_apply_f32(const float* y, const float* stats, double count, const float* gamma, const float* beta,
                              float* mean, float* rstd, float* running_mean, float* running_var,
                              int64_t* num_batches_tracked, float momentum, float eps, const float* drop_mask,
                              float drop_scale, float* out, int64_t rows, int F, int relu, void* stream);
int xps_bn_apply_eval_f32(const float* y, const float* running_mean, const float* running_var, float eps,
                          const float* gamma, const float* beta, float* out,
                          int64_t rows, int F, int relu, void* stream);
size_t xps_bn_bwd_workspace(int64_t rows, int F);
int xps_bn_bwd_reduce_f32(const float* dout, const float* out, const float* y, const float* mean,
                          const float* rstd, const float* drop_mask, float drop_scale, int relu,
                          float* sums, float* dbeta_acc, float* dgamma_acc, int64_t rows, int F,
                          void* workspace, size_t workspace_bytes, void* stream);
int xps_bn_bwd_apply_f32(const float* dout, const float* out, const float* y, const float* mean,
                         const float* rstd, const float* gamma, const float* drop_mask,
                         float drop_scale, int relu, const float* sums, double count,
                         float* dy, int64_t rows, int F, void* stream);

int xps_decoder_supported(int H, int C, int L);
int xps_decoder_fwd_f32(const float* table, const float* w_hh, const float* b_hh, const float* h0,
                        const float* w_fc, const float* b_fc, const int64_t* teacher, const int32_t* flags,
                        float* logits, int64_t* tokens, float* hs, float* saved,
                        int B, int H, int C, int L, int ntok, int start_token, void* stream);
int xps_decoder_bwd_f32(const float* dlogits, const float* hs, const float* saved, const float* w_hh_t,
                        const float* w_fc, float* dgi, float* dghn, float* dh0,
                        int B, int H, int C, int L, void* stream);

int xps_gemv_f32(const float* x, const float* W, const float* bias, float* out, int N, int K, int B,
                 void* stream);
int xps_gru_cell_gemv_f32(const float* x, int K, const float* w_ih, const float* w_hh, const float* b_ih,
                          const float* b_hh, const float* h_prev, float* h_new, int H, int B, void* stream);

int xps_window_shift_f32(const double* power, int k, int C, const double* W, const double* c, const float* src,
                         float* dst, int win, int d, int B, void* stream);
int xps_ctc_collapse_f32(const float* logits, int n_classes, int blank, int64_t* argmax, int32_t* state,
                         int64_t* tokens, int max_tokens, int B, void* stream);

size_t xps_ctc_beam_workspace(int B, int T, int beam_size, int n_classes);
int xps_ctc_beam_f64(const void* log_probs, int is_f32, int B, int T, int n_classes, const int64_t* input_lengths,
                     int blank, int beam_size, int from_logits, int64_t* prefix, int64_t* prefix_len, double* nll,
                     void* workspace, size_t workspace_bytes, void* stream);
size_t xps_ctc_beam_state_bytes(int n_streams, int beam_size, int max_steps);
int xps_ctc_beam_step_f32(const float* logits, int n_classes, int blank, int beam_size, int max_steps, void* state,
                          size_t state_bytes, int B, void* stream);
int xps_ctc_beam_readout(const void* state, size_t state_bytes, int B, int beam_size, int max_steps, int s,
                         int64_t* prefix, int64_t* prefix_len, double* nll, void* stream);

int xps_gather_rows_f32(const float* table, const int64_t* idx, float* out,
                        int B, int cols, int n_rows, void* stream);
size_t xps_scatter_rows_f32_workspace(int B, int cols, int n_rows);
int xps_scatter_rows_f32(const float* dout, const int64_t* idx, float* dtable,
                         int B, int cols, int n_rows, int accumulate,
                         void* workspace, size_t workspace_bytes, void* stream);
int xps_next_token(const float* logits, int n_classes, const int64_t* teacher, int64_t teacher_stride,
                   const int32_t* use_teacher, int64_t* next, int B, void* stream);
int xps_decoder_select_f32(const float* h, const float* w_fc, const float* b_fc, float* logits,
                           const int64_t* teacher, int64_t teacher_stride, const int32_t* use_teacher,
                           const float* table, int64_t* next, float* gi_next, int B, int H, int C, int ntok, void* stream);
int xps_dropout_f32(const float* x, float* out, float* mask, int64_t n, float p, uint64_t seed, void* stream);
int xps_split4_f32(const float* x, float* out, int64_t n, float drop_p, uint64_t seed, void* stream);
int xps_split4_pad_f32(const float* x, int64_t ldx, int rows, int cols, float* out, int64_t ldo, void* stream);
int xps_mask_scale_f32(const float* x, const float* mask, float scale, float* out, int64_t n, void* stream);
int xps_add_f32(const float* a, const float* b, float* out, int64_t n, void* stream);

int xps_cross_entropy_fwd_f32(const float* logits, const int64_t* target, float* row_loss,
                              float* loss, int64_t rows, int n_classes, void* stream);
int xps_cross_entropy_bwd_f32(const float* logits, const int64_t* target, const float* gout,
                              float* dlogits, int64_t rows, int n_classes, void* stream);
size_t xps_cross_entropy_loss_grad_f32_workspace(int64_t rows);
int xps_cross_entropy_loss_grad_f32(const float* logits, const int64_t* target, float* row_loss, float* loss,
                                    float* dlogits, void* workspace, size_t workspace_bytes, int64_t rows,
                                    int n_classes, void* stream);
size_t xps_classify_loss_acc_f32_workspace(int64_t rows);
int xps_classify_loss_acc_f32(const float* logits, const int64_t* target, float* row_loss, float* loss, float* dlogits,
                              int64_t* cmat, float* acc, void* workspace, size_t workspace_bytes, int64_t rows,
                              int n_classes, void* stream);
int xps_time_max_fwd_f32(const float* z, float* out, int* arg, int T, int B, int F, void* stream);
int xps_time_max_bwd_f32(const float* dout, const int* arg, float* dz, int T, int B, int F, void* stream);

int xps_attention_supported(int B, int S, int n_head, int dh);
int xps_attention_fwd_f32(const float* qkv, float* ctx, float* lse, int B, int S, int n_head, int dh, float p, uint64_t seed,
                          void* stream);
size_t xps_attention_bwd_f32_workspace(int B, int S, int n_head, int dh);
int xps_attention_bwd_f32(const float* dctx, const float* qkv, const float* ctx, const float* lse, float* dqkv, int B, int S,
                          int n_head, int dh, float p, uint64_t seed, void* workspace, size_t workspace_bytes, void* stream);
int xps_add_layer_norm_fwd_f32(const float* x, const float* r, const float* gamma, const float* beta, float* y, float* mean,
                               float* rstd, int64_t rows, int D, float eps, float p, uint64_t seed, void* stream);
size_t xps_add_layer_norm_bwd_f32_workspace(int64_t rows, int D);
int xps_add_layer_norm_bwd_f32(const float* dy, const float* x, const float* r, const float* gamma, const float* mean,
                               const float* rstd, float* dx, float* dr, float* dgamma, float* dbeta, int64_t rows, int D, float p,
                               uint64_t seed, void* workspace, size_t workspace_bytes, void* stream);
int xps_relu_dropout_fwd_f32(const float* x, float* out, int64_t n, float p, uint64_t seed, void* stream);
int xps_relu_dropout_bwd_f32(const float* dout, const float* out, float* dx, int64_t n, float p, void* stream);
int xps_add_positional_f32(const float* z, const float* table, float* out, int S, int B, int D, int batch_major, void* stream);
int xps_time_mean_fwd_f32(const float* z, float* out, int T, int B, int F, void* stream);
int xps_time_mean_bwd_f32(const float* dout, float* dz, int T, int B, int F, void* stream);
size_t xps_ctc_loss_f32_workspace(int T, int B, int max_target_len);
int xps_ctc_loss_f32(const float* logits, const int64_t* targets, int64_t target_stride,
                     const int64_t* input_lengths, const int64_t* target_lengths, int T, int B, int C,
                     int max_target_len, int blank, int zero_infinity, float* nll, float* loss,
                     float* dlogits, void* workspace, size_t workspace_bytes, void* stream);
size_t xps_sumsq_f32_workspace(int64_t n);
int xps_sumsq_f32(const float* g, int64_t n, float* sumsq, void* workspace, size_t workspace_bytes,
                  void* stream);
int xps_adamw_f32(float* p, float* g, float* m, float* v, int64_t n, const float* sumsq, float max_norm,
                  float lr, float beta1, float beta2, float eps, float weight_decay, int step,
                  void* stream);
int xps_clip_adamw_f32(float* p, float* g, float* m, float* v, int64_t n, float* sumsq, float max_norm, float lr,
                       float beta1, float beta2, float eps, float weight_decay, int step, void* workspace,
                       size_t workspace_bytes, void* stream);

int xps_cnd_avg_f32(const float* data, const int32_t* order, const int32_t* start, double* out,
                    int n_cond, int64_t row_len, void* stream);
int xps_cnd_avg_f64(const double* data, const int32_t* order, const int32_t* start, double* out,
                    int n_cond, int64_t row_len, void* stream);
size_t xps_colsum_f64_workspace(int64_t n, int d);
int xps_colsum_f64(const void* X, int is_f32, int64_t ldx, int64_t n, int d, double* out,
                   void* workspace, size_t workspace_bytes, void* stream);
size_t xps_xcov_f64_workspace(int64_t n, int da, int db);
int xps_xcov_f64(const void* A, int a_is_f32, int64_t lda, const double* mean_a,
                 const void* B, int b_is_f32, int64_t ldb, const double* mean_b,
                 double* C, int64_t ldc, int64_t n, int da, int db,
                 void* workspace, size_t workspace_bytes, void* stream);
size_t xps_jacobi_f64_workspace(int n);
int xps_jacobi_sweeps_f64(double* W, int64_t ldw, double* V, int64_t ldv, int m, int n, int sweeps,
                          double* off, void* workspace, size_t workspace_bytes, void* stream);
int xps_chol_whiten_supported(int n);
int xps_chol_whiten_f64(const double* R, int64_t ldr, int64_t stride_r, double scale, double shift, double* A, int64_t lda,
                        int64_t stride_a, double* S, int64_t lds, int64_t stride_s, int n, int batch, int32_t* info,
                        void* stream);
int xps_jacobi_small_supported(int m, int n, int want_v);
int xps_jacobi_small_f64(double* W, int64_t ldw, int64_t stride_w, double* V, int64_t ldv, int64_t stride_v,
                         int m, int n, int batch, int max_sweeps, double tol, int32_t* sweeps_done, double* off,
                         void* stream);
size_t xps_process_hg_f64_workspace(int C, int Tn, int bands);
int xps_process_hg_f64(const double* data, int C, int Tn, const uint8_t* good, const double* b, const double* a,
                       int bands, int taps, double* zi, int do_car, double* car_out, double* filtered,
                       double* power, void* workspace, size_t workspace_bytes, void* stream);
size_t xps_pipe_frontend_f64_workspace(int n_streams, int C, int Tn, int bands);
int xps_pipe_frontend_f64(const double* bins, int n_streams, int k, int C, int Tn, const uint8_t* good, const double* b,
                          const double* a, int bands, int taps, double* zi, double* power, void* workspace,
                          size_t workspace_bytes, void* stream);
size_t xps_hg_trials_f64_workspace(int64_t N, int n_bins, int C, int Tn, int bands);
// ... 64 lines not shown
```

Before: 313,100 trials/s.

## Fold cluster init and setup work into neighbouring decoder and GRU kernels

Folds the GRU cluster init (header zeroing, state staging) into the decoder select and start kernels, so each decoder step no longer needs a separate init launch. It also merges the backward transpose of w_hh with header zeroing into one setup kernel, adds a batched split4, a conv prologue that generates the dropout mask, and writes logits straight into the final layout instead of permuting. The aim is fewer small kernel launches across the 20 decoder steps and the backward pass. In exchange the code carries more entry points with 'ready' flags that assume their setup kernels ran first.

New measurement: 317,000 trials/s, median of 5. +1.2%, better.

```diff
diff --git a/cross_patient_speech_decoding_amd/csrc/xps_decoder_glue.h b/cross_patient_speech_decoding_amd/csrc/xps_decoder_glue.h
--- /dev/null
+++ b/cross_patient_speech_decoding_amd/csrc/xps_decoder_glue.h
@@ -0,0 +1,60 @@
+#pragma once
+#include "xps_common.h"
+
+constexpr int SEL_MAXC = 16;
+
+__device__ __forceinline__ void decoder_select_row(const float* __restrict__ h, const float* __restrict__ w_fc,
+                                                   const float* __restrict__ b_fc, float* __restrict__ logits, long long ldl,
+                                                   const long long* __restrict__ teacher, long long tstride,
+                                                   const int* __restrict__ use_teacher, const float* __restrict__ table,
+                                                   long long* __restrict__ next, float* __restrict__ gi_next,
+                                                   int b, int lane, int H, int C, int ntok) {
+    float acc[SEL_MAXC];
+#pragma unroll
+    for (int c = 0; c < SEL_MAXC; ++c) acc[c] = 0.f;
+    const float* hr = h + (long long)b * H;
+    for (int k = lane * 4; k < H; k += 256) {
+        const f32x4 hv = *reinterpret_cast<const f32x4*>(hr + k);
+#pragma unroll
+        for (int c = 0; c < SEL_MAXC; ++c) {
+            if (c < C) {
+                const f32x4 wv = *reinterpret_cast<const f32x4*>(w_fc + (long long)c * H + k);
+                acc[c] += (hv[0] * wv[0] + hv[1] * wv[1]) + (hv[2] * wv[2] + hv[3] * wv[3]);
+            }
+        }
+    }
+#pragma unroll
+    for (int c = 0; c < SEL_MAXC; ++c) {
+        if (c < C) {
+#pragma unroll
+            for (int o = 32; o > 0; o >>= 1) acc[c] += __shfl_xor(acc[c], o);
+        }
+    }
+    float best = 0.f;
+    int bi = 0;
+#pragma unroll
+    for (int c = 0; c < SEL_MAXC; ++c) {
+        if (c < C) {
+            const float v = acc[c] + b_fc[c];
+            if (lane == c) logits[(long long)b * ldl + c] = v;
+            if (c == 0 || v > best) { best = v; bi = c; }
+        }
+    }
+    if (!next) return;
+    long long tok = bi;
+    if (use_teacher && teacher && use_teacher[0]) tok = teacher[(long long)b * tstride];
+    if (lane == 0) next[b] = tok;
+    if (gi_next && tok >= 0 && tok < ntok) {
+        const float* src = table + tok * 3LL * H;
+        float* dst = gi_next + (long long)b * 3 * H;
+        for (int k = lane * 4; k < 3 * H; k += 256) *reinterpret_cast<f32x4*>(dst + k) = *reinterpret_cast<const f32x4*>(src + k);
+    }
+}
+
+__device__ __forceinline__ void decoder_start_rows(const float* __restrict__ table, long long start, long long* __restrict__ tokens,
+                                                   float* __restrict__ gi, int B, int cols, int n_rows, long long tid, long long nthreads) {
+    const long long r = start < 0 ? 0 : (start >= n_rows ? n_rows - 1 : start);
+    const long long total = (long long)B * cols;
+    for (long long i = tid; i < total; i += nthreads) gi[i] = table[r * cols + (int)(i % cols)];
+    for (long long b = tid; b < B; b += nthreads) tokens[b] = start;
+}
diff --git a/cross_patient_speech_decoding_amd/csrc/xps_gru.hip b/cross_patient_speech_decoding_amd/csrc/xps_gru.hip
--- a/cross_patient_speech_decoding_amd/csrc/xps_gru.hip
+++ b/cross_patient_speech_decoding_amd/csrc/xps_gru.hip
@@ -11,11 +11,13 @@
 size_t xps_internal_gru_cluster_status_offset(int B, int H, int ndir);
 int xps_internal_gru_cluster_fwd(const float* gi, const float* const* w_hh, const float* const* b_hh, const float* h0,
                                  float* y_ext, float* saved, int T, int B, int H, int ndir, void* workspace, hipStream_t st,
-                                 float* y_split, float* yd_split, float drop_p, unsigned long long drop_seed);
+                                 float* y_split, float* yd_split, float drop_p, unsigned long long drop_seed, int ready = 0);
 int xps_internal_gru_cluster_bwd(const float* dy, const float* dhn, const float* y_ext, const float* saved,
                                  const float* const* w_hh_t, float* dgi, float* dghn, float* dh0,
-                                 int T, int B, int H, int ndir, void* workspace, hipStream_t st, int split_out);
+                                 int T, int B, int H, int ndir, void* workspace, hipStream_t st, int split_out, int header_ready = 0);
 bool xps_internal_gru_cluster_ximg_ok(int B, int H, int ndir);
+size_t xps_internal_gru_cluster_bwd_header(int B, int H, int ndir);
+bool xps_internal_gru_cluster_fold_ok(int B, int H);
 
 namespace {
 
@@ -1123,6 +1125,26 @@
     }
 }
 
+typedef unsigned gru_u32x4 __attribute__((ext_vector_type(4)));
+__global__ void gru_bwd_setup_kernel(TransposeBatch tb, int rows, int cols, gru_u32x4* __restrict__ header, int header_u4) {
+    __shared__ float tile[32][33];
+    const long long nthreads = (long long)gridDim.x * gridDim.y * gridDim.z * 256;
+    const long long tid = (((long long)blockIdx.z * gridDim.y + blockIdx.y) * gridDim.x + blockIdx.x) * 256 + threadIdx.y * 32 + threadIdx.x;
+    for (long long i = tid; i < header_u4; i += nthreads) header[i] = (gru_u32x4){0u, 0u, 0u, 0u};
+    const float* __restrict__ src = tb.src[blockIdx.z];
+    float* __restrict__ dst = tb.dst[blockIdx.z];
+    const int bx = blockIdx.x * 32, by = blockIdx.y * 32;
+    for (int i = threadIdx.y; i < 32; i += blockDim.y) {
+        int r = by + i, c = bx + threadIdx.x;
+        tile[i][threadIdx.x] = (r < rows && c < cols) ? src[(long long)r * cols + c] : 0.f;
+    }
+    __syncthreads();
+    for (int i = threadIdx.y; i < 32; i += blockDim.y) {
+        int c = bx + i, r = by + threadIdx.x;
+        if (c < cols && r < rows) dst[(long long)c * rows + r] = tile[threadIdx.x][i];
+    }
+}
+
 inline bool aligned16(const void* p) { return (reinterpret_cast<uintptr_t>(p) & 15) == 0; }
 
 inline bool use_step_path() {
@@ -1155,7 +1177,7 @@
 static int gru_seq_fwd_impl(const float* gi, const float* const* w_hh, const float* const* b_hh,
                             const float* h0, float* y_ext, float* saved,
                             int T, int B, int H, int ndir, float* y_drop, float drop_p, unsigned long long drop_seed,
-                            void* workspace, size_t workspace_bytes, void* stream);
+                            void* workspace, size_t workspace_bytes, void* stream, int ready = 0);
 
 extern "C" int xps_gru_seq_fwd_f32(const float* gi, const float* const* w_hh, const float* const* b_hh,
                                    const float* h0, float* y_ext, float* saved,
@@ -1204,7 +1226,7 @@
 static int gru_seq_fwd_impl(const float* gi, const float* const* w_hh, const float* const* b_hh,
                             const float* h0, float* y_ext, float* saved,
                             int T, int B, int H, int ndir, float* y_drop, float drop_p, unsigned long long drop_seed,
-                            void* workspace, size_t workspace_bytes, void* stream) {
+                            void* workspace, size_t workspace_bytes, void* stream, int ready) {
     XPS_CHECK_ARG(gi && w_hh && b_hh && y_ext, "null argument");
     XPS_CHECK_ARG(T >= 1 && B >= 1 && H >= 1, "T, B, H must be >= 1");
     XPS_CHECK_ARG(ndir == 1 || ndir == 2, "ndir must be 1 or 2");
@@ -1215,7 +1237,7 @@
             return XPS_E_WORKSPACE;
         }
         return xps_internal_gru_cluster_fwd(gi, w_hh, b_hh, h0, y_ext, saved, T, B, H, ndir, workspace, (hipStream_t)stream,
-                                            nullptr, nullptr, 0.f, 0ull);
+                                            nullptr, nullptr, 0.f, 0ull, ready);
     }
     GruFwdParams p;
     p.gi = gi; p.h0 = h0; p.y_ext = y_ext; p.saved = saved;
@@ -1284,7 +1306,7 @@
 static int gru_seq_bwd_impl(const float* dy, const float* dhn, const float* y_ext, const float* saved,
                             const float* const* w_hh, const float* const* w_hh_t, float* dgi, float* dghn, float* dh0,
                             int T, int B, int H, int ndir, int has_drop, float drop_p, unsigned long long drop_seed,
-                            void* workspace, size_t workspace_bytes, void* stream, int split_out = 0);
+                            void* workspace, size_t workspace_bytes, void* stream, int split_out = 0, int header_ready = 0);
 
 extern "C" int xps_gru_seq_bwd_f32(const float* dy, const float* dhn, const float* y_ext, const float* saved,
                                    const float* const* w_hh, const float* const* w_hh_t, float* dgi, float* dghn, float* dh0,
@@ -1323,7 +1345,7 @@
 static int gru_seq_bwd_impl(const float* dy, const float* dhn, const float* y_ext, const float* saved,
                             const float* const* w_hh, const float* const* w_hh_t, float* dgi, float* dghn, float* dh0,
                             int T, int B, int H, int ndir, int has_drop, float drop_p, unsigned long long drop_seed,
-                            void* workspace, size_t workspace_bytes, void* stream, int split_out) {
+                            void* workspace, size_t workspace_bytes, void* stream, int split_out, int header_ready) {
     XPS_CHECK_ARG(y_ext && saved && w_hh && w_hh_t && dgi && dghn, "null argument");
     XPS_CHECK_ARG(!split_out || xps_gru_seq_bwd_split4_supported(T, B, H, ndir),
                   "XPS_FMT_SPLIT4 outputs: shape / precision mode not served (see xps_gru_seq_bwd_split4_supported)");
@@ -1336,7 +1358,8 @@
             xps_set_error("xps_gru_seq_bwd_f32: workspace too small");
             return XPS_E_WORKSPACE;
         }
-        return xps_internal_gru_cluster_bwd(dy, dhn, y_ext, saved, w_hh_t, dgi, dghn, dh0, T, B, H, ndir, workspace, (hipStream_t)stream, split_out);
+        return xps_internal_gru_cluster_bwd(dy, dhn, y_ext, saved, w_hh_t, dgi, dghn, dh0, T, B, H, ndir, workspace, (hipStream_t)stream, split_out,
+                                            header_ready);
     }
     GruBwdParams p;
     p.dy = dy; p.dhn = dhn; p.y_ext = y_ext; p.saved = saved; p.dgi = dgi; p.dghn = dghn; p.dh0 = dh0;
@@ -1444,3 +1467,51 @@
     XPS_CHECK_LAUNCH();
     return XPS_OK;
 }
+
+
+extern "C" int xps_gru_seq_fwd_setup_folds(int B, int H) {
+    if (B < 1 || H < 1) return 0;
+    return (cluster_shape_ok(1, B, H, 1) && xps_internal_gru_cluster_fold_ok(B, H)) ? 1 : 0;
+}
+
+extern "C" int xps_gru_seq_fwd_ready_f32(const float* gi, const float* const* w_hh, const float* const* b_hh,
+                                         const float* h0, float* y_ext, float* saved,
+                                         int T, int B, int H, int ndir, void* workspace, size_t workspace_bytes, void* stream) {
+    XPS_CHECK_ARG(T == 1 && ndir == 1 && xps_gru_seq_fwd_setup_folds(B, H), "one step, one direction, a shape xps_gru_seq_fwd_setup_folds accepts");
+    return gru_seq_fwd_impl(gi, w_hh, b_hh, h0, y_ext, saved, T, B, H, ndir, nullptr, 0.f, 0ull, workspace, workspace_bytes, stream, 1);
+}
+
+extern "C" int xps_gru_seq_bwd_setup_f32(const float* const* w_hh, float* const* w_hh_t, int T, int B, int H, int ndir,
+                                         void* workspace, size_t workspace_bytes, void* stream) {
+    XPS_CHECK_ARG(w_hh && w_hh_t && T >= 1 && B >= 1 && H >= 1 && (ndir == 1 || ndir == 2), "bad argument");
+    TransposeBatch tb;
+    for (int i = 0; i < 4; ++i) {
+        const int j = i < ndir ? i : 0;
+        XPS_CHECK_ARG(w_hh[j] && w_hh_t[j], "null matrix pointer");
+        tb.src[i] = w_hh[j]; tb.dst[i] = w_hh_t[j];
+    }
+    size_t header = 0;
+    if (cluster_shape_ok(T, B, H, ndir)) {
+        header = xps_internal_gru_cluster_bwd_header(B, H, ndir);
+        if (!workspace || workspace_bytes < xps_gru_seq_bwd_f32_workspace(T, B, H, ndir) || workspace_bytes < header || !aligned16(workspace)) {
+            xps_set_error("xps_gru_seq_bwd_setup_f32: workspace too small or misaligned");
+            return XPS_E_WORKSPACE;
+        }
+    }
+    const int rows = 3 * H, cols = H;
+    hipLaunchKernelGGL(gru_bwd_setup_kernel, dim3(cdiv(cols, 32), cdiv(rows, 32), ndir), dim3(32, 8), 0, (hipStream_t)stream,
+                       tb, rows, cols, (gru_u32x4*)workspace, (int)(header / 16));
+    XPS_CHECK_LAUNCH();
+    return XPS_OK;
+}
+
+extern "C" int xps_gru_seq_bwd_ready_f32(const float* dy, const float* dhn, const float* y_ext, const float* saved,
+                                         const float* const* w_hh, const float* const* w_hh_t, float* dgi, float* dghn, float* dh0,
+                                         int T, int B, int H, int ndir, float drop_p, uint64_t drop_seed, int split_out,
+                                         void* workspace, size_t workspace_bytes, void* stream) {
+    XPS_CHECK_ARG(drop_p >= 0.f && drop_p < 1.f && (split_out == 0 || split_out == 1), "0 <= p < 1, split_out 0 or 1");
+    XPS_CHECK_ARG(drop_p == 0.f || (dy && xps_gru_seq_fused_dropout_supported(T, B, H, ndir)),
+                  "fused dropout: dy must be given and the shape must be on the resident kernels");
+    return gru_seq_bwd_impl(dy, dhn, y_ext, saved, w_hh, w_hh_t, dgi, dghn, dh0, T, B, H, ndir, drop_p > 0.f ? 1 : 0, drop_p,
+                            (unsigned long long)drop_seed, workspace, workspace_bytes, stream, split_out, 1);
+}
diff --git a/cross_patient_speech_decoding_amd/csrc/xps_gru_cluster.hip b/cross_patient_speech_decoding_amd/csrc/xps_gru_cluster.hip
--- a/cross_patient_speech_decoding_amd/csrc/xps_gru_cluster.hip
+++ b/cross_patient_speech_decoding_amd/csrc/xps_gru_cluster.hip
@@ -4,6 +4,7 @@
 #include "xps_common.h"
 #include <atomic>
 #include "xps_gemm_tile.h"
+#include "xps_decoder_glue.h"
 using xps_tile::bf16x4;
 using xps_tile::bf16x8;
 using xps_tile::bf_split;
@@ -575,12 +576,12 @@
 }
 
 template <bool BF>
-__global__ void gru_cluster_init_kernel(const float* __restrict__ h0, float* __restrict__ y_ext, void* __restrict__ xbuf,
-                                        int T, int B, int H, int ndir, int Bp, int KP, u32x4* __restrict__ header, int header_u4,
-                                        float* __restrict__ y_split) {
-    for (int i = blockIdx.x * blockDim.x + threadIdx.x; i < header_u4; i += gridDim.x * blockDim.x) header[i] = (u32x4){0u, 0u, 0u, 0u};
+__device__ __forceinline__ void cl_init_rows(const float* __restrict__ h0, float* __restrict__ y_ext, void* __restrict__ xbuf,
+                                             int T, int B, int H, int ndir, int Bp, int KP, u32x4* __restrict__ header, int header_u4,
+                                             float* __restrict__ y_split, long long tid, long long nthreads) {
+    for (long long i = tid; i < header_u4; i += nthreads) header[i] = (u32x4){0u, 0u, 0u, 0u};
     const long long total = (long long)ndir * Bp * (KP / 4);
-    for (long long i = (long long)blockIdx.x * blockDim.x + threadIdx.x; i < total; i += (long long)gridDim.x * blockDim.x) {
+    for (long long i = tid; i < total; i += nthreads) {
         const int k = (int)(i % (KP / 4)) * 4;
         const long long rb = i / (KP / 4);
         const int b = (int)(rb % Bp), dir = (int)(rb / Bp);
@@ -615,6 +616,45 @@
             *reinterpret_cast<f32x4*>(row + k * 4) = v;
         }
     }
+}
+
+template <bool BF>
+__global__ void gru_cluster_init_kernel(const float* __restrict__ h0, float* __restrict__ y_ext, void* __restrict__ xbuf,
+                                        int T, int B, int H, int ndir, int Bp, int KP, u32x4* __restrict__ header, int header_u4,
+                                        float* __restrict__ y_split) {
+    cl_init_rows<BF>(h0, y_ext, xbuf, T, B, H, ndir, Bp, KP, header, header_u4, y_split,
+                     (long long)blockIdx.x * blockDim.x + threadIdx.x, (long long)gridDim.x * blockDim.x);
+}
+
+struct ClInitArgs {
+    float* y_ext;
+    void* xbuf;
+    u32x4* header;
+    int header_u4, B, H, Bp, KP;
+};
+
+template <bool BF>
+__global__ __launch_bounds__(256) void decoder_select_init_kernel(const float* __restrict__ h, const float* __restrict__ w_fc,
+                                                                  const float* __restrict__ b_fc, float* __restrict__ logits, long long ldl,
+                                                                  const long long* __restrict__ teacher, long long tstride,
+                                                                  const int* __restrict__ use_teacher, const float* __restrict__ table,
+                                                                  long long* __restrict__ next, float* __restrict__ gi_next,
+                                                                  int B, int H, int C, int ntok, ClInitArgs ci) {
+    cl_init_rows<BF>(h, ci.y_ext, ci.xbuf, 1, ci.B, ci.H, 1, ci.Bp, ci.KP, ci.header, ci.header_u4, nullptr,
+                     (long long)blockIdx.x * blockDim.x + threadIdx.x, (long long)gridDim.x * blockDim.x);
+    const int lane = threadIdx.x & 63;
+    const int b = blockIdx.x * 4 + (threadIdx.x >> 6);
+    if (b >= B) return;
+    decoder_select_row(h, w_fc, b_fc, logits, ldl, teacher, tstride, use_teacher, table, next, gi_next, b, lane, H, C, ntok);
+}
+
+template <bool BF>
+__global__ void decoder_start_init_kernel(const float* __restrict__ table, long long start, long long* __restrict__ tokens,
+                                          float* __restrict__ gi, int B, int cols, int n_rows, const float* __restrict__ h0,
+                                          ClInitArgs ci) {
+    const long long tid = (long long)blockIdx.x * blockDim.x + threadIdx.x, nthreads = (long long)gridDim.x * blockDim.x;
+    cl_init_rows<BF>(h0, ci.y_ext, ci.xbuf, 1, ci.B, ci.H, 1, ci.Bp, ci.KP, ci.header, ci.header_u4, nullptr, tid, nthreads);
+    decoder_start_rows(table, start, tokens, gi, B, cols, n_rows, tid, nthreads);
 }
 
 struct ClBwd {
@@ -1780,9 +1820,10 @@
 
 int xps_internal_gru_cluster_fwd(const float* gi, const float* const* w_hh, const float* const* b_hh, const float* h0,
                                  float* y_ext, float* saved, int T, int B, int H, int ndir, void* workspace, hipStream_t st,
-                                 float* y_split, float* yd_split, float drop_p, unsigned long long drop_seed) {
+                                 float* y_split, float* yd_split, float drop_p, unsigned long long drop_seed, int ready) {
     const ClPlan pl = cl_plan(B, H, ndir);
     if (!pl.ok) { xps_set_error("gru cluster forward: unsupported shape"); return XPS_E_INVALID; }
+    if (ready && (pl.CS * pl.U < pl.KP || y_split || yd_split)) { xps_set_error("gru cluster forward: this shape has no folded set-up"); return XPS_E_INVALID; }
     const bool bf = xps_internal_gemm_mode() == 1;
     if ((y_split || yd_split) && (!bf || H % 4 != 0 || !cl_aligned16(y_split) || !cl_aligned16(yd_split))) {
         xps_set_error("gru cluster forward: XPS_FMT_SPLIT4 images exist in bf16x3 mode only (H a multiple of 4, 16-byte aligned)");
@@ -1809,7 +1850,7 @@
     if (pl.CS * pl.U < pl.KP) {
         if (hipMemsetAsync(p.xbuf, 0, pl.xbuf_fwd, st) != hipSuccess) { xps_set_error("gru cluster forward: memset failed"); return XPS_E_HIP; }
     }
-    {
+    if (!ready) {
         const long long total = (long long)ndir * pl.Bp * (pl.KP / 4);
         const int blocks = (int)((total + 255) / 256 > 2048 ? 2048 : (total + 255) / 256);
         if (bf) hipLaunchKernelGGL(gru_cluster_init_kernel<true>, dim3(blocks), dim3(256), 0, st, h0, y_ext, ximg ? (void*)nullptr : p.xbuf, T, B, H, ndir, pl.Bp, pl.KP, (u32x4*)ws, (int)(pl.flags_bytes / 16), y_split);
@@ -1841,7 +1882,7 @@
 
 int xps_internal_gru_cluster_bwd(const float* dy, const float* dhn, const float* y_ext, const float* saved,
                                  const float* const* w_hh_t, float* dgi, float* dghn, float* dh0,
-                                 int T, int B, int H, int ndir, void* workspace, hipStream_t st, int split_out) {
+                                 int T, int B, int H, int ndir, void* workspace, hipStream_t st, int split_out, int header_ready) {
     const ClPlan pl = cl_plan(B, H, ndir);
     if (!pl.ok) { xps_set_error("gru cluster backward: unsupported shape"); return XPS_E_INVALID; }
     const bool bf = xps_internal_gemm_mode() == 1;
@@ -1869,7 +1910,7 @@
         q.pbuf_bytes = (unsigned)p2.pbuf;
         q.T = T; q.B = B; q.H = H; q.ndir = ndir; q.Bp = p2.Bp; q.Mc = p2.Mc; q.NR = p2.NR; q.nblk = p2.nblk;
         q.saved_mm = (H % 32 == 0) ? 1 : 0;
-        if (hipMemsetAsync(ws, 0, p2.flags_bytes, st) != hipSuccess) { xps_set_error("gru cluster backward: memset failed"); return XPS_E_HIP; }
+        if (!header_ready && hipMemsetAsync(ws, 0, p2.flags_bytes, st) != hipSuccess) { xps_set_error("gru cluster backward: memset failed"); return XPS_E_HIP; }
         const int ps_total = T + (dh0 ? 1 : 0);
         q.ps_total = ps_total;
         if (!cl_set_lds(gru_cluster2_bwd_kernel, C2_LDS)) { xps_set_error("gru cluster backward: cannot raise the dynamic LDS limit"); return XPS_E_HIP; }
@@ -1912,7 +1953,7 @@
     p.T = T; p.B = B; p.H = H; p.ndir = ndir; p.Bp = pl.Bp; p.Mc = pl.Mc; p.NR = pl.NR; p.nblk = pl.nblk; p.CS = pl.CS;
     p.saved_mm = (H % 32 == 0) ? 1 : 0;
     const bool xout = bf && split_out && H == pl.KP && pl.Bp == B && cl_xout_enabled();
-    if (hipMemsetAsync(ws, 0, pl.flags_bytes, st) != hipSuccess) { xps_set_error("gru cluster backward: memset failed"); return XPS_E_HIP; }
+    if (!header_ready && hipMemsetAsync(ws, 0, pl.flags_bytes, st) != hipSuccess) { xps_set_error("gru cluster backward: memset failed"); return XPS_E_HIP; }
     if (pl.CS * pl.U < pl.KP) {
         if (hipMemsetAsync(p.xbuf, 0, pl.xbuf_bwd, st) != hipSuccess) { xps_set_error("gru cluster backward: memset failed"); return XPS_E_HIP; }
     }
@@ -1942,6 +1983,57 @@
     return XPS_OK;
 }
 
+size_t xps_internal_gru_cluster_bwd_header(int B, int H, int ndir) {
+    const ClPlan2 p2 = cl_plan2(B, H, ndir);
+    if (xps_internal_gemm_mode() == 1 && p2.ok) return p2.flags_bytes;
+    const ClPlan pl = cl_plan(B, H, ndir);
+    return pl.ok ? pl.flags_bytes : 0;
+}
+
+bool xps_internal_gru_cluster_fold_ok(int B, int H) {
+    const ClPlan pl = cl_plan(B, H, 1);
+    return pl.ok && pl.CS * pl.U >= pl.KP;
+}
+
+static bool cl_init_args(ClInitArgs& ci, float* hs_next, int B, int H, void* workspace) {
+    const ClPlan pl = cl_plan(B, H, 1);
+    if (!pl.ok || pl.CS * pl.U < pl.KP || !cl_aligned16(hs_next) || !cl_aligned16(workspace)) return false;
+    unsigned char* ws = (unsigned char*)workspace;
+    ci.y_ext = hs_next; ci.xbuf = ws + pl.flags_bytes; ci.header = (u32x4*)ws; ci.header_u4 = (int)(pl.flags_bytes / 16);
+    ci.B = B; ci.H = H; ci.Bp = pl.Bp; ci.KP = pl.KP;
+    return true;
+}
+
+int xps_internal_decoder_select_init(const float* h, const float* w_fc, const float* b_fc, float* logits, long long ldl,
+                                     const long long* teacher, long long tstride, const int* use_teacher, const float* table,
+                                     long long* next, float* gi_next, float* hs_next, int B, int H, int C, int ntok,
+                                     void* workspace, hipStream_t st) {
+    ClInitArgs ci;
+    if (!cl_init_args(ci, hs_next, B, H, workspace)) { xps_set_error("decoder select: this shape has no folded recurrence set-up"); return XPS_E_INVALID; }
+    if (xps_internal_gemm_mode() == 1)
+        hipLaunchKernelGGL(decoder_select_init_kernel<true>, dim3((B + 3) / 4), dim3(256), 0, st, h, w_fc, b_fc, logits, ldl, teacher, tstride,
+                           use_teacher, table, next, gi_next, B, H, C, ntok, ci);
+    else
+        hipLaunchKernelGGL(decoder_select_init_kernel<false>, dim3((B + 3) / 4), dim3(256), 0, st, h, w_fc, b_fc, logits, ldl, teacher, tstride,
+                           use_teacher, table, next, gi_next, B, H, C, ntok, ci);
+    XPS_CHECK_LAUNCH();
+    return XPS_OK;
+}
+
+int xps_internal_decoder_start_init(const float* table, long long start, long long* tokens, float* gi, const float* h0, float* hs,
+                                    int B, int H, int ntok, void* workspace, hipStream_t st) {
+    ClInitArgs ci;
+    if (!cl_init_args(ci, hs, B, H, workspace) || !cl_aligned16(h0)) { xps_set_error("decoder start: this shape has no folded recurrence set-up"); return XPS_E_INVALID; }
+    const long long total = (long long)B * 3 * H;
+    const int blocks = (int)((total + 255) / 256 > 2048 ? 2048 : (total + 255) / 256);
+    if (xps_internal_gemm_mode() == 1)
+        hipLaunchKernelGGL(decoder_start_init_kernel<true>, dim3(blocks), dim3(256), 0, st, table, start, tokens, gi, B, 3 * H, ntok, h0, ci);
+    else
+        hipLaunchKernelGGL(decoder_start_init_kernel<false>, dim3(blocks), dim3(256), 0, st, table, start, tokens, gi, B, 3 * H, ntok, h0, ci);
+    XPS_CHECK_LAUNCH();
+    return XPS_OK;
+}
+
 extern "C" long long xps_debug_gru_bwd_status_offset(int B, int H, int ndir) {
     const ClPlan2 p2 = cl_plan2(B, H, ndir);
     if (xps_internal_gemm_mode() == 1 && p2.ok) return (long long)p2.flags_bytes - 256;
diff --git a/cross_patient_speech_decoding_amd/csrc/xps_nn.hip b/cross_patient_speech_decoding_amd/csrc/xps_nn.hip
--- a/cross_patient_speech_decoding_amd/csrc/xps_nn.hip
+++ b/cross_patient_speech_decoding_amd/csrc/xps_nn.hip
@@ -1,5 +1,13 @@
 #include "xps_common.h"
 #include "xps_ce.h"
+#include "xps_decoder_glue.h"
+
+int xps_internal_decoder_select_init(const float* h, const float* w_fc, const float* b_fc, float* logits, long long ldl,
+                                     const long long* teacher, long long tstride, const int* use_teacher, const float* table,
+                                     long long* next, float* gi_next, float* hs_next, int B, int H, int C, int ntok,
+                                     void* workspace, hipStream_t st);
+int xps_internal_decoder_start_init(const float* table, long long start, long long* tokens, float* gi, const float* h0, float* hs,
+                                    int B, int H, int ntok, void* workspace, hipStream_t st);
 
 namespace {
 
@@ -303,9 +311,8 @@
     next[b] = bi;
 }
 
-constexpr int SEL_MAXC = 16;
 __global__ __launch_bounds__(256) void decoder_select_kernel(const float* __restrict__ h, const float* __restrict__ w_fc,
-                                                             const float* __restrict__ b_fc, float* __restrict__ logits,
+                                                             const float* __restrict__ b_fc, float* __restrict__ logits, long long ldl,
                                                              const long long* __restrict__ teacher, long long tstride,
                                                              const int* __restrict__ use_teacher, const float* __restrict__ table,
                                                              long long* __restrict__ next, float* __restrict__ gi_next,
@@ -313,46 +320,13 @@
     const int lane = threadIdx.x & 63;
     const int b = blockIdx.x * 4 + (threadIdx.x >> 6);
     if (b >= B) return;
-    float acc[SEL_MAXC];
-#pragma unroll
-    for (int c = 0; c < SEL_MAXC; ++c) acc[c] = 0.f;
-    const float* hr = h + (long long)b * H;
-    for (int k = lane * 4; k < H; k += 256) {
-        const f32x4 hv = *reinterpret_cast<const f32x4*>(hr + k);
-#pragma unroll
-        for (int c = 0; c < SEL_MAXC; ++c) {
-            if (c < C) {
-                const f32x4 wv = *reinterpret_cast<const f32x4*>(w_fc + (long long)c * H + k);
-                acc[c] += (hv[0] * wv[0] + hv[1] * wv[1]) + (hv[2] * wv[2] + hv[3] * wv[3]);
-            }
-        }
-    }
-#pragma unroll
-    for (int c = 0; c < SEL_MAXC; ++c) {
-        if (c < C) {
-#pragma unroll
-            for (int o = 32; o > 0; o >>= 1) acc[c] += __shfl_xor(acc[c], o);
-        }
-    }
-    float best = 0.f;
-    int bi = 0;
-#pragma unroll
-    for (int c = 0; c < SEL_MAXC; ++c) {
-        if (c < C) {
-            const float v = acc[c] + b_fc[c];
-            if (lane == c) logits[(long long)b * C + c] = v;
-            if (c == 0 || v > best) { best = v; bi = c; }
-        }
-    }
-    if (!next) return;
-    long long tok = bi;
-    if (use_teacher && teacher && use_teacher[0]) tok = teacher[(long long)b * tstride];
-    if (lane == 0) next[b] = tok;
-    if (gi_next && tok >= 0 && tok < ntok) {
-        const float* src = table + tok * 3LL * H;
-        float* dst = gi_next + (long long)b * 3 * H;
-        for (int k = lane * 4; k < 3 * H; k += 256) *reinterpret_cast<f32x4*>(dst + k) = *reinterpret_cast<const f32x4*>(src + k);
-    }
+    decoder_select_row(h, w_fc, b_fc, logits, ldl, teacher, tstride, use_teacher, table, next, gi_next, b, lane, H, C, ntok);
+}
+
+__global__ void decoder_start_kernel(const float* __restrict__ table, long long start, long long* __restrict__ tokens,
+                                     float* __restrict__ gi, int B, int cols, int n_rows) {
+    decoder_start_rows(table, start, tokens, gi, B, cols, n_rows, (long long)blockIdx.x * blockDim.x + threadIdx.x,
+                       (long long)gridDim.x * blockDim.x);
 }
 
 __global__ void mask_scale_kernel(const float* __restrict__ x, const float* __restrict__ mask, float scale,
@@ -362,11 +336,11 @@
 }
 
 template <bool VEC>
-__global__ void dropout_kernel(const float* __restrict__ x, float* __restrict__ out, float* __restrict__ mask,
-                               long long n, float p, float scale, unsigned long long seed) {
+__device__ __forceinline__ void dropout_rows(const float* __restrict__ x, float* __restrict__ out, float* __restrict__ mask,
+                                             long long n, float p, float scale, unsigned long long seed, long long tid, long long nthreads) {
     if (VEC) {
         const long long nquad = n / 4;
-        for (long long q = (long long)blockIdx.x * blockDim.x + threadIdx.x; q < nquad; q += (long long)gridDim.x * blockDim.x) {
+        for (long long q = tid; q < nquad; q += nthreads) {
             const f32x4 m = dropout_keep4(seed, q, p);
             if (mask) *reinterpret_cast<f32x4*>(mask + 4 * q) = m;
             if (x) {
@@ -377,7 +351,7 @@
         return;
     }
     const long long npair = (n + 1) / 2;
-    for (long long q = (long long)blockIdx.x * blockDim.x + threadIdx.x; q < npair; q += (long long)gridDim.x * blockDim.x) {
+    for (long long q = tid; q < npair; q += nthreads) {
         float u0, u1;
         rng_pair(seed, q, u0, u1);
         const long long i = 2 * q;
@@ -395,6 +369,25 @@
     }
 }
 
+template <bool VEC>
+__global__ void dropout_kernel(const float* __restrict__ x, float* __restrict__ out, float* __restrict__ mask,
+                               long long n, float p, float scale, unsigned long long seed) {
+    dropout_rows<VEC>(x, out, mask, n, p, scale, seed, (long long)blockIdx.x * blockDim.x + threadIdx.x, (long long)gridDim.x * blockDim.x);
+}
+
+template <bool VEC>
+__global__ void conv_prologue_kernel(const float* __restrict__ conv_w, float* __restrict__ w2, int F, int Cin, int k,
+                                     float* __restrict__ mask, long long n, float p, unsigned long long seed) {
+    const long long tid = (long long)blockIdx.x * blockDim.x + threadIdx.x, nthreads = (long long)gridDim.x * blockDim.x;
+    const long long total = (long long)F * Cin * k;
+    for (long long i = tid; i < total; i += nthreads) {
+        const int c = (int)(i % Cin), kk = (int)((i / Cin) % k);
+        const long long f = i / ((long long)Cin * k);
+        w2[i] = conv_w[(f * Cin + c) * k + kk];
+    }
+    if (mask) dropout_rows<VEC>(nullptr, nullptr, mask, n, p, 1.0f / (1.0f - p), seed, tid, nthreads);
+}
+
 __global__ void split4_kernel(const float* __restrict__ x, float* __restrict__ out, long long nquad, float p, float scale,
                               unsigned long long seed) {
     for (long long q = (long long)blockIdx.x * blockDim.x + threadIdx.x; q < nquad; q += (long long)gridDim.x * blockDim.x) {
@@ -402,6 +395,14 @@
         if (p > 0.f) v = v * dropout_keep4(seed, q, p) * scale;
         *reinterpret_cast<f32x4*>(out + 4 * q) = split4_pack(v);
     }
+}
+
+struct Split4Batch { const float* x[4]; float* out[4]; };
+__global__ void split4_batched_kernel(Split4Batch sb, long long nquad) {
+    const float* __restrict__ x = sb.x[blockIdx.y];
+    float* __restrict__ out = sb.out[blockIdx.y];
+    for (long long q = (long long)blockIdx.x * blockDim.x + threadIdx.x; q < nquad; q += (long long)gridDim.x * blockDim.x)
+        *reinterpret_cast<f32x4*>(out + 4 * q) = split4_pack(*reinterpret_cast<const f32x4*>(x + 4 * q));
 }
 
 __global__ void add_kernel(const float* __restrict__ a, const float* __restrict__ b, float* __restrict__ out, long long n) {
@@ -758,8 +759,73 @@
     XPS_CHECK_ARG((bits & 15) == 0, "h, w_fc, table and gi_next must be 16-byte aligned");
     if (B == 0) return XPS_OK;
     hipLaunchKernelGGL(decoder_select_kernel, dim3(cdiv(B, 4)), dim3(256), 0, (hipStream_t)stream, h, w_fc, b_fc, logits,
-                       (const long long*)teacher, (long long)teacher_stride, (const int*)use_teacher, table, (long long*)next,
+                       (long long)C, (const long long*)teacher, (long long)teacher_stride, (const int*)use_teacher, table, (long long*)next,
                        gi_next, B, H, C, ntok);
+    XPS_CHECK_LAUNCH();
+    return XPS_OK;
+}
+
+extern "C" int xps_decoder_select_setup_f32(const float* h, const float* w_fc, const float* b_fc, float* logits, int64_t logits_ld,
+                                            const int64_t* teacher, int64_t teacher_stride, const int32_t* use_teacher,
+                                            const float* table, int64_t* next, float* gi_next, float* hs_next,
+                                            int B, int H, int C, int ntok, void* workspace, size_t workspace_bytes, void* stream) {
+    XPS_CHECK_ARG(h && w_fc && b_fc && logits && B >= 0 && H >= 4 && C >= 1 && logits_ld >= C, "bad argument");
+    XPS_CHECK_ARG(C <= SEL_MAXC && H % 4 == 0, "at most 16 classes, H a multiple of 4");
+    XPS_CHECK_ARG(!gi_next || (table && next && ntok >= 1), "the gather needs the table and the token output");
+    const uintptr_t bits = reinterpret_cast<uintptr_t>(h) | reinterpret_cast<uintptr_t>(w_fc) | reinterpret_cast<uintptr_t>(table) |
+                           reinterpret_cast<uintptr_t>(gi_next) | reinterpret_cast<uintptr_t>(hs_next);
+    XPS_CHECK_ARG((bits & 15) == 0, "h, w_fc, table, gi_next and hs_next must be 16-byte aligned");
+    if (B == 0) return XPS_OK;
+    if (hs_next) {
+        XPS_CHECK_ARG(xps_gru_seq_fwd_setup_folds(B, H), "hs_next: the shape must be one xps_gru_seq_fwd_setup_folds accepts");
+        if (!workspace || workspace_bytes < xps_gru_seq_fwd_f32_workspace(1, B, H, 1)) {
+            xps_set_error("xps_decoder_select_setup_f32: workspace too small");
+            return XPS_E_WORKSPACE;
+        }
+        return xps_internal_decoder_select_init(h, w_fc, b_fc, logits, (long long)logits_ld, (const long long*)teacher,
+                                                (long long)teacher_stride, (const int*)use_teacher, table, (long long*)next, gi_next,
+                                                hs_next, B, H, C, ntok, workspace, (hipStream_t)stream);
+    }
+    hipLaunchKernelGGL(decoder_select_kernel, dim3(cdiv(B, 4)), dim3(256), 0, (hipStream_t)stream, h, w_fc, b_fc, logits,
+                       (long long)logits_ld, (const long long*)teacher, (long long)teacher_stride, (const int*)use_teacher, table,
+                       (long long*)next, gi_next, B, H, C, ntok);
+    XPS_CHECK_LAUNCH();
+    return XPS_OK;
+}
+
+extern "C" int xps_decoder_start_f32(const float* table, int64_t start_token, int64_t* tokens, float* gi, const float* h0, float* hs,
+                                     int B, int H, int ntok, void* workspace, size_t workspace_bytes, void* stream) {
+    XPS_CHECK_ARG(table && tokens && gi && B >= 0 && H >= 1 && ntok >= 1, "bad argument");
+    XPS_CHECK_ARG((h0 == nullptr) == (hs == nullptr), "h0 and hs must both be given or both NULL");
+    if (B == 0) return XPS_OK;
+    if (hs) {
+        XPS_CHECK_ARG(xps_gru_seq_fwd_setup_folds(B, H), "h0 / hs: the shape must be one xps_gru_seq_fwd_setup_folds accepts");
+        if (!workspace || workspace_bytes < xps_gru_seq_fwd_f32_workspace(1, B, H, 1)) {
+            xps_set_error("xps_decoder_start_f32: workspace too small");
+            return XPS_E_WORKSPACE;
+        }
+        return xps_internal_decoder_start_init(table, (long long)start_token, (long long*)tokens, gi, h0, hs, B, H, ntok, workspace,
+                                               (hipStream_t)stream);
+    }
+    hipLaunchKernelGGL(decoder_start_kernel, dim3(ew_grid((long long)B * 3 * H)), dim3(256), 0, (hipStream_t)stream, table,
+                       (long long)start_token, (long long*)tokens, gi, B, 3 * H, ntok);
+    XPS_CHECK_LAUNCH();
+    return XPS_OK;
+}
+
+extern "C" int xps_conv_prologue_f32(const float* conv_w, float* w2, int F, int Cin, int k, float* mask, int64_t n, float p,
+                                     uint64_t seed, void* stream) {
+    XPS_CHECK_ARG(conv_w && w2 && F >= 1 && Cin >= 1 && k >= 1, "bad argument");
+    XPS_CHECK_ARG(!mask || (n >= 0 && p >= 0.f && p < 1.f), "mask: n >= 0, 0 <= p < 1");
+    XPS_CHECK_ARG((reinterpret_cast<uintptr_t>(mask) & 7) == 0, "mask must be 8-byte aligned");
+    const long long total = (long long)F * Cin * k;
+    const bool vec = mask && (reinterpret_cast<uintptr_t>(mask) & 15) == 0 && n % 4 == 0;
+    const long long work = !mask ? total : (vec ? n / 4 : (n + 1) / 2);
+    const int grid = ew_grid(work > total ? work : total);
+    if (vec) hipLaunchKernelGGL(conv_prologue_kernel<true>, dim3(grid), dim3(256), 0, (hipStream_t)stream, conv_w, w2, F, Cin, k, mask,
+                                (long long)n, p, (unsigned long long)seed);
+    else hipLaunchKernelGGL(conv_prologue_kernel<false>, dim3(grid), dim3(256), 0, (hipStream_t)stream, conv_w, w2, F, Cin, k, mask,
+                            (long long)n, p, (unsigned long long)seed);
     XPS_CHECK_LAUNCH();
     return XPS_OK;
 }
@@ -801,6 +867,23 @@
     return XPS_OK;
 }
 
+extern "C" int xps_split4_batched_f32(const float* const* x, float* const* out, int count, int64_t n, void* stream) {
+    XPS_CHECK_ARG(x && out && count >= 1 && count <= 4 && n >= 0 && n % 4 == 0, "bad argument (1..4 tensors, n a multiple of 4)");
+    Split4Batch sb;
+    uintptr_t bits = 0;
+    for (int i = 0; i < 4; ++i) {
+        const int j = i < count ? i : 0;
+        XPS_CHECK_ARG(x[j] && out[j], "null tensor pointer");
+        sb.x[i] = x[j]; sb.out[i] = out[j];
+        bits |= reinterpret_cast<uintptr_t>(x[j]) | reinterpret_cast<uintptr_t>(out[j]);
+    }
+    XPS_CHECK_ARG((bits & 15) == 0, "buffers must be 16-byte aligned");
+    if (n == 0) return XPS_OK;
+    hipLaunchKernelGGL(split4_batched_kernel, dim3(ew_grid(n / 4), count), dim3(256), 0, (hipStream_t)stream, sb, (long long)(n / 4));
+    XPS_CHECK_LAUNCH();
+    return XPS_OK;
+}
+
 namespace {
 __global__ __launch_bounds__(256) void split4_pad_kernel(const float* __restrict__ x, long long ldx, int rows, int cols, float* __restrict__ out,
                                                          long long ldo) {
diff --git a/cross_patient_speech_decoding_amd/nn_models/functional.py b/cross_patient_speech_decoding_amd/nn_models/functional.py
--- a/cross_patient_speech_decoding_amd/nn_models/functional.py
+++ b/cross_patient_speech_decoding_amd/nn_models/functional.py
@@ -343,29 +343,18 @@
         dhn = dhn.contiguous()
     if dy is None and dhn is None:
         dhn = torch.zeros(ndir, B, H, dtype=_f32, device=dev)
-    if len(w_hh) > 1:
-        w_t = [torch.empty(H, 3 * H, dtype=_f32, device=dev) for _ in w_hh]
-        call('xps_transpose_batched_f32', _ptr_array(w_hh), _ptr_array(w_t), len(w_hh), 3 * H, H, _stream())
-    else:
-        w_t = [transpose(w, 3 * H, H) for w in w_hh]
+    w_t = [torch.empty(H, 3 * H, dtype=_f32, device=dev) for _ in w_hh]
     dgi = torch.empty(ndir, T, B, 3 * H, dtype=_f32, device=dev)
     dghn = torch.empty(ndir, T, B, H, dtype=_f32, device=dev)
     dh0 = torch.empty(ndir, B, H, dtype=_f32, device=dev) if need_dh0 else None
     nbytes = _gru_ws_bytes('xps_gru_seq_bwd_f32_workspace', T, B, H, ndir)
     ws = _ws(nbytes, dev)
     _gru_status_register(dev)
-    if split4:
-        fused = drop is not None and dy is not None
-        call('xps_gru_seq_bwd_split4_f32', _ptr(dy), _ptr(dhn), _ptr(y_ext), _ptr(saved), _ptr_array(w_hh), _ptr_array(w_t), _ptr(dgi),
-             _ptr(dghn), _ptr(dh0), T, B, H, ndir, float(drop[0]) if fused else 0.0, int(drop[1]) if fused else 0, _ptr(ws), nbytes,
-             _stream())
-        return dgi, dghn, dh0
-    if drop is not None and dy is not None:
-        call('xps_gru_seq_bwd_drop_f32', _ptr(dy), _ptr(dhn), _ptr(y_ext), _ptr(saved), _ptr_array(w_hh), _ptr_array(w_t), _ptr(dgi),
-             _ptr(dghn), _ptr(dh0), T, B, H, ndir, float(drop[0]), int(drop[1]), _ptr(ws), nbytes, _stream())
-        return dgi, dghn, dh0
-    call('xps_gru_seq_bwd_f32', _ptr(dy), _ptr(dhn), _ptr(y_ext), _ptr(saved), _ptr_array(w_hh), _ptr_array(w_t), _ptr(dgi),
-         _ptr(dghn), _ptr(dh0), T, B, H, ndir, _ptr(ws), nbytes, _stream())
+    call('xps_gru_seq_bwd_setup_f32', _ptr_array(w_hh), _ptr_array(w_t), T, B, H, ndir, _ptr(ws), nbytes, _stream())
+    fused = drop is not None and dy is not None
+    call('xps_gru_seq_bwd_ready_f32', _ptr(dy), _ptr(dhn), _ptr(y_ext), _ptr(saved), _ptr_array(w_hh), _ptr_array(w_t), _ptr(dgi),
+         _ptr(dghn), _ptr(dh0), T, B, H, ndir, float(drop[0]) if fused else 0.0, int(drop[1]) if fused else 0, int(bool(split4)),
+         _ptr(ws), nbytes, _stream())
     return dgi, dghn, dh0
 
 
@@ -459,6 +448,14 @@
     return out
 
 
+def split4_all(xs):
+    if len(xs) < 2 or len(xs) > 4 or any(x.shape != xs[0].shape for x in xs):
+        return [split4(x) for x in xs]
+    outs = [torch.empty_like(x) for x in xs]
+    call('xps_split4_batched_f32', _ptr_array(xs), _ptr_array(outs), len(xs), xs[0].numel(), _stream())
+    return outs
+
+
 class GruPlan(NamedTuple):
     cluster_on: bool
     precision: int
@@ -507,7 +504,7 @@
         plan = ctx.plan = gru_layer_plan(T, B, In, H, ndir, drop_p, fmt)
         gi = torch.empty(ndir, T, B, 3 * H, dtype=_f32, device=x.device)
         if plan.w_fmt:
-            w_ih = [split4(w) for w in w_ih]
+            w_ih = split4_all(w_ih)
         ra, rb, rc = rowmap(In, fmt=plan.x_fmt), rowmap(In, fmt=plan.w_fmt), rowmap(3 * H)
         call('xps_gemm_nt_multi_f32', _ptr(x), C.byref(ra), _ptr_array(w_ih), C.byref(rb), _ptr_array([gi[d] for d in range(ndir)]),
              C.byref(rc), _ptr_array(b_ih), ndir, T * B, 3 * H, In, _stream())
@@ -662,7 +659,7 @@
 
     @staticmethod
     def forward(ctx, x, conv_w, conv_b, gamma, beta, running_mean, running_var, stride, training,
-                relu, drop_mask, drop_scale, momentum, eps, group, global_trials=None, num_batches_tracked=None):
+                relu, drop_mask, drop_scale, momentum, eps, group, global_trials=None, num_batches_tracked=None, drop_gen=None):
         _need_gpu(x, conv_w)
         x = x.contiguous()
         B, T, Cin = x.shape
@@ -670,8 +667,14 @@
         Tp = (T - k) // stride + 1
         if Tp < 1:
             raise ValueError('TemporalConv: sequence shorter than the kernel')
-        w2 = conv_w.permute(0, 2, 1).contiguous().view(F, k * Cin)
         rows = Tp * B
+        w2 = torch.empty(F, k * Cin, dtype=_f32, device=x.device)
+        if drop_mask is None and drop_gen is not None and training:
+            drop_mask = torch.empty(Tp, B, F, dtype=_f32, device=x.device)
+            call('xps_conv_prologue_f32', _ptr(conv_w.contiguous()), _ptr(w2), F, Cin, k, _ptr(drop_mask), drop_mask.numel(),
+                 float(drop_gen[0]), int(drop_gen[1]), _stream())
+        else:
+            call('xps_conv_prologue_f32', _ptr(conv_w.contiguous()), _ptr(w2), F, Cin, k, None, 0, 0.0, 0, _stream())
         y = torch.empty(Tp, B, F, dtype=_f32, device=x.device)
         ra = rowmap(stride * Cin, rpg=Tp, gs=T * Cin)
         rc = rowmap(B * F, rpg=Tp, gs=F)
@@ -744,7 +747,7 @@
             dconv_w = None
         else:
             dconv_w = dw2.view(F, k, Cin).permute(0, 2, 1).contiguous()
-        return (None, dconv_w, r_cb, dgamma, dbeta) + (None,) * 12
+        return (None, dconv_w, r_cb, dgamma, dbeta) + (None,) * 13
 
 
 def decoder_supported(H, C, L):
@@ -850,37 +853,46 @@
             teacher = teacher.contiguous()
             if tuple(teacher.shape) != (B, L):
                 raise ValueError('teacher tokens must be (batch, seq_length)')
-        steps = torch.empty(L, B, C, dtype=_f32, device=dev)
         tokens = torch.empty(L, B, dtype=torch.int64, device=dev)
-        tokens[0].fill_(int(start_token))
         hs = torch.empty(L + 2, B, H, dtype=_f32, device=dev)
         saved = torch.empty(1, L, B, 4 * H, dtype=_f32, device=dev) if save else None
         ctx.form = _launch_form(B, H)
         gi = torch.empty(B, 3 * H, dtype=_f32, device=dev)
         nbytes = _gru_ws_bytes('xps_gru_seq_fwd_f32_workspace', 1, B, H, 1)
+        ws = _ws(nbytes, dev)
         _gru_status_register(dev)
         w_arr, b_arr = _ptr_array([w_hh_c]), _ptr_array([b_hh_c])
-        rc = rowmap(C)
         fused_select = C <= 16
-        for s in range(L):
-            if s == 0 or not fused_select:
-                call('xps_gather_rows_f32', _ptr(table), _ptr(tokens[s]), _ptr(gi), B, 3 * H, ntok, _stream())
-            ws = _ws(nbytes, dev)
-            call('xps_gru_seq_fwd_f32', _ptr(gi), w_arr, b_arr, _ptr(h0c if s == 0 else hs[s]), _ptr(hs[s:]),
-                 _ptr(saved[0, s]) if save else None, 1, B, H, 1, _ptr(ws), nbytes, _stream())
-            tstride = teacher.stride(0) if teacher is not None else 0
-            if fused_select:
+        tstride = teacher.stride(0) if teacher is not None else 0
+        if fused_select:
+            fold = bool(lib().xps_gru_seq_fwd_setup_folds(B, H))
+            fwd = 'xps_gru_seq_fwd_ready_f32' if fold else 'xps_gru_seq_fwd_f32'
+            logits = torch.empty(B, L, C, dtype=_f32, device=dev)
+            call('xps_decoder_start_f32', _ptr(table), int(start_token), _ptr(tokens[0]), _ptr(gi), _ptr(h0c) if fold else None,
+                 _ptr(hs) if fold else None, B, H, ntok, _ptr(ws) if fold else None, nbytes if fold else 0, _stream())
+            for s in range(L):
+                call(fwd, _ptr(gi), w_arr, b_arr, _ptr(h0c if s == 0 else hs[s]), _ptr(hs[s:]),
+                     _ptr(saved[0, s]) if save else None, 1, B, H, 1, _ptr(ws), nbytes, _stream())
                 last = s + 1 == L
-                call('xps_decoder_select_f32', _ptr(hs[s + 1]), _ptr(w_fc_c), _ptr(b_fc_c), _ptr(steps[s]),
+                nxt = fold and not last
+                call('xps_decoder_select_setup_f32', _ptr(hs[s + 1]), _ptr(w_fc_c), _ptr(b_fc_c), _ptr(logits[:, s]), L * C,
                      _ptr(teacher[:, s]) if (teacher is not None and not last) else None, tstride,
                      _ptr(flags[s:s + 1]) if (teacher is not None and not last) else None, _ptr(table),
-                     None if last else _ptr(tokens[s + 1]), None if last else _ptr(gi), B, H, C, ntok, _stream())
-                continue
-            gemm_nt(hs[s + 1], w_fc_c, steps[s], B, C, H, bias=b_fc_c, rc=rc)
-            if s + 1 < L:
-                call('xps_next_token', _ptr(steps[s]), C, _ptr(teacher[:, s]) if teacher is not None else None, tstride,
-                     _ptr(flags[s:s + 1]) if teacher is not None else None, _ptr(tokens[s + 1]), B, _stream())
-        logits = steps.permute(1, 0, 2).contiguous()
+                     None if last else _ptr(tokens[s + 1]), None if last else _ptr(gi), _ptr(hs[s + 1:]) if nxt else None,
+                     B, H, C, ntok, _ptr(ws) if nxt else None, nbytes if nxt else 0, _stream())
+        else:
+            steps = torch.empty(L, B, C, dtype=_f32, device=dev)
+            tokens[0].fill_(int(start_token))
+            rc = rowmap(C)
+            for s in range(L):
+                call('xps_gather_rows_f32', _ptr(table), _ptr(tokens[s]), _ptr(gi), B, 3 * H, ntok, _stream())
+                call('xps_gru_seq_fwd_f32', _ptr(gi), w_arr, b_arr, _ptr(h0c if s == 0 else hs[s]), _ptr(hs[s:]),
+                     _ptr(saved[0, s]) if save else None, 1, B, H, 1, _ptr(ws), nbytes, _stream())
+                gemm_nt(hs[s + 1], w_fc_c, steps[s], B, C, H, bias=b_fc_c, rc=rc)
+                if s + 1 < L:
+                    call('xps_next_token', _ptr(steps[s]), C, _ptr(teacher[:, s]) if teacher is not None else None, tstride,
+                         _ptr(flags[s:s + 1]) if teacher is not None else None, _ptr(tokens[s + 1]), B, _stream())
+            logits = steps.permute(1, 0, 2).contiguous()
         if save:
             ctx.save_for_backward(tokens, hs, saved, w_hh_c, w_fc_c)
         ctx.params = (w_hh, b_hh, w_fc, b_fc)
diff --git a/cross_patient_speech_decoding_amd/nn_models/models.py b/cross_patient_speech_decoding_amd/nn_models/models.py
--- a/cross_patient_speech_decoding_amd/nn_models/models.py
+++ b/cross_patient_speech_decoding_amd/nn_models/models.py
@@ -78,17 +78,17 @@
         Tp = (T - k) // s + 1
         F = self.conv.out_channels
         training = self.training
-        mask, scale, p = None, 1.0, self.dropout.p
+        gen, scale, p = None, 1.0, self.dropout.p
         if training and p > 0:
-            mask = XF.dropout_mask((Tp, B, F), p, x.device)
+            gen = (float(p), XF.next_dropout_seed())
             scale = 1.0 / (1.0 - p)
         momentum = 0.1 if self.bn.momentum is None else self.bn.momentum
         nbt = self.bn.num_batches_tracked if training and self.bn.track_running_stats else None
         return XF.TemporalConvFn.apply(x, self.conv.weight, self.conv.bias, self.bn.weight, self.bn.bias,
                                        self.bn.running_mean, self.bn.running_var, s, training,
-                                       bool(self.activation), mask, scale, momentum, self.bn.eps,
+                                       bool(self.activation), None, scale, momentum, self.bn.eps,
                                        self.process_group, self.global_batch if self.process_group is not None else None,
-                                       nbt)
+                                       nbt, gen)
 
     def forward(self, x):
         return self.forward_tm(x.permute(0, 2, 1)).permute(1, 2, 0)
diff --git a/include/xps.h b/include/xps.h
--- a/include/xps.h
+++ b/include/xps.h
@@ -101,7 +101,19 @@
 
 int xps_transpose_f32(const float* src, float* dst, int rows, int cols, void* stream);
 int xps_transpose_batched_f32(const float* const* src, float* const* dst, int n, int rows, int cols, void* stream);
-
+int xps_gru_seq_bwd_setup_f32(const float* const* w_hh, float* const* w_hh_t, int T, int B, int H, int ndir,
+                              void* workspace, size_t workspace_bytes, void* stream);
+int xps_gru_seq_bwd_ready_f32(const float* dy, const float* dhn, const float* y_ext, const float* saved,
+                              const float* const* w_hh, const float* const* w_hh_t, float* dgi, float* dghn, float* dh0,
+                              int T, int B, int H, int ndir, float drop_p, uint64_t drop_seed, int split_out,
+                              void* workspace, size_t workspace_bytes, void* stream);
+int xps_gru_seq_fwd_setup_folds(int B, int H);
+int xps_gru_seq_fwd_ready_f32(const float* gi, const float* const* w_hh, const float* const* b_hh,
+                              const float* h0, float* y_ext, float* saved,
+                              int T, int B, int H, int ndir, void* workspace, size_t workspace_bytes, void* stream);
+
+int xps_conv_prologue_f32(const float* conv_w, float* w2, int F, int Cin, int k, float* mask, int64_t n, float p,
+                          uint64_t seed, void* stream);
 int xps_bn_centered_sumsq_f32(const float* y, int rows, int F, const float* stats, double count, float* out_sq,
                               void* workspace, size_t workspace_bytes, void* stream);
 int xps_bn_finalize_f32(const float* stats, double count, float* mean, float* rstd,
@@ -167,8 +179,15 @@
 int xps_decoder_select_f32(const float* h, const float* w_fc, const float* b_fc, float* logits,
                            const int64_t* teacher, int64_t teacher_stride, const int32_t* use_teacher,
                            const float* table, int64_t* next, float* gi_next, int B, int H, int C, int ntok, void* stream);
+int xps_decoder_select_setup_f32(const float* h, const float* w_fc, const float* b_fc, float* logits, int64_t logits_ld,
+                                 const int64_t* teacher, int64_t teacher_stride, const int32_t* use_teacher,
+                                 const float* table, int64_t* next, float* gi_next, float* hs_next,
+                                 int B, int H, int C, int ntok, void* workspace, size_t workspace_bytes, void* stream);
+int xps_decoder_start_f32(const float* table, int64_t start_token, int64_t* tokens, float* gi, const float* h0, float* hs,
+                          int B, int H, int ntok, void* workspace, size_t workspace_bytes, void* stream);
 int xps_dropout_f32(const float* x, float* out, float* mask, int64_t n, float p, uint64_t seed, void* stream);
 int xps_split4_f32(const float* x, float* out, int64_t n, float drop_p, uint64_t seed, void* stream);
+int xps_split4_batched_f32(const float* const* x, float* const* out, int count, int64_t n, void* stream);
 int xps_split4_pad_f32(const float* x, int64_t ldx, int rows, int cols, float* out, int64_t ldo, void* stream);
 int xps_mask_scale_f32(const float* x, const float* mask, float scale, float* out, int64_t n, void* stream);
 int xps_add_f32(const float* a, const float* b, float* out, int64_t n, void* stream);
```
